# WHOIGit/ifcb_classifier

Measured on AMD Instinct MI355X. Metric: train images/sec, inception_v3 299^2 IFCB ROIs, higher is better.
Workload: dtype bf16; 1 GPU; inception_v3 100-class bf16 TRAIN, batch 256 per GPU, synthetic u8 ROIs h,w~U{32..299} resized on-GPU to 299x299 (BASELINE.json configs[1]); global_batch=256, parallelism=dp1, program_lanes=4, IFCBK_LANES=4, weight_gradient_lanes=1, optimizer=adam lr=1e-3, loss=CE + 0.4*CE_aux, input_pipeline=preprocess then step on one stream

## Files before the change

ifcb_classifier_amd/_lib.py:

```python
import ctypes as C
import os

_HERE = os.path.dirname(os.path.abspath(__file__))
LIB_PATH = os.path.join(_HERE, 'libifcbk.so')
if os.environ.get('IFCBK_LIB'):
    _alt = os.environ['IFCBK_LIB']
    if not (os.path.isabs(_alt) and os.path.isfile(_alt)):
        raise RuntimeError('IFCBK_LIB must be the absolute path of an existing libifcbk build, got %r' % _alt)
    import sys as _sys
    print('[ifcbk] IFCBK_LIB: loading %s instead of the in-tree library' % _alt, file=_sys.stderr)
    LIB_PATH = _alt

BF16, F32 = 0, 1
OK, EINVAL, EHIP, ENOMEM, EUNSUPPORTED = 0, -1, -2, -3, -4

(OP_CONV_FWD, OP_CONV_DGRAD, OP_CONV_WGRAD, OP_WEIGHT_PACK, OP_BN_FINALIZE, OP_BN_APPLY, OP_BN_BWD,
 OP_MAXPOOL_FWD, OP_MAXPOOL_BWD, OP_AVGPOOL_FWD, OP_AVGPOOL_BWD, OP_HEAD_FWD, OP_HEAD_BWD,
 OP_SOFTMAX_XENT, OP_SOFTMAX, OP_ADAM, OP_MEMSET, OP_COPY2D, OP_DROPOUT_MASK, OP_CONV_FWD_AFFINE,
 OP_WEIGHT_PACK_MULTI, OP_CONV_WGRAD_SEG, OP_BN_APPLY_MAXPOOL, OP_BN_BWD_MAXPOOL, OP_CONV_DGRAD_BNSTAT,
 OP_BN_BWD_PARTIALS, OP_BN_STATS, OP_AVGPOOL_AFFINE, OP_CONV_FWD_AFFINE_SEG, OP_SGD, OP_RETIRED_31,
 OP_BIAS_RELU_BWD, OP_DROPOUT, OP_FLATTEN_CHW, OP_STEM_U8_FWD, OP_STEM_U8_WGRAD, OP_CONV_FWD_AFFINE_MAXPOOL,
 OP_STEP_COUNTERS, OP_CONV_WGRAD_GROUP, OP_SOFTMAX_XENT_W) = range(1, 41)

OP_NAMES = {1: 'conv_fwd', 2: 'conv_dgrad', 3: 'conv_wgrad', 4: 'weight_pack', 5: 'bn_finalize', 6: 'bn_apply',
            7: 'bn_bwd', 8: 'maxpool_fwd', 9: 'maxpool_bwd', 10: 'avgpool_fwd', 11: 'avgpool_bwd', 12: 'head_fwd',
            13: 'head_bwd', 14: 'softmax_xent', 15: 'softmax', 16: 'adam', 17: 'memset', 18: 'copy2d',
            19: 'dropout_mask', 20: 'conv_fwd_affine', 21: 'weight_pack_multi', 22: 'conv_wgrad', 23: 'bn_apply_maxpool',
            24: 'bn_bwd_maxpool', 25: 'conv_dgrad', 26: 'bn_bwd', 27: 'bn_stats', 28: 'avgpool_fwd', 29: 'conv_fwd_affine', 30: 'sgd', 31: 'retired',
            32: 'bias_relu_bwd', 33: 'dropout', 34: 'flatten_chw', 35: 'conv_fwd', 36: 'conv_wgrad', 37: 'conv_fwd_affine', 38: 'step_counters', 39: 'conv_wgrad',
            40: 'softmax_xent_w'}


class ConvDesc(C.Structure):
    _fields_ = [(n, C.c_int32) for n in
                ('N', 'H', 'W', 'C', 'ldx', 'K', 'R', 'S', 'stride_h', 'stride_w', 'pad_h', 'pad_w', 'P', 'Q',
                 'ldy', 'Cw', 'dtype')]


class BnDesc(C.Structure):
    _fields_ = [(n, C.c_int32) for n in ('M', 'C', 'ldx', 'ldy', 'relu', 'dtype')] + \
               [('eps', C.c_float), ('momentum', C.c_float)]


class PoolDesc(C.Structure):
    _fields_ = [(n, C.c_int32) for n in
                ('N', 'H', 'W', 'C', 'ldx', 'R', 'S', 'stride_h', 'stride_w', 'pad_h', 'pad_w', 'P', 'Q', 'ldy',
                 'dtype')]


class HeadDesc(C.Structure):
    _fields_ = [(n, C.c_int32) for n in ('N', 'HW', 'C', 'ldx', 'NC', 'dtype')] + [('keep_scale', C.c_float)]


class RoiDesc(C.Structure):
    _fields_ = [(n, C.c_int32) for n in ('n_img', 'S', 'in_channels', 'out_channels', 'flip_bits_valid', 'dtype')] + \
               [('mean', C.c_float * 3), ('std', C.c_float * 3), ('tin_scale', C.c_float * 3),
                ('tin_shift', C.c_float * 3)]


class WgradItem(C.Structure):
    _fields_ = [('d', ConvDesc), ('x', C.c_void_p), ('dy', C.c_void_p), ('dw', C.c_void_p)]


class PackItem(C.Structure):
    _fields_ = [('w_master', C.c_void_p), ('w', C.c_void_p), ('wT', C.c_void_p), ('K', C.c_int32), ('RS', C.c_int32),
                ('C', C.c_int32), ('Cw', C.c_int32), ('first_block', C.c_int64), ('wT_ld', C.c_int32), ('pad_', C.c_int32)]


class _OpU(C.Union):
    _fields_ = [('conv', ConvDesc), ('bn', BnDesc), ('pool', PoolDesc), ('head', HeadDesc)]


class Op(C.Structure):
    _fields_ = [('kind', C.c_int32), ('flags', C.c_int32), ('p', C.c_void_p * 12), ('i', C.c_int64 * 4),
                ('f', C.c_float * 8), ('u', _OpU)]


_vp, _i, _f, _sz = C.c_void_p, C.c_int, C.c_float, C.c_size_t
_PROTOS = {
    'ifcbk_version': (C.c_char_p, []),
    'ifcbk_ctx_create': (_i, [_i, C.POINTER(_vp)]),
    'ifcbk_ctx_destroy': (_i, [_vp]),
    'ifcbk_ctx_reserve': (_i, [_vp, _sz]),
    'ifcbk_ctx_workspace_bytes': (_sz, [_vp]),
    'ifcbk_ctx_set_lanes': (_i, [_vp, _i]),
    'ifcbk_ctx_live_graphs': (_i, [_vp]),
    'ifcbk_last_error': (C.c_char_p, [_vp]),
    'ifcbk_conv2d_fwd': (_i, [_vp, C.POINTER(ConvDesc), _vp, _vp, _vp, _vp, _vp]),
    'ifcbk_conv2d_fwd_affine': (_i, [_vp, C.POINTER(ConvDesc), _vp, _vp, _vp, _vp, _vp, _vp, _i, _i, _vp]),
    'ifcbk_conv2d_fwd_affine_maxpool_ok': (_i, [C.POINTER(ConvDesc)]),
    'ifcbk_conv2d_fwd_affine_maxpool': (_i, [_vp, C.POINTER(ConvDesc), _vp, _vp, _vp, _i, _vp, _vp, _i, _vp]),
    'ifcbk_conv2d_dgrad': (_i, [_vp, C.POINTER(ConvDesc), _vp, _vp, _vp, _i, _vp]),
    'ifcbk_conv2d_wgrad': (_i, [_vp, C.POINTER(ConvDesc), _vp, _vp, _vp, _i, _vp]),
    'ifcbk_conv2d_wgrad_segments': (_i, [_vp, C.POINTER(ConvDesc), _vp, _vp, _i, C.POINTER(_vp), C.POINTER(C.c_int32), _i, _vp]),
    'ifcbk_bn_finalize_ld': (_i, [_vp, C.POINTER(BnDesc), _vp, _i, _i] + [_vp] * 9),
    'ifcbk_conv2d_wgrad_workspace': (_sz, [C.POINTER(ConvDesc)]),
    'ifcbk_conv2d_wgrad_group': (_i, [_vp, _i, C.POINTER(ConvDesc), C.POINTER(_vp), C.POINTER(_vp), C.POINTER(_vp), _i, _vp]),
    'ifcbk_conv2d_wgrad_group_workspace': (_sz, [_i, C.POINTER(ConvDesc)]),
    'ifcbk_conv2d_wgrad_group_member_kh': (_i, [C.POINTER(ConvDesc)]),
    'ifcbk_conv2d_wgrad_group_info': (_i, [_i, C.POINTER(ConvDesc), C.POINTER(_i), C.POINTER(_i), C.POINTER(_i)]),
    'ifcbk_conv2d_fwd_mblocks': (_i, [C.POINTER(ConvDesc)]),
    'ifcbk_weight_pack': (_i, [_vp, C.POINTER(ConvDesc), _vp, _vp, _vp, _vp]),
    'ifcbk_weight_pack_multi': (_i, [_vp, _vp, _i, C.c_int64, _i, _vp]),
    'ifcbk_bn_finalize': (_i, [_vp, C.POINTER(BnDesc), _vp, _i] + [_vp] * 9),
    'ifcbk_bn_apply': (_i, [_vp, C.POINTER(BnDesc), _vp, _vp, _vp, _vp, _i, _vp, _vp]),
    'ifcbk_bn_bwd': (_i, [_vp, C.POINTER(BnDesc), _vp, _vp, _vp, _i, _vp, _vp, _vp, _vp, _i, _vp, _i, _i, _vp, _vp,
                          _i, _vp, _vp, _vp]),
    'ifcbk_conv2d_fwd_affine_segments': (_i, [_vp, C.POINTER(ConvDesc), _vp, _vp, _i, C.POINTER(_vp), C.POINTER(C.c_int32),
                                          C.POINTER(C.c_int32), C.POINTER(C.c_int32), _vp, _vp, _vp]),
    'ifcbk_avgpool3x3_affine': (_i, [_vp, C.POINTER(PoolDesc), _vp, _vp, _vp, _i, _vp, _vp]),
    'ifcbk_bn_stats_rows': (_i, [C.c_int64]),
    'ifcbk_bn_stats': (_i, [_vp, C.POINTER(BnDesc), _vp, _vp, _vp]),
    'ifcbk_conv2d_dgrad_bnstat_mblocks': (_i, [C.POINTER(ConvDesc)]),
    'ifcbk_conv2d_dgrad_bnstat': (_i, [_vp, C.POINTER(ConvDesc), _vp, _vp, _vp, _vp, _i, _vp, _vp, _vp, _vp, _vp, _vp]),
    'ifcbk_bn_bwd_partials': (_i, [_vp, C.POINTER(BnDesc), _vp, _vp, _i, _vp, _vp, _vp, _vp, _vp, _vp, _i, _vp, _i, _vp, _vp, _i,
                                   _vp]),
    'ifcbk_bn_bwd_partials_ld': (_i, [_vp, C.POINTER(BnDesc), _vp, _vp, _i, _vp, _vp, _vp, _vp, _vp, _vp, _i, _i, _vp, _i, _vp, _vp,
                                      _i, _vp]),
    'ifcbk_bn_apply_maxpool': (_i, [_vp, C.POINTER(PoolDesc), _vp, _vp, _vp, _i, _vp, _vp, _vp]),
    'ifcbk_bn_bwd_maxpool': (_i, [_vp, C.POINTER(PoolDesc), _vp, _vp, _vp, _vp, _vp, _vp, _vp, _vp, _i, _vp, _i, _vp, _vp, _i,
                                  _vp]),
    'ifcbk_maxpool_fwd': (_i, [_vp, C.POINTER(PoolDesc), _vp, _vp, _vp, _vp]),
    'ifcbk_maxpool_bwd': (_i, [_vp, C.POINTER(PoolDesc), _vp, _vp, _vp, _i, _vp]),
    'ifcbk_avgpool_fwd': (_i, [_vp, C.POINTER(PoolDesc), _vp, _vp, _vp]),
    'ifcbk_avgpool_bwd': (_i, [_vp, C.POINTER(PoolDesc), _vp, _vp, _i, _vp]),
    'ifcbk_head_fwd': (_i, [_vp, C.POINTER(HeadDesc), _vp, _vp, _vp, _vp, _vp, _vp, _vp]),
    'ifcbk_head_bwd': (_i, [_vp, C.POINTER(HeadDesc), _vp, _vp, _vp, _vp, _vp, _vp, _vp, _i, _i, _vp]),
    'ifcbk_dropout_mask': (_i, [_vp, _vp, C.c_int64, _f, C.c_uint64, C.c_uint64, _vp]),
    'ifcbk_bias_relu_bwd': (_i, [_vp, C.c_int64, _i, _i, _vp, _i, _vp, _i, _vp, _i, _i, _vp, _i, _vp]),
    'ifcbk_bias_relu_bwd_workspace': (_sz, [C.c_int64, _i]),
    'ifcbk_bias_relu_bwd_rows': (_i, [C.c_int64]),
    'ifcbk_dropout_apply': (_i, [_vp, C.c_int64, _i, _vp, _vp, _f, _vp, _i, _vp]),
    'ifcbk_flatten_chw': (_i, [_vp, _i, _i, _i, _i, _vp, _i, _vp, _i, _i, _vp]),
    'ifcbk_softmax_xent': (_i, [_vp, _vp, _vp, _i, _i, _f, _vp, _i, _vp, _vp]),
    'ifcbk_softmax': (_i, [_vp, _vp, _i, _i, _vp, _vp]),
    'ifcbk_softmax_xent_w': (_i, [_vp, _vp, _vp, _vp, _i, _i, _f, _vp, _i, _vp, _vp]),
    'ifcbk_step_counters': (_i, [_vp, _vp, _i, _vp, _vp, _vp]),
    'ifcbk_adam_flat': (_i, [_vp, _vp, _vp, _vp, _vp, C.c_int64, _f, _f, _f, _f, _f, _i, _f, _vp]),
    'ifcbk_sgd_flat': (_i, [_vp, _vp, _vp, _vp, C.c_int64, _f, _f, _f, _f, _vp]),
    'ifcbk_roi_preprocess': (_i, [_vp, C.POINTER(RoiDesc), _vp, _vp, _vp, _vp, _vp, _i, _i, _vp, _vp, _vp]),
    'ifcbk_roi_preprocess_workspace': (_sz, [C.POINTER(RoiDesc), _i, _i]),
    'ifcbk_u8_channel_moments': (_i, [_vp, _vp, _i, C.c_int64, _i, _vp, _vp]),
    'ifcbk_stem_u8_rows': (_i, [C.POINTER(ConvDesc)]),
    'ifcbk_stem_u8_fwd': (_i, [_vp, C.POINTER(ConvDesc), _vp, _vp, _vp, _vp, _vp, _vp, _vp, _i, _vp]),
    'ifcbk_stem_u8_wgrad_workspace': (_sz, [C.POINTER(ConvDesc)]),
    'ifcbk_stem_u8_wgrad': (_i, [_vp, C.POINTER(ConvDesc), _vp, _vp, _vp, _vp, _i, _vp]),
    'ifcbk_nchw_to_nhwc': (_i, [_vp, _vp, _i, _i, _i, _i, _i, _i, C.POINTER(_f), C.POINTER(_f), _vp, _vp]),
    'ifcbk_nhwc_to_nchw_f32': (_i, [_vp, _vp, _i, _i, _i, _i, _i, _i, _vp, _vp]),
    'ifcbk_run_program': (_i, [_vp, C.POINTER(Op), _i, _vp, C.POINTER(_f)]),
    'ifcbk_run_program_ev': (_i, [_vp, C.POINTER(Op), _i, _vp, _i]),
    'ifcbk_program_times': (_i, [_vp, _i, _i, C.POINTER(_f)]),
    'ifcbk_program_capture': (_i, [_vp, C.POINTER(Op), _i, C.POINTER(_vp)]),
    'ifcbk_graph_launch': (_i, [_vp, _vp, _vp]),
    'ifcbk_graph_destroy': (_i, [_vp, _vp]),
    'ifcbk_op_kernel': (_i, [C.POINTER(Op), C.c_char_p, _sz]),
    'ifcbk_op_cost': (_i, [C.POINTER(Op), C.POINTER(C.c_double), C.POINTER(C.c_double)]),
}
EXPORTS = tuple(_PROTOS)

_lib = None


def load():
    global _lib
    if _lib is None:
        if not os.path.exists(LIB_PATH):
            raise RuntimeError('libifcbk.so not found at %s -- build it with `python -c "import __graft_entry__ as g; '
                               'g.build()"` (hipcc --offload-arch=gfx950); there is no CPU fallback' % LIB_PATH)
        import torch
        lib = C.CDLL(LIB_PATH)
        for name, (res, args) in _PROTOS.items():
            fn = getattr(lib, name)
            fn.restype = res
            fn.argtypes = args
        _lib = lib
    return _lib


class Context:

    def __init__(self, device=0):
        self.lib = load()
        h = _vp()
        rc = self.lib.ifcbk_ctx_create(int(device), C.byref(h))
        if rc != 0:
            raise RuntimeError('ifcbk_ctx_create(device=%d) failed with %d: %s' % (device, rc, self.lib.ifcbk_last_error(None).decode()))
        self.h = h
        self.device = device

    def call(self, name, *args):
        rc = getattr(self.lib, name)(self.h, *args)
        if rc != 0:
            raise RuntimeError('%s failed (%d): %s' % (name, rc, self.lib.ifcbk_last_error(self.h).decode()))

    def reserve(self, nbytes):
        self.call('ifcbk_ctx_reserve', int(nbytes))

    def run_program(self, ops, n, stream, op_ms=None):
        self.call('ifcbk_run_program', ops, int(n), stream, op_ms)

    def capture(self, ops, n):
        g = _vp()
        self.call('ifcbk_program_capture', ops, int(n), C.byref(g))
        return g

    def graph_launch(self, g, stream):
        self.call('ifcbk_graph_launch', g, stream)

    def live_graphs(self):
        return int(self.lib.ifcbk_ctx_live_graphs(self.h)) if self.h else 0

    def close(self):
        if getattr(self, 'h', None):
            self.lib.ifcbk_ctx_destroy(self.h)
            self.h = None

    def __del__(self):
        try:
            self.close()
        except Exception:
            pass


class PlanOnlyContext:

    def __init__(self):
        self.lib = load()
        self.h = None
        self.device = None

    def reserve(self, nbytes):
        pass

    def close(self):
        pass

    def call(self, name, *args):
        raise RuntimeError('%s: this engine was built with plan_only=True (no HIP context)' % name)

    run_program = capture = graph_launch = call


def ptr(t):
    return None if t is None else _vp(t.data_ptr())


def cur_stream():
    import torch
    return _vp(torch.cuda.current_stream().cuda_stream)
```

ifcb_classifier_amd/csrc/bn.hip:

```cpp
#include "common.h"
#include <stdlib.h>

namespace {

#ifdef IFCBK_EXPERIMENT_NOFINALIZE
__global__ void experiment_empty_kernel(float* p) { if (p && threadIdx.x == 1000) p[0] = 0.f; }
bool experiment_skip_finalize(hipStream_t st) {
    static const char* e = getenv("IFCBK_EXPERIMENT_NOFINALIZE");
    static const char* k = getenv("IFCBK_EXPERIMENT_EMPTYFINALIZE");
    static long seen = 0;
    if (!e) return false;
    const bool skip = ++seen > atol(e);
    if (skip && k) hipLaunchKernelGGL(experiment_empty_kernel, dim3(1), dim3(64), 0, st, (float*)nullptr);
    return skip;
}
#else
constexpr bool experiment_skip_finalize(hipStream_t) { return false; }
#endif

__global__ __launch_bounds__(1024) void bn_finalize_kernel(const float* part, int mblocks, int ldp, int C, double invM,
                                                            double unbias, const float* gamma, const float* beta,
                                                            float* rmean, float* rvar, float* mean_o, float* invstd_o,
                                                            float* scale, float* shift, float eps, float momentum) {
    __shared__ double s1[64][16], s2[64][16];
// ... 437 lines not shown
        }
    }
#pragma unroll
    for (int off = 8; off < 64; off <<= 1)
#pragma unroll
        for (int j = 0; j < E; ++j) {
            sb[j] += __shfl_xor(sb[j], off);
            sg[j] += __shfl_xor(sg[j], off);
        }
    if (lane < 8) {
#pragma unroll
        for (int j = 0; j < E; ++j) {
            red[wave][0][cc * E + j] = sb[j];
            red[wave][1][cc * E + j] = sg[j];
        }
    }
    __syncthreads();
    if (t < 2 * CG) {
        int which = t / CG, n = t - which * CG;
        int ch = blockIdx.y * CG + n;
        if (ch < C) {
            float s = red[0][which][n] + red[1][which][n] + red[2][which][n] + red[3][which][n];
            part[((size_t)blockIdx.x * 2 + which) * C + ch] = s;
        }
    }
}

__global__ __launch_bounds__(1024) void bn_bwd_finalize_kernel(const float* part, int ntiles, int C, float* dgamma,
                                                                float* dbeta, float* tmp, int accumulate, int ldp) {
    __shared__ double s[2][64][16];
    const int c = threadIdx.x & 15, rg = threadIdx.x >> 4;
    const int ch = blockIdx.x * 16 + c;
    double a = 0.0, b = 0.0;
    if (ch < C) {
        int i = rg;
        for (; i + 192 < ntiles; i += 256) {
            float v[8];
#pragma unroll
            for (int u = 0; u < 4; ++u) {
                v[2 * u] = part[((size_t)(i + 64 * u) * 2 + 0) * ldp + ch];
                v[2 * u + 1] = part[((size_t)(i + 64 * u) * 2 + 1) * ldp + ch];
            }
#pragma unroll
            for (int u = 0; u < 4; ++u) {
                a += (double)v[2 * u];
                b += (double)v[2 * u + 1];
            }
        }
        for (; i < ntiles; i += 64) {
            a += (double)part[((size_t)i * 2 + 0) * ldp + ch];
            b += (double)part[((size_t)i * 2 + 1) * ldp + ch];
        }
    }
    s[0][rg][c] = a;
    s[1][rg][c] = b;
    __syncthreads();
    if (threadIdx.x < 16 && ch < C) {
        double sa = 0.0, sg = 0.0;
        for (int i = 0; i < 64; ++i) {
            sa += s[0][i][c];
            sg += s[1][i][c];
        }
        tmp[ch] = (float)sa;
        tmp[C + ch] = (float)sg;
        dbeta[ch] = accumulate ? dbeta[ch] + (float)sa : (float)sa;
        dgamma[ch] = accumulate ? dgamma[ch] + (float)sg : (float)sg;
    }
}

template <class T, int MASK, bool POOLED>
__global__ __launch_bounds__(256) void bn_bwd_dx_kernel(const T* x, int ldx, const T* y, int ldy, const T* dy, int lddy,
                                                         const float* gamma, const float* mean, const float* invstd,
                                                         const float* scale, const float* shift, const float* tmp,
                                                         T* dx, int lddx, T* dres, int lddres, int dres_acc, int64_t M,
                                                         int C, float invM, fastdiv_t fcpr, PoolGather pg) {
    constexpr int E = Chunk<T>::N;
    extern __shared__ __attribute__((aligned(16))) float coef[];
    for (int c = threadIdx.x; c < C; c += 256) {
        float is = invstd[c], a_ = gamma[c] * is, dg = tmp[C + c] * invM, db = tmp[c] * invM;
        coef[c] = a_;
        coef[C + c] = -a_ * is * dg;
        coef[2 * C + c] = a_ * (mean[c] * is * dg - db);
        if (MASK == 2) {
            coef[3 * C + c] = scale[c];
            coef[4 * C + c] = shift[c];
        }
    }
    __syncthreads();
    const int cpr = C / E;
    const int64_t total = M * cpr;
    int64_t i = (int64_t)blockIdx.x * (256 * EW_ITER) + threadIdx.x;
#pragma unroll 2
    for (int it = 0; it < EW_ITER; ++it, i += 256) {
        if (i >= total) break;
        uint32_t m = fdiv((uint32_t)i, fcpr);
        int c = ((int)i - (int)m * cpr) * E;
        float fx[E], fy[E], fd[E], o[E];
        Chunk<T>::load(x + (int64_t)m * ldx + c, fx);
        if (POOLED) pooled_dy<T>(pg, dy, m, c, fd);
        else Chunk<T>::load(dy + (int64_t)m * lddy + c, fd);
        if (MASK == 1) Chunk<T>::load(y + (int64_t)m * ldy + c, fy);
#pragma unroll
        for (int j = 0; j < E; ++j) {
            float dz = fd[j];
            if (MASK == 1) dz = fy[j] > 0.f ? dz : 0.f;
            if (MASK == 2) dz = (fx[j] * coef[3 * C + c + j] + coef[4 * C + c + j]) > 0.f ? dz : 0.f;
            fd[j] = dz;
            o[j] = coef[c + j] * dz + (coef[C + c + j] * fx[j] + coef[2 * C + c + j]);
        }
        if (dres_acc & 2) {
            float fo[E];
            Chunk<T>::load(dx + (int64_t)m * lddx + c, fo);
#pragma unroll
            for (int j = 0; j < E; ++j) o[j] += fo[j];
        }
        if (dres) {
            T* rp = dres + (int64_t)m * lddres + c;
            if (dres_acc & 1) {
                float fr[E];
                Chunk<T>::load(rp, fr);
#pragma unroll
                for (int j = 0; j < E; ++j) fd[j] += fr[j];
            }
            Chunk<T>::store(rp, fd);
        }
        Chunk<T>::store(dx + (int64_t)m * lddx + c, o);
    }
}

template <class T>
int apply_t(ifcbk_ctx* ctx, const ifcbk_bn_desc* d, const void* x, const float* scale, const float* shift,
            const void* residual, int ldr, void* y, hipStream_t st) {
    constexpr int E = Chunk<T>::N;
    if (d->C % E || d->ldx % E || d->ldy % E) IFCBK_FAIL(ctx, IFCBK_EINVAL, "bn_apply: channels must be multiples of %d", E);
    const int cpr = d->C / E;
    const int64_t total = (int64_t)d->M * cpr;
    if (total >= (1ll << 31)) IFCBK_FAIL(ctx, IFCBK_EINVAL, "bn_apply: tensor too large");
    dim3 grid(cdiv(total, 256 * EW_ITER)), block(256);
    const size_t shm = (size_t)2 * d->C * sizeof(float);
    const fastdiv_t fc = make_fastdiv(cpr);
    const T* xx = (const T*)x; const T* rr = (const T*)residual; T* yy = (T*)y;
    if (d->relu && rr) hipLaunchKernelGGL((bn_apply_kernel<T, true, true>), grid, block, shm, st, xx, d->ldx, scale, shift, rr, ldr, yy, d->ldy, (int64_t)d->M, cpr, fc);
    else if (d->relu) hipLaunchKernelGGL((bn_apply_kernel<T, true, false>), grid, block, shm, st, xx, d->ldx, scale, shift, rr, ldr, yy, d->ldy, (int64_t)d->M, cpr, fc);
    else if (rr) hipLaunchKernelGGL((bn_apply_kernel<T, false, true>), grid, block, shm, st, xx, d->ldx, scale, shift, rr, ldr, yy, d->ldy, (int64_t)d->M, cpr, fc);
    else hipLaunchKernelGGL((bn_apply_kernel<T, false, false>), grid, block, shm, st, xx, d->ldx, scale, shift, rr, ldr, yy, d->ldy, (int64_t)d->M, cpr, fc);
    IFCBK_LAUNCH_CHECK(ctx, "bn_apply");
    return 0;
}

template <class T>
int bwd_t(ifcbk_ctx* ctx, const ifcbk_bn_desc* d, const void* x, const void* y, const void* dy, int lddy,
          const float* gamma, const float* mean, const float* invstd, void* dx, int lddx, void* dres, int lddres,
          int dres_accumulate, float* dgamma, float* dbeta, int param_accumulate, const float* scale, const float* shift,
          hipStream_t st, const PoolGather* pool = nullptr, const float* part_in = nullptr, int ntiles_in = 0, int part_ld_in = 0) {
    constexpr int E = Chunk<T>::N;
    constexpr int CG = 8 * E;
    PoolGather pg = {};
    if (pool) pg = *pool;
    const int C = d->C;
    if (C % E || d->ldx % E || lddy % E || lddx % E) IFCBK_FAIL(ctx, IFCBK_EINVAL, "bn_bwd: channels must be multiples of %d", E);
    const int64_t M = d->M;
    const int rows = bwd_rows(M, cdiv(C, CG));
    int ntiles = cdiv(M, rows);
    size_t need = ((size_t)ntiles * 2 * C + 2 * C) * sizeof(float);
    if (need > ctx->ws_bytes) IFCBK_FAIL(ctx, IFCBK_ENOMEM, "bn_bwd: workspace %zu > reserved %zu", need, ctx->ws_bytes);
    float* part = (float*)ctx->ws;
    float* tmp = part + (size_t)ntiles * 2 * C;
    const T* xx = (const T*)x; const T* yy = (const T*)y; const T* dd = (const T*)dy;
    dim3 g1(ntiles, cdiv(C, CG));
    const int mask = !d->relu ? 0 : ((scale && shift && !dres) ? 2 : 1);
    if (mask == 1 && !yy) IFCBK_FAIL(ctx, IFCBK_EINVAL, "bn_bwd: y is required for the ReLU mask");
    if (pool && pg.ph == 0 && pg.pw == 0) {
        if (mask == 1) IFCBK_FAIL(ctx, IFCBK_EINVAL, "bn_bwd_maxpool: needs scale/shift (the activation is not stored)");
        const int HB = (pg.H + 1) / 2, WB = (pg.W + 1) / 2;
        const int64_t nblk = (int64_t)(M / ((int64_t)pg.H * pg.W)) * HB * WB;
        const int64_t tot = nblk * (C / E);
        if (tot >= (1ll << 31) - 256) IFCBK_FAIL(ctx, IFCBK_EINVAL, "bn_bwd_maxpool: tensor too large");
        const int nt2 = cdiv(nblk, 256);
        if (((size_t)nt2 * 2 * C + 2 * C) * sizeof(float) > ctx->ws_bytes) IFCBK_FAIL(ctx, IFCBK_ENOMEM, "bn_bwd_maxpool: workspace");
        float* tmp2 = part + (size_t)nt2 * 2 * C;
        const fastdiv_t fHBWB = make_fastdiv(HB * WB), fWB = make_fastdiv(WB), fc2 = make_fastdiv(C / E);
        dim3 g2(nt2, cdiv(C, CG));
        if (mask == 2) hipLaunchKernelGGL((bn_bwd_reduce_pool2x2_kernel<T, 2>), g2, dim3(256), 0, st, xx, d->ldx, dd, mean, invstd, scale, shift, part, C, pg, HB, WB, (uint32_t)nblk, fHBWB, fWB);
        else hipLaunchKernelGGL((bn_bwd_reduce_pool2x2_kernel<T, 0>), g2, dim3(256), 0, st, xx, d->ldx, dd, mean, invstd, scale, shift, part, C, pg, HB, WB, (uint32_t)nblk, fHBWB, fWB);
        IFCBK_LAUNCH_CHECK(ctx, "bn_bwd_reduce_pool2x2");
        if (!experiment_skip_finalize(st)) hipLaunchKernelGGL(bn_bwd_finalize_kernel, dim3(cdiv(C, 16)), dim3(1024), 0, st, (const float*)part, nt2, C, dgamma, dbeta, tmp2, param_accumulate, C);
        IFCBK_LAUNCH_CHECK(ctx, "bn_bwd_finalize");
        const float invM2 = (float)(1.0 / (double)M);
        const size_t shm2 = (size_t)5 * C * sizeof(float);
        if (mask == 2) hipLaunchKernelGGL((bn_bwd_dx_pool2x2_kernel<T, 2>), dim3(cdiv(tot, 256)), dim3(256), shm2, st, xx, d->ldx, dd, gamma, mean, invstd, scale, shift, (const float*)tmp2, (T*)dx, lddx, C, invM2, pg, HB, WB, (uint32_t)tot, fc2, fHBWB, fWB);
        else hipLaunchKernelGGL((bn_bwd_dx_pool2x2_kernel<T, 0>), dim3(cdiv(tot, 256)), dim3(256), shm2, st, xx, d->ldx, dd, gamma, mean, invstd, scale, shift, (const float*)tmp2, (T*)dx, lddx, C, invM2, pg, HB, WB, (uint32_t)tot, fc2, fHBWB, fWB);
        IFCBK_LAUNCH_CHECK(ctx, "bn_bwd_dx_pool2x2");
        return 0;
    }
    if (part_in) {
        if (mask != 2 || dres) IFCBK_FAIL(ctx, IFCBK_EINVAL, "bn_bwd_partials: ReLU layer without residual, scale/shift required");
        part = const_cast<float*>(part_in);
        ntiles = ntiles_in;
        tmp = (float*)ctx->ws;
        if ((size_t)2 * C * sizeof(float) > ctx->ws_bytes) IFCBK_FAIL(ctx, IFCBK_ENOMEM, "bn_bwd_partials: workspace");
    } else if (pool) {
        if (mask == 1) IFCBK_FAIL(ctx, IFCBK_EINVAL, "bn_bwd_maxpool: needs scale/shift (the activation is not stored)");
        if (mask == 2) hipLaunchKernelGGL((bn_bwd_reduce_kernel<T, 2, true>), g1, dim3(256), 0, st, xx, d->ldx, yy, d->ldy, dd, lddy, mean, invstd, scale, shift, part, M, C, pg, rows);
        else hipLaunchKernelGGL((bn_bwd_reduce_kernel<T, 0, true>), g1, dim3(256), 0, st, xx, d->ldx, yy, d->ldy, dd, lddy, mean, invstd, scale, shift, part, M, C, pg, rows);
    } else if (mask == 2) hipLaunchKernelGGL((bn_bwd_reduce_kernel<T, 2, false>), g1, dim3(256), 0, st, xx, d->ldx, yy, d->ldy, dd, lddy, mean, invstd, scale, shift, part, M, C, pg, rows);
    else if (mask == 1) hipLaunchKernelGGL((bn_bwd_reduce_kernel<T, 1, false>), g1, dim3(256), 0, st, xx, d->ldx, yy, d->ldy, dd, lddy, mean, invstd, scale, shift, part, M, C, pg, rows);
    else hipLaunchKernelGGL((bn_bwd_reduce_kernel<T, 0, false>), g1, dim3(256), 0, st, xx, d->ldx, yy, d->ldy, dd, lddy, mean, invstd, scale, shift, part, M, C, pg, rows);
    IFCBK_LAUNCH_CHECK(ctx, "bn_bwd_reduce");
    if (!experiment_skip_finalize(st)) hipLaunchKernelGGL(bn_bwd_finalize_kernel, dim3(cdiv(C, 16)), dim3(1024), 0, st, (const float*)part, ntiles, C, dgamma, dbeta, tmp, param_accumulate, (part_in && part_ld_in > 0) ? part_ld_in : C);
    IFCBK_LAUNCH_CHECK(ctx, "bn_bwd_finalize");
    const int64_t total = M * (C / E);
    if (total >= (1ll << 31)) IFCBK_FAIL(ctx, IFCBK_EINVAL, "bn_bwd: tensor too large");
    const float invM = (float)(1.0 / (double)M);
    dim3 g3(cdiv(total, 256 * EW_ITER));
    const size_t shm = (size_t)5 * C * sizeof(float);
    const fastdiv_t fc = make_fastdiv(C / E);
    if (pool) {
        if (mask == 2) hipLaunchKernelGGL((bn_bwd_dx_kernel<T, 2, true>), g3, dim3(256), shm, st, xx, d->ldx, yy, d->ldy, dd, lddy, gamma, mean, invstd, scale, shift, (const float*)tmp, (T*)dx, lddx, (T*)dres, lddres, dres_accumulate, M, C, invM, fc, pg);
        else hipLaunchKernelGGL((bn_bwd_dx_kernel<T, 0, true>), g3, dim3(256), shm, st, xx, d->ldx, yy, d->ldy, dd, lddy, gamma, mean, invstd, scale, shift, (const float*)tmp, (T*)dx, lddx, (T*)dres, lddres, dres_accumulate, M, C, invM, fc, pg);
    } else if (mask == 2) hipLaunchKernelGGL((bn_bwd_dx_kernel<T, 2, false>), g3, dim3(256), shm, st, xx, d->ldx, yy, d->ldy, dd, lddy, gamma, mean, invstd, scale, shift, (const float*)tmp, (T*)dx, lddx, (T*)dres, lddres, dres_accumulate, M, C, invM, fc, pg);
    else if (mask == 1) hipLaunchKernelGGL((bn_bwd_dx_kernel<T, 1, false>), g3, dim3(256), shm, st, xx, d->ldx, yy, d->ldy, dd, lddy, gamma, mean, invstd, scale, shift, (const float*)tmp, (T*)dx, lddx, (T*)dres, lddres, dres_accumulate, M, C, invM, fc, pg);
    else hipLaunchKernelGGL((bn_bwd_dx_kernel<T, 0, false>), g3, dim3(256), shm, st, xx, d->ldx, yy, d->ldy, dd, lddy, gamma, mean, invstd, scale, shift, (const float*)tmp, (T*)dx, lddx, (T*)dres, lddres, dres_accumulate, M, C, invM, fc, pg);
    IFCBK_LAUNCH_CHECK(ctx, "bn_bwd_dx");
    return 0;
}

}

extern "C" int ifcbk_bn_finalize(ifcbk_ctx* ctx, const ifcbk_bn_desc* d, const float* part, int mblocks,
                                 const float* gamma, const float* beta, float* running_mean, float* running_var,
                                 float* mean, float* invstd, float* scale, float* shift, void* stream) {
    return ifcbk_bn_finalize_ld(ctx, d, part, mblocks, 0, gamma, beta, running_mean, running_var, mean, invstd, scale, shift, stream);
}

extern "C" int ifcbk_bn_finalize_ld(ifcbk_ctx* ctx, const ifcbk_bn_desc* d, const float* part, int mblocks, int part_ld,
                                    const float* gamma, const float* beta, float* running_mean, float* running_var,
                                    float* mean, float* invstd, float* scale, float* shift, void* stream) {
    if (!d || d->C <= 0) IFCBK_FAIL(ctx, IFCBK_EINVAL, "bn_finalize: bad desc");
    hipStream_t st = (hipStream_t)stream;
    int ldp = part_ld > 0 ? part_ld : d->C;
    if (part) {
        double M = (double)d->M;
        double unbias = d->M > 1 ? M / (M - 1.0) : 1.0;
        if (mblocks > 1536) {
            const int rpc = 64;
            int nchunk = cdiv(mblocks, rpc);
            size_t need = (size_t)nchunk * 2 * d->C * sizeof(float);
            if (need > ctx->ws_bytes) IFCBK_FAIL(ctx, IFCBK_ENOMEM, "bn_finalize: workspace %zu > reserved %zu", need, ctx->ws_bytes);
            hipLaunchKernelGGL(bn_prereduce_kernel, dim3(cdiv(d->C, 64), nchunk), dim3(256), 0, st, part, mblocks, ldp, d->C, rpc,
                               (float*)ctx->ws);
            IFCBK_LAUNCH_CHECK(ctx, "bn_prereduce");
            part = (const float*)ctx->ws;
            mblocks = nchunk;
            ldp = d->C;
        }
        if (!experiment_skip_finalize(st)) hipLaunchKernelGGL(bn_finalize_kernel, dim3(cdiv(d->C, 16)), dim3(1024), 0, st, part, mblocks, ldp, d->C, 1.0 / M,
                           unbias, gamma, beta, running_mean, running_var, mean, invstd, scale, shift, d->eps,
                           d->momentum);
    } else {
        hipLaunchKernelGGL(bn_eval_scale_kernel, dim3(cdiv(d->C, 256)), dim3(256), 0, st, d->C, gamma, beta,
                           (const float*)running_mean, (const float*)running_var, scale, shift, d->eps);
    }
    IFCBK_LAUNCH_CHECK(ctx, "bn_finalize");
    return 0;
}

extern "C" int ifcbk_bn_stats_rows(int64_t M) { return (int)((M + STAT_ROWS - 1) / STAT_ROWS); }

extern "C" int ifcbk_bn_stats(ifcbk_ctx* ctx, const ifcbk_bn_desc* d, const void* x, float* part, void* stream) {
    if (!d || !x || !part) IFCBK_FAIL(ctx, IFCBK_EINVAL, "bn_stats: null operand");
    if (d->dtype != IFCBK_BF16 && d->dtype != IFCBK_F32) IFCBK_FAIL(ctx, IFCBK_EUNSUPPORTED, "bn_stats: dtype must be bf16 or f32");
    const int e = dtype_chunk(d->dtype);
    if (d->C % e || d->ldx % e || d->M <= 0) IFCBK_FAIL(ctx, IFCBK_EINVAL, "bn_stats: C=%d ldx=%d must be multiples of %d, M > 0", d->C, d->ldx, e);
    const dim3 grid((unsigned)ifcbk_bn_stats_rows(d->M), (unsigned)cdiv(d->C, 8 * e));
    if (d->dtype == IFCBK_F32) hipLaunchKernelGGL(bn_stats_kernel<float>, grid, dim3(256), 0, (hipStream_t)stream, (const float*)x, d->ldx, part, d->M, d->C);
    else hipLaunchKernelGGL(bn_stats_kernel<bf16_t>, grid, dim3(256), 0, (hipStream_t)stream, (const bf16_t*)x, d->ldx, part, d->M, d->C);
    IFCBK_LAUNCH_CHECK(ctx, "bn_stats");
    return 0;
}

extern "C" int ifcbk_bn_apply(ifcbk_ctx* ctx, const ifcbk_bn_desc* d, const void* x, const float* scale,
                              const float* shift, const void* residual, int ldr, void* y, void* stream) {
    if (!d) IFCBK_FAIL(ctx, IFCBK_EINVAL, "bn_apply: null desc");
    if (d->dtype == IFCBK_F32) return apply_t<float>(ctx, d, x, scale, shift, residual, ldr, y, (hipStream_t)stream);
    if (d->dtype == IFCBK_BF16) return apply_t<bf16_t>(ctx, d, x, scale, shift, residual, ldr, y, (hipStream_t)stream);
    IFCBK_FAIL(ctx, IFCBK_EINVAL, "bn_apply: bad dtype");
}

extern "C" int ifcbk_bn_bwd(ifcbk_ctx* ctx, const ifcbk_bn_desc* d, const void* x, const void* y, const void* dy,
                            int lddy, const float* gamma, const float* mean, const float* invstd, void* dx, int lddx,
                            void* dres, int lddres, int dres_accumulate, float* dgamma, float* dbeta,
                            int param_accumulate, const float* scale, const float* shift, void* stream) {
    if (!d) IFCBK_FAIL(ctx, IFCBK_EINVAL, "bn_bwd: null desc");
    if (d->dtype == IFCBK_F32)
        return bwd_t<float>(ctx, d, x, y, dy, lddy, gamma, mean, invstd, dx, lddx, dres, lddres, dres_accumulate, dgamma,
                            dbeta, param_accumulate, scale, shift, (hipStream_t)stream);
    if (d->dtype == IFCBK_BF16)
        return bwd_t<bf16_t>(ctx, d, x, y, dy, lddy, gamma, mean, invstd, dx, lddx, dres, lddres, dres_accumulate, dgamma,
                             dbeta, param_accumulate, scale, shift, (hipStream_t)stream);
    IFCBK_FAIL(ctx, IFCBK_EINVAL, "bn_bwd: bad dtype");
}

namespace {
struct ApplyPoolArgs {
    int H, W, P, Q, cpr, ldx, ldy, sh, sw, ph, pw, relu;
    uint32_t total;
    fastdiv_t f_cpr, f_q, f_p;
};
template <class T>
__global__ __launch_bounds__(256) void bn_apply_maxpool_kernel(const T* x, const float* scale, const float* shift, T* y,
                                                               uint8_t* arg, ApplyPoolArgs a) {
    constexpr int E = Chunk<T>::N;
    extern __shared__ __attribute__((aligned(16))) float coef[];
    const int C = a.cpr * E;
    for (int c = threadIdx.x; c < C; c += 256) {
        coef[c] = scale[c];
        coef[C + c] = shift[c];
    }
    __syncthreads();
    const uint32_t i = xcd_remap(blockIdx.x, gridDim.x) * 256u + threadIdx.x;
    if (i >= a.total) return;
    const uint32_t pix = fdiv(i, a.f_cpr);
    const int c = (int)(i - pix * a.cpr) * E;
    const uint32_t t2 = fdiv(pix, a.f_q);
    const int q = (int)(pix - t2 * a.Q);
    const uint32_t n = fdiv(t2, a.f_p);
    const int p = (int)(t2 - n * a.P);
    const int h0 = p * a.sh - a.ph, w0 = q * a.sw - a.pw;
    float sc[E], sf[E], best[E];
    int bi[E];
#pragma unroll
    for (int j = 0; j < E; ++j) { sc[j] = coef[c + j]; sf[j] = coef[C + c + j]; best[j] = -INFINITY; bi[j] = 0; }
    typename Chunk<T>::raw_t rv[9];
#pragma unroll
    for (int r = 0; r < 3; ++r)
#pragma unroll
        for (int s = 0; s < 3; ++s) {
            const int h = min(max(h0 + r, 0), a.H - 1), w = min(max(w0 + s, 0), a.W - 1);
            rv[r * 3 + s] = Chunk<T>::load_raw(x + ((int64_t)(n * a.H + h) * a.W + w) * a.ldx + c);
        }
    bool first = true;
#pragma unroll
    for (int r = 0; r < 3; ++r)
#pragma unroll
        for (int s = 0; s < 3; ++s) {
            const int h = h0 + r, w = w0 + s;
            const bool in = h >= 0 && h < a.H && w >= 0 && w < a.W;
            float f[E];
            Chunk<T>::widen(rv[r * 3 + s], f);
#pragma unroll
            for (int j = 0; j < E; ++j) {
                float v = f[j] * sc[j] + sf[j];
                if (a.relu) v = fmaxf(v, 0.f);
                v = Chunk<T>::round(v);
                if (in && (first || v > best[j] || v != v)) { best[j] = v; bi[j] = r * 3 + s; }
            }
            first = first && !in;
        }
    Chunk<T>::store(y + (int64_t)pix * a.ldy + c, best);
    if (arg) ArgPack<E>::store(arg + (int64_t)pix * C + c, bi);
}

int pooled_check(ifcbk_ctx* ctx, const ifcbk_pool_desc* d, const char* who) {
    if (!d || (d->dtype != IFCBK_BF16 && d->dtype != IFCBK_F32)) IFCBK_FAIL(ctx, IFCBK_EINVAL, "%s: bad desc", who);
    const int e = dtype_chunk(d->dtype);
    if (d->C % e || d->ldx % e || d->ldy % e) IFCBK_FAIL(ctx, IFCBK_EINVAL, "%s: channels must be multiples of %d", who, e);
    if (d->R != 3 || d->S != 3 || d->stride_h != 2 || d->stride_w != 2 || d->pad_h > 1 || d->pad_w > 1 || d->pad_h < 0 || d->pad_w < 0)
        IFCBK_FAIL(ctx, IFCBK_EUNSUPPORTED, "%s: only 3x3 / stride 2 / pad <= 1 max pools are fused", who);
    if ((int64_t)d->N * d->H * d->W * (d->C / e) >= (1ll << 31) - 256) IFCBK_FAIL(ctx, IFCBK_EINVAL, "%s: tensor too large", who);
    return 0;
}
}

extern "C" int ifcbk_bn_apply_maxpool(ifcbk_ctx* ctx, const ifcbk_pool_desc* d, const void* x, const float* scale,
                                      const float* shift, int relu, void* y, uint8_t* argmax, void* stream) {
    if (int e = pooled_check(ctx, d, "bn_apply_maxpool")) return e;
    ApplyPoolArgs a;
    a.H = d->H; a.W = d->W; a.P = d->P; a.Q = d->Q; a.ldx = d->ldx; a.ldy = d->ldy;
    a.sh = 2; a.sw = 2; a.ph = d->pad_h; a.pw = d->pad_w; a.relu = relu;
    a.cpr = d->C / dtype_chunk(d->dtype);
    a.total = (uint32_t)((int64_t)d->N * d->P * d->Q * a.cpr);
    a.f_cpr = make_fastdiv(a.cpr); a.f_q = make_fastdiv(d->Q); a.f_p = make_fastdiv(d->P);
    if (a.total == 0) return IFCBK_OK;
    const size_t shm = (size_t)2 * d->C * sizeof(float);
    hipStream_t st = (hipStream_t)stream;
    if (d->dtype == IFCBK_F32) hipLaunchKernelGGL(bn_apply_maxpool_kernel<float>, dim3(cdiv(a.total, 256)), dim3(256), shm, st, (const float*)x, scale, shift, (float*)y, argmax, a);
    else hipLaunchKernelGGL(bn_apply_maxpool_kernel<bf16_t>, dim3(cdiv(a.total, 256)), dim3(256), shm, st, (const bf16_t*)x, scale, shift, (bf16_t*)y, argmax, a);
    IFCBK_LAUNCH_CHECK(ctx, "bn_apply_maxpool");
    return 0;
}

extern "C" int ifcbk_bn_bwd_partials_ld(ifcbk_ctx* ctx, const ifcbk_bn_desc* d, const void* x, const void* dy, int lddy,
                                        const float* gamma, const float* mean, const float* invstd, const float* scale,
                                        const float* shift, const float* part, int ntiles, int part_ld, void* dx, int lddx,
                                        float* dgamma, float* dbeta, int param_accumulate, void* stream) {
    if (!d || !part || ntiles <= 0 || part_ld < 0) IFCBK_FAIL(ctx, IFCBK_EINVAL, "bn_bwd_partials: bad args");
    if (d->dtype == IFCBK_F32)
        return bwd_t<float>(ctx, d, x, nullptr, dy, lddy, gamma, mean, invstd, dx, lddx, nullptr, 0, 0, dgamma, dbeta,
                            param_accumulate, scale, shift, (hipStream_t)stream, nullptr, part, ntiles, part_ld);
    if (d->dtype == IFCBK_BF16)
        return bwd_t<bf16_t>(ctx, d, x, nullptr, dy, lddy, gamma, mean, invstd, dx, lddx, nullptr, 0, 0, dgamma, dbeta,
                             param_accumulate, scale, shift, (hipStream_t)stream, nullptr, part, ntiles, part_ld);
    IFCBK_FAIL(ctx, IFCBK_EINVAL, "bn_bwd_partials: bad dtype");
}

extern "C" int ifcbk_bn_bwd_partials(ifcbk_ctx* ctx, const ifcbk_bn_desc* d, const void* x, const void* dy, int lddy,
                                     const float* gamma, const float* mean, const float* invstd, const float* scale,
                                     const float* shift, const float* part, int ntiles, void* dx, int lddx, float* dgamma,
                                     float* dbeta, int param_accumulate, void* stream) {
    return ifcbk_bn_bwd_partials_ld(ctx, d, x, dy, lddy, gamma, mean, invstd, scale, shift, part, ntiles, 0, dx, lddx, dgamma, dbeta,
                                    param_accumulate, stream);
}

extern "C" int ifcbk_bn_bwd_maxpool(ifcbk_ctx* ctx, const ifcbk_pool_desc* d, const void* x, const void* dpool,
                                    const uint8_t* argmax, const float* gamma, const float* mean, const float* invstd,
                                    const float* scale, const float* shift, int relu, void* dx, int lddx, float* dgamma,
                                    float* dbeta, int param_accumulate, void* stream) {
    if (int e = pooled_check(ctx, d, "bn_bwd_maxpool")) return e;
    if (!argmax || !dpool) IFCBK_FAIL(ctx, IFCBK_EINVAL, "bn_bwd_maxpool: pooled gradient and arg-max required");
    ifcbk_bn_desc b;
    b.M = (int64_t)d->N * d->H * d->W; b.C = d->C; b.ldx = d->ldx; b.ldy = d->ldx; b.relu = relu; b.dtype = d->dtype;
    b.eps = 0.f; b.momentum = 0.f;
    PoolGather pg;
    pg.arg = argmax; pg.H = d->H; pg.W = d->W; pg.P = d->P; pg.Q = d->Q; pg.ph = d->pad_h; pg.pw = d->pad_w;
    pg.ldp = d->ldy; pg.C = d->C;
    pg.fHW = make_fastdiv(d->H * d->W); pg.fW = make_fastdiv(d->W);
    if (d->dtype == IFCBK_F32)
        return bwd_t<float>(ctx, &b, x, nullptr, dpool, 0, gamma, mean, invstd, dx, lddx, nullptr, 0, 0, dgamma, dbeta,
                            param_accumulate, scale, shift, (hipStream_t)stream, &pg);
    return bwd_t<bf16_t>(ctx, &b, x, nullptr, dpool, 0, gamma, mean, invstd, dx, lddx, nullptr, 0, 0, dgamma, dbeta,
                         param_accumulate, scale, shift, (hipStream_t)stream, &pg);
}
```

ifcb_classifier_amd/csrc/conv_stem_u8.hip:

```cpp
#include "common.h"
#include <stdlib.h>

namespace {

constexpr int K1 = 32;
constexpr int PIXB = 2048;

struct StemArgs {
    const uint8_t* g;
    const float* w;
    const float* ab;
    void* y;
    const void* dy;
    float* part;
    const float* scale;
    const float* shift;
    int relu, H, W, P, Q, ld;
    unsigned M, PQ;
    fastdiv_t dPQ, dQ;
    unsigned rows, gpr;
    fastdiv_t dP, dG;
#ifdef IFCBK_EXPERIMENT_STEM
    int dbg;
#endif
};
#ifdef IFCBK_EXPERIMENT_STEM
#define STEM_DBG(a, bit) ((a).dbg & (bit))
#else
#define STEM_DBG(a, bit) 0
#endif

template <class T> __device__ __forceinline__ void store8(T* p, const float* f);
template <> __device__ __forceinline__ void store8<bf16_t>(bf16_t* p, const float* f) { *reinterpret_cast<uint4*>(p) = pack8(f); }
template <> __device__ __forceinline__ void store8<float>(float* p, const float* f) {
    *reinterpret_cast<float4*>(p) = make_float4(f[0], f[1], f[2], f[3]);
    *reinterpret_cast<float4*>(p + 4) = make_float4(f[4], f[5], f[6], f[7]);
}
template <class T> __device__ __forceinline__ void load8(const T* p, float* f);
template <> __device__ __forceinline__ void load8<bf16_t>(const bf16_t* p, float* f) { unpack8(*reinterpret_cast<const uint4*>(p), f); }
template <> __device__ __forceinline__ void load8<float>(const float* p, float* f) {
    *reinterpret_cast<float4*>(f) = *reinterpret_cast<const float4*>(p);
    *reinterpret_cast<float4*>(f + 4) = *reinterpret_cast<const float4*>(p + 4);
}

__device__ __forceinline__ void taps_raw(const StemArgs& a, unsigned m, uint8_t* gb) {
    const unsigned n = fdiv(m, a.dPQ), rem = m - n * a.PQ;
    const unsigned p = fdiv(rem, a.dQ), q = rem - p * (unsigned)a.Q;
    const uint8_t* s = a.g + ((size_t)n * a.H + 2 * p) * a.W + 2 * q;
#pragma unroll
    for (int r = 0; r < 3; ++r)
#pragma unroll
        for (int c = 0; c < 3; ++c) gb[r * 3 + c] = s[(size_t)r * a.W + c];
}

constexpr int UNR = 4;

template <class T, bool AFFINE>
__global__ __launch_bounds__(256) void stem_u8_fwd_kernel(StemArgs a) {
    const int c8 = threadIdx.x & 3, pl = threadIdx.x >> 2;
    float we[8][9], bias[8];
    {
        float av[3], bv[3];
#pragma unroll
        for (int c = 0; c < 3; ++c) { av[c] = a.ab[c]; bv[c] = a.ab[3 + c]; }
#pragma unroll
        for (int j = 0; j < 8; ++j) {
            const float* wk = a.w + (size_t)(c8 * 8 + j) * 27;
            float b = 0.f;
#pragma unroll
            for (int t = 0; t < 9; ++t) {
                const float w0 = wk[t * 3], w1 = wk[t * 3 + 1], w2 = wk[t * 3 + 2];
                we[j][t] = w0 * av[0] + w1 * av[1] + w2 * av[2];
                b += w0 * bv[0] + w1 * bv[1] + w2 * bv[2];
            }
            bias[j] = b;
        }
    }
    float sc[8], sh[8];
    if (AFFINE) {
#pragma unroll
        for (int j = 0; j < 8; ++j) { sc[j] = a.scale[c8 * 8 + j]; sh[j] = a.shift[c8 * 8 + j]; }
    }
    float s1[8], s2[8];
#pragma unroll
    for (int j = 0; j < 8; ++j) s1[j] = s2[j] = 0.f;
    const unsigned m0 = blockIdx.x * (unsigned)PIXB + pl;
    T* y = (T*)a.y;
    for (int it = 0; it < PIXB / 64; it += UNR) {
        if (m0 + it * 64 >= a.M) break;
        uint8_t gb[UNR][9];
#pragma unroll
        for (int u = 0; u < UNR; ++u) {
            const unsigned m = m0 + (it + u) * 64;
            taps_raw(a, m < a.M ? m : a.M - 1, gb[u]);
        }
#pragma unroll
        for (int u = 0; u < UNR; ++u) {
            const unsigned m = m0 + (it + u) * 64;
            if (m >= a.M) break;
            float gt[9], o[8];
#pragma unroll
            for (int t = 0; t < 9; ++t) gt[t] = (float)gb[u][t];
#pragma unroll
            for (int j = 0; j < 8; ++j) {
                float v = bias[j];
#pragma unroll
                for (int t = 0; t < 9; ++t) v = fmaf(gt[t], we[j][t], v);
                if (AFFINE) {
                    v = fmaf(v, sc[j], sh[j]);
                    if (a.relu) v = v > 0.f ? v : 0.f;
                } else {
                    v = Chunk<T>::round(v);
                    s1[j] += v;
                    s2[j] = fmaf(v, v, s2[j]);
                }
                o[j] = v;
            }
            store8<T>(y + (size_t)m * a.ld + c8 * 8, o);
        }
    }
    if (AFFINE || !a.part) return;
    __shared__ float red[4][2][K1];
#pragma unroll
    for (int j = 0; j < 8; ++j) {
#pragma unroll
        for (int d = 4; d < 64; d <<= 1) {
            s1[j] += __shfl_xor(s1[j], d);
            s2[j] += __shfl_xor(s2[j], d);
        }
    }
    const int lane = threadIdx.x & 63, wv = threadIdx.x >> 6;
    if (lane < 4) {
#pragma unroll
        for (int j = 0; j < 8; ++j) { red[wv][0][lane * 8 + j] = s1[j]; red[wv][1][lane * 8 + j] = s2[j]; }
    }
    __syncthreads();
    if (threadIdx.x < 2 * K1) {
        const int st = threadIdx.x >> 5, ch = threadIdx.x & 31;
        a.part[((size_t)blockIdx.x * 2 + st) * K1 + ch] = (red[0][st][ch] + red[1][st][ch]) + (red[2][st][ch] + red[3][st][ch]);
    }
}

template <class T>
__global__ __launch_bounds__(256) void stem_u8_wgrad_kernel(StemArgs a) {
    const int c8 = threadIdx.x & 3, pl = threadIdx.x >> 2;
    float acc[8][10];
#pragma unroll
    for (int j = 0; j < 8; ++j)
#pragma unroll
        for (int t = 0; t < 10; ++t) acc[j][t] = 0.f;
    const unsigned m0 = blockIdx.x * (unsigned)PIXB + pl;
    const T* dy = (const T*)a.dy;
    for (int it = 0; it < PIXB / 64; it += UNR) {
        if (m0 + it * 64 >= a.M) break;
        uint8_t gb[UNR][9];
        float d[UNR][8];
#pragma unroll
        for (int u = 0; u < UNR; ++u) {
            const unsigned m = m0 + (it + u) * 64, mc = m < a.M ? m : a.M - 1;
            load8<T>(dy + (size_t)mc * a.ld + c8 * 8, d[u]);
            taps_raw(a, mc, gb[u]);
        }
#pragma unroll
        for (int u = 0; u < UNR; ++u) {
            if (m0 + (it + u) * 64 >= a.M) break;
            float gt[9];
#pragma unroll
            for (int t = 0; t < 9; ++t) gt[t] = (float)gb[u][t];
#pragma unroll
            for (int j = 0; j < 8; ++j) {
#pragma unroll
                for (int t = 0; t < 9; ++t) acc[j][t] = fmaf(d[u][j], gt[t], acc[j][t]);
                acc[j][9] += d[u][j];
            }
        }
    }
    __shared__ float red[4][K1 * 10];
    const int lane = threadIdx.x & 63, wv = threadIdx.x >> 6;
#pragma unroll
    for (int j = 0; j < 8; ++j)
#pragma unroll
        for (int t = 0; t < 10; ++t) {
            float v = acc[j][t];
#pragma unroll
            for (int d = 4; d < 64; d <<= 1) v += __shfl_xor(v, d);
            if (lane < 4) red[wv][(lane * 8 + j) * 10 + t] = v;
        }
    __syncthreads();
    for (int i = threadIdx.x; i < K1 * 10; i += 256)
        a.part[(size_t)blockIdx.x * (K1 * 10) + i] = (red[0][i] + red[1][i]) + (red[2][i] + red[3][i]);
}

typedef __attribute__((ext_vector_type(16))) float f32x16_t;
constexpr int RB = 8;

__device__ __forceinline__ unsigned bfbits(float f) { return __float_as_uint(f) >> 16; }
__device__ __forceinline__ unsigned bfpair(unsigned lo, unsigned hi) { return lo | (hi << 16); }
__device__ __forceinline__ void split3(float w, unsigned& hi, unsigned& mid, unsigned& lo) {
    hi = f2bf(w);
    const float r1 = w - bf2f((bf16_t)hi);
    mid = f2bf(r1);
    lo = f2bf(r1 - bf2f((bf16_t)mid));
}
__device__ __forceinline__ bf16x8_t frag(unsigned a, unsigned b, unsigned c, unsigned d) {
    u32x4_t v = {a, b, c, d};
    return __builtin_bit_cast(bf16x8_t, v);
}

template <bool AFFINE>
__global__ __launch_bounds__(256) void stem_u8_fwd_mfma_kernel(StemArgs a) {
    const int lane = threadIdx.x & 63, wv = __builtin_amdgcn_readfirstlane(threadIdx.x >> 6);
    const int j = lane & 31, h = lane >> 5;
    bf16x8_t W1, W2;
    {
        const float* wk = a.w + (size_t)j * 27;
        unsigned hi[9], mid[9], lo[9], bh, bm, bl;
        float b = 0.f;
#pragma unroll
        for (int t = 0; t < 9; ++t) {
            const float w0 = wk[t * 3], w1 = wk[t * 3 + 1], w2 = wk[t * 3 + 2];
            split3(w0 * a.ab[0] + w1 * a.ab[1] + w2 * a.ab[2], hi[t], mid[t], lo[t]);
            b += w0 * a.ab[3] + w1 * a.ab[4] + w2 * a.ab[5];
        }
        split3(b, bh, bm, bl);
        if (h == 0) {
            W1 = frag(bfpair(hi[0], hi[1]), bfpair(hi[2], hi[3]), bfpair(hi[4], hi[5]), bfpair(hi[6], hi[7]));
            W2 = frag(bfpair(mid[0], mid[1]), bfpair(mid[2], mid[3]), bfpair(mid[4], mid[5]), bfpair(mid[6], mid[7]));
        } else {
            W1 = frag(bfpair(hi[8], mid[8]), bfpair(lo[8], bh), bfpair(bm, bl), 0u);
            W2 = frag(bfpair(lo[0], lo[1]), bfpair(lo[2], lo[3]), bfpair(lo[4], lo[5]), bfpair(lo[6], lo[7]));
        }
    }
    float sc = 1.f, sh = 0.f;
    if (AFFINE) { sc = a.scale[j]; sh = a.shift[j]; }
    float s1 = 0.f, s2 = 0.f;
    unsigned voff[16];
#pragma unroll
    for (int v = 0; v < 16; ++v) voff[v] = ((unsigned)(8 * (v >> 2) + 4 * h + (v & 3)) * (unsigned)a.ld + (unsigned)j) * 2u;
    const unsigned row0 = blockIdx.x * (unsigned)RB, nitem = (unsigned)RB * a.gpr;
    const unsigned ONE = 0x3f80u;
    const unsigned ovl = a.gpr * 32 - (unsigned)a.Q;
    auto fetch = [&](unsigned item, unsigned& row, unsigned& grp, unsigned short* r01, uint8_t* r2) {
        const unsigned rr = fdiv(item, a.dG);
        grp = item - rr * a.gpr;
        row = row0 + rr;
        const unsigned rowc = row < a.rows ? row : a.rows - 1;
        const unsigned n = fdiv(rowc, a.dP), p = rowc - n * (unsigned)a.P;
        const unsigned q = grp * 32 - (grp == a.gpr - 1 ? ovl : 0u) + j;
        const uint8_t* s = a.g + ((size_t)n * a.H + 2 * p) * a.W + 2 * q;
#pragma unroll
        for (int r = 0; r < 3; ++r) {
            __builtin_memcpy(&r01[r], s + (size_t)r * a.W, 2);
            r2[r] = s[(size_t)r * a.W + 2];
        }
    };
    unsigned row, grp, row_n, grp_n;
    unsigned short r01[3], r01_n[3];
    uint8_t r2[3], r2_n[3];
    fetch(wv, row_n, grp_n, r01_n, r2_n);
    __builtin_amdgcn_s_waitcnt(0x0F70);
    for (unsigned item = wv; item < nitem; item += 4) {
        row = row_n; grp = grp_n;
#pragma unroll
        for (int r = 0; r < 3; ++r) { r01[r] = r01_n[r]; r2[r] = r2_n[r]; }
        if (row >= a.rows) break;
        __builtin_amdgcn_sched_barrier(0);
        unsigned t[9];
#pragma unroll
        for (int r = 0; r < 3; ++r) {
            t[3 * r] = bfbits((float)(r01[r] & 0xffu));
            t[3 * r + 1] = bfbits((float)(r01[r] >> 8));
            t[3 * r + 2] = bfbits((float)r2[r]);
        }
        if (STEM_DBG(a, 1)) {
#pragma unroll
            for (int i = 0; i < 9; ++i) t[i] = bfbits((float)((lane + i) & 255));
        }
        fetch(item + 4 < nitem ? item + 4 : item, row_n, grp_n, r01_n, r2_n);
        const bf16x8_t G2 = frag(bfpair(t[0], t[1]), bfpair(t[2], t[3]), bfpair(t[4], t[5]), bfpair(t[6], t[7]));
        const bf16x8_t G1 = h ? frag(bfpair(t[8], t[8]), bfpair(t[8], ONE), bfpair(ONE, ONE), 0u) : G2;
        f32x16_t acc;
#pragma unroll
        for (int v = 0; v < 16; ++v) acc[v] = 0.f;
        acc = __builtin_amdgcn_mfma_f32_32x32x16_bf16(G1, W1, acc, 0, 0, 0);
        acc = __builtin_amdgcn_mfma_f32_32x32x16_bf16(G2, W2, acc, 0, 0, 0);
        const unsigned skip = grp == a.gpr - 1 ? ovl : 0u;
        const size_t gbase = ((size_t)row * a.Q + grp * 32 - skip) * a.ld * 2;
        uint8_t* yb = (uint8_t*)a.y + (((size_t)(unsigned)__builtin_amdgcn_readfirstlane((unsigned)(gbase >> 32)) << 32) |
                                       (size_t)(unsigned)__builtin_amdgcn_readfirstlane((unsigned)gbase));
        unsigned short ob[16];
#pragma unroll
        for (int v = 0; v < 16; ++v) {
            float x = acc[v];
            if (AFFINE) {
                x = fmaf(x, sc, sh);
                if (a.relu) x = x > 0.f ? x : 0.f;
            }
            ob[v] = f2bf(x);
        }
        if (!AFFINE && !STEM_DBG(a, 4)) {
            if (skip == 0) {
#pragma unroll
                for (int v = 0; v < 16; ++v) {
                    const float x = bf2f(ob[v]);
                    s1 += x;
                    s2 = fmaf(x, x, s2);
                }
            } else {
#pragma unroll
                for (int v = 0; v < 16; ++v) {
                    const float x = (unsigned)(8 * (v >> 2) + 4 * h + (v & 3)) >= skip ? bf2f(ob[v]) : 0.f;
                    s1 += x;
                    s2 = fmaf(x, x, s2);
                }
            }
        }
#pragma unroll
        for (int v = 0; v < 16; ++v)
            if (!STEM_DBG(a, 2) || ob[v] == 0x1234) *reinterpret_cast<bf16_t*>(yb + voff[v]) = ob[v];
        __builtin_amdgcn_sched_barrier(0);
    }
    if (AFFINE || !a.part) return;
    __shared__ float red[4][2][K1];
    s1 += __shfl_xor(s1, 32);
    s2 += __shfl_xor(s2, 32);
    if (h == 0) { red[wv][0][j] = s1; red[wv][1][j] = s2; }
    __syncthreads();
    if (threadIdx.x < 2 * K1) {
        const int st = threadIdx.x >> 5, ch = threadIdx.x & 31;
        a.part[((size_t)blockIdx.x * 2 + st) * K1 + ch] = (red[0][st][ch] + red[1][st][ch]) + (red[2][st][ch] + red[3][st][ch]);
    }
}

__global__ __launch_bounds__(256) void stem_u8_wgrad_mfma_kernel(StemArgs a) {
    const int lane = threadIdx.x & 63, wv = __builtin_amdgcn_readfirstlane(threadIdx.x >> 6);
    const int c = lane & 15, kg = lane >> 4;
    const int tr = c < 9 ? c / 3 : 0, tc = c < 9 ? c % 3 : 0;
    f32x4_t acc0 = {0.f, 0.f, 0.f, 0.f}, acc1 = {0.f, 0.f, 0.f, 0.f};
    const unsigned row0 = blockIdx.x * (unsigned)RB, nitem = (unsigned)RB * a.gpr;
    const bf16_t* dy = (const bf16_t*)a.dy;
    for (unsigned item = wv; item < nitem; item += 4) {
        const unsigned rr = fdiv(item, a.dG), grp = item - rr * a.gpr, row = row0 + rr;
        if (row >= a.rows) break;
        const unsigned n = fdiv(row, a.dP), p = row - n * (unsigned)a.P;
        const unsigned q0 = grp * 32 + 8 * kg;
        const bf16_t* dp = dy + (size_t)row * a.Q * a.ld + c;
        const uint8_t* s = a.g + ((size_t)n * a.H + 2 * p + tr) * a.W + tc;
        unsigned d0[8], d1[8], gb[8];
#pragma unroll
        for (int e = 0; e < 8; ++e) {
            const unsigned q = q0 + e;
            const bool ok = q < (unsigned)a.Q;
            const unsigned qc = ok ? q : (unsigned)a.Q - 1;
            const unsigned v0 = dp[(size_t)qc * a.ld], v1 = dp[(size_t)qc * a.ld + 16];
            d0[e] = ok ? v0 : 0u;
            d1[e] = ok ? v1 : 0u;
            gb[e] = s[2 * qc];
        }
        unsigned g16[8];
#pragma unroll
        for (int e = 0; e < 8; ++e) g16[e] = c < 9 ? bfbits((float)gb[e]) : (c == 9 ? 0x3f80u : 0u);
        const bf16x8_t A0 = frag(bfpair(d0[0], d0[1]), bfpair(d0[2], d0[3]), bfpair(d0[4], d0[5]), bfpair(d0[6], d0[7]));
        const bf16x8_t A1 = frag(bfpair(d1[0], d1[1]), bfpair(d1[2], d1[3]), bfpair(d1[4], d1[5]), bfpair(d1[6], d1[7]));
        const bf16x8_t B = frag(bfpair(g16[0], g16[1]), bfpair(g16[2], g16[3]), bfpair(g16[4], g16[5]), bfpair(g16[6], g16[7]));
        acc0 = __builtin_amdgcn_mfma_f32_16x16x32_bf16(A0, B, acc0, 0, 0, 0);
        acc1 = __builtin_amdgcn_mfma_f32_16x16x32_bf16(A1, B, acc1, 0, 0, 0);
    }
    __shared__ float red[4][K1][16];
#pragma unroll
    for (int v = 0; v < 4; ++v) {
        red[wv][4 * kg + v][c] = acc0[v];
        red[wv][16 + 4 * kg + v][c] = acc1[v];
    }
    __syncthreads();
    for (int i = threadIdx.x; i < K1 * 10; i += 256) {
        const int k = i / 10, t = i - k * 10;
        a.part[(size_t)blockIdx.x * (K1 * 10) + i] = (red[0][k][t] + red[1][k][t]) + (red[2][k][t] + red[3][k][t]);
    }
}

__global__ __launch_bounds__(640) void stem_u8_wgrad_reduce_kernel(const float* part, int nblk, const float* ab, float* dw, int accumulate) {
    __shared__ double s[64][10];
    __shared__ double tot[10];
    const int k = blockIdx.x, t = threadIdx.x % 10, rg = threadIdx.x / 10;
    double v = 0.0;
    int i = rg;
    for (; i + 192 < nblk; i += 256) {
        float f[4];
#pragma unroll
        for (int u = 0; u < 4; ++u) f[u] = part[((size_t)(i + 64 * u) * K1 + k) * 10 + t];
#pragma unroll
        for (int u = 0; u < 4; ++u) v += (double)f[u];
    }
    for (; i < nblk; i += 64) v += (double)part[((size_t)i * K1 + k) * 10 + t];
    s[rg][t] = v;
    __syncthreads();
    if (threadIdx.x < 10) {
        double z = 0.0;
        for (int r = 0; r < 64; ++r) z += s[r][threadIdx.x];
        tot[threadIdx.x] = z;
    }
    __syncthreads();
    if (threadIdx.x < 27) {
        const int tap = threadIdx.x / 3, c = threadIdx.x % 3;
        const float val = (float)((double)ab[c] * tot[tap] + (double)ab[3 + c] * tot[9]);
        float* o = dw + (size_t)k * 27 + threadIdx.x;
        *o = accumulate ? *o + val : val;
    }
}

bool stem_ok(const ifcbk_conv_desc* d) {
    return d && (d->dtype == IFCBK_BF16 || d->dtype == IFCBK_F32) && d->K == K1 && d->R == 3 && d->S == 3 && d->stride_h == 2 &&
           d->stride_w == 2 && d->pad_h == 0 && d->pad_w == 0 && d->Cw == 3 && d->N > 0 && d->H >= 3 && d->W >= 3 &&
           d->P == (d->H - 3) / 2 + 1 && d->Q == (d->W - 3) / 2 + 1 && d->ldy >= K1 && d->ldy % 8 == 0 &&
           (int64_t)d->N * d->P * d->Q < (1ll << 31) - PIXB;
}

StemArgs stem_args(const ifcbk_conv_desc* d, const uint8_t* g, const float* w, const float* ab) {
    StemArgs a = {};
    a.g = g; a.w = w; a.ab = ab;
    a.H = d->H; a.W = d->W; a.P = d->P; a.Q = d->Q; a.ld = d->ldy;
    a.PQ = (unsigned)(d->P * d->Q);
    a.M = (unsigned)((int64_t)d->N * d->P * d->Q);
    a.dPQ = make_fastdiv(a.PQ);
    a.dQ = make_fastdiv((unsigned)d->Q);
    a.rows = (unsigned)(d->N * d->P);
    a.gpr = (unsigned)cdiv(d->Q, 32);
    a.dP = make_fastdiv((unsigned)d->P);
    a.dG = make_fastdiv(a.gpr);
#ifdef IFCBK_EXPERIMENT_STEM
    a.dbg = getenv("IFCBK_STEM_DBG") ? atoi(getenv("IFCBK_STEM_DBG")) : 0;
#endif
    return a;
}

}

static bool stem_mfma(const ifcbk_conv_desc* d) { return d->dtype == IFCBK_BF16 && d->Q >= 32; }
extern "C" int ifcbk_stem_u8_rows(const ifcbk_conv_desc* d) {
    if (!stem_ok(d)) return 0;
    return stem_mfma(d) ? cdiv((int64_t)d->N * d->P, RB) : cdiv((int64_t)d->N * d->P * d->Q, PIXB);
}

extern "C" size_t ifcbk_stem_u8_wgrad_workspace(const ifcbk_conv_desc* d) {
    return stem_ok(d) ? (size_t)ifcbk_stem_u8_rows(d) * K1 * 10 * sizeof(float) : 0;
}

extern "C" int ifcbk_stem_u8_fwd(ifcbk_ctx* ctx, const ifcbk_conv_desc* d, const uint8_t* g, const float* w_master, const float* ab,
                                 void* y, float* bn_part, const float* scale, const float* shift, int relu, void* stream) {
    if (!stem_ok(d)) IFCBK_FAIL(ctx, IFCBK_EUNSUPPORTED, "stem_u8_fwd: 3x3 / stride 2 / unpadded / 32 output channels / Cw = 3 only");
    if (!g || !w_master || !ab || !y || ((scale == nullptr) != (shift == nullptr))) IFCBK_FAIL(ctx, IFCBK_EINVAL, "stem_u8_fwd: null operand");
    StemArgs a = stem_args(d, g, w_master, ab);
    a.y = y; a.part = bn_part; a.scale = scale; a.shift = shift; a.relu = relu;
    const dim3 grid((unsigned)ifcbk_stem_u8_rows(d)), blk(256);
    hipStream_t st = (hipStream_t)stream;
    const bool f32 = d->dtype == IFCBK_F32;
    if (scale) {
        if (f32) hipLaunchKernelGGL((stem_u8_fwd_kernel<float, true>), grid, blk, 0, st, a);
        else if (stem_mfma(d)) hipLaunchKernelGGL((stem_u8_fwd_mfma_kernel<true>), grid, blk, 0, st, a);
        else hipLaunchKernelGGL((stem_u8_fwd_kernel<bf16_t, true>), grid, blk, 0, st, a);
    } else {
        if (f32) hipLaunchKernelGGL((stem_u8_fwd_kernel<float, false>), grid, blk, 0, st, a);
        else if (stem_mfma(d)) hipLaunchKernelGGL((stem_u8_fwd_mfma_kernel<false>), grid, blk, 0, st, a);
        else hipLaunchKernelGGL((stem_u8_fwd_kernel<bf16_t, false>), grid, blk, 0, st, a);
    }
    IFCBK_LAUNCH_CHECK(ctx, "stem_u8_fwd");
    return IFCBK_OK;
}

extern "C" int ifcbk_stem_u8_wgrad(ifcbk_ctx* ctx, const ifcbk_conv_desc* d, const uint8_t* g, const void* dy, const float* ab,
                                   float* dw, int accumulate, void* stream) {
    if (!stem_ok(d)) IFCBK_FAIL(ctx, IFCBK_EUNSUPPORTED, "stem_u8_wgrad: 3x3 / stride 2 / unpadded / 32 output channels / Cw = 3 only");
    if (!g || !dy || !ab || !dw) IFCBK_FAIL(ctx, IFCBK_EINVAL, "stem_u8_wgrad: null operand");
    const size_t need = ifcbk_stem_u8_wgrad_workspace(d);
    if (need > ctx->ws_bytes) IFCBK_FAIL(ctx, IFCBK_ENOMEM, "stem_u8_wgrad: workspace %zu > reserved %zu", need, ctx->ws_bytes);
    StemArgs a = stem_args(d, g, nullptr, ab);
    a.dy = dy; a.part = (float*)ctx->ws;
    const int nblk = ifcbk_stem_u8_rows(d);
    hipStream_t st = (hipStream_t)stream;
    if (d->dtype == IFCBK_F32) hipLaunchKernelGGL(stem_u8_wgrad_kernel<float>, dim3(nblk), dim3(256), 0, st, a);
    else if (stem_mfma(d)) hipLaunchKernelGGL(stem_u8_wgrad_mfma_kernel, dim3(nblk), dim3(256), 0, st, a);
    else hipLaunchKernelGGL(stem_u8_wgrad_kernel<bf16_t>, dim3(nblk), dim3(256), 0, st, a);
    IFCBK_LAUNCH_CHECK(ctx, "stem_u8_wgrad");
    hipLaunchKernelGGL(stem_u8_wgrad_reduce_kernel, dim3(K1), dim3(640), 0, st, (const float*)ctx->ws, nblk, ab, dw, accumulate);
    IFCBK_LAUNCH_CHECK(ctx, "stem_u8_wgrad_reduce");
    return IFCBK_OK;
}
```

ifcb_classifier_amd/csrc/ctx.hip:

```cpp
#include "common.h"
#include <execinfo.h>
#include <signal.h>
#include <stdlib.h>
#include <string.h>
#include <unistd.h>

static void segv_backtrace(int sig) {
    static const char head[] = "\n[ifcbk] fatal signal -- host backtrace:\n";
    (void)!write(2, head, sizeof(head) - 1);
    void* frames[48];
    const int n = backtrace(frames, 48);
    backtrace_symbols_fd(frames, n, 2);
    signal(sig, SIG_DFL);
    raise(sig);
}
static void maybe_install_backtrace() {
    static int done = 0;
    if (done) return;
    done = 1;
    const char* e = getenv("IFCBK_SEGV_BACKTRACE");
    if (!e || !atoi(e)) return;
    void* warm[4];
    (void)backtrace(warm, 4);
    static char altstack[1 << 16];
    stack_t ss;
    ss.ss_sp = altstack; ss.ss_size = sizeof(altstack); ss.ss_flags = 0;
    sigaltstack(&ss, nullptr);
    struct sigaction sa;
    memset(&sa, 0, sizeof(sa));
    sa.sa_handler = segv_backtrace;
    sa.sa_flags = SA_ONSTACK | SA_NODEFER;
    sigaction(SIGSEGV, &sa, nullptr);
    sigaction(SIGABRT, &sa, nullptr);
    sigaction(SIGBUS, &sa, nullptr);
}

extern "C" const char* ifcbk_version(void) { return "ifcbk 0.1 (gfx950, bf16 MFMA)"; }

static char g_create_err[256] = "no ifcbk_ctx_create call has failed";

extern "C" int ifcbk_ctx_create(int device, ifcbk_ctx** out) {
    if (!out) return IFCBK_EINVAL;
    *out = nullptr;
    maybe_install_backtrace();
    int n = 0;
    hipError_t e = hipGetDeviceCount(&n);
    if (e != hipSuccess || device < 0 || device >= n) {
        snprintf(g_create_err, sizeof(g_create_err), "ifcbk_ctx_create(device=%d): hipGetDeviceCount -> %d device(s), %s", device, n,
                 hipGetErrorString(e));
        return IFCBK_EHIP;
    }
    ifcbk_ctx* c = (ifcbk_ctx*)calloc(1, sizeof(ifcbk_ctx));
    if (!c) return IFCBK_ENOMEM;
    c->device = device;
    c->ws_lanes = 4;
    const char* what = "hipSetDevice";
    e = hipSetDevice(device);
    if (e == hipSuccess) { what = "hipMalloc"; e = hipMalloc(&c->zeros, 4096); }
    if (e == hipSuccess) { what = "hipMemset"; e = hipMemset(c->zeros, 0, 4096); }
    if (e != hipSuccess) {
        snprintf(g_create_err, sizeof(g_create_err), "ifcbk_ctx_create(device=%d): %s: %s", device, what, hipGetErrorString(e));
        free(c);
        return IFCBK_EHIP;
    }
    *out = c;
    return IFCBK_OK;
}

static void graph_free(ifcbk_ctx* c, ifcbk_graph* g);

extern "C" int ifcbk_ctx_destroy(ifcbk_ctx* c) {
    if (!c) return IFCBK_OK;
    while (c->graphs) graph_free(c, c->graphs);
    if (c->ws_base) (void)hipFree(c->ws_base);
    if (c->zeros) (void)hipFree(c->zeros);
    for (int l = 1; l < IFCBK_MAX_LANES; ++l) {
        if (c->lane_st[l]) (void)hipStreamDestroy(c->lane_st[l]);
        if (c->cap_st[l]) (void)hipStreamDestroy(c->cap_st[l]);
    }
    for (int i = 0; i < c->n_xev; ++i) (void)hipEventDestroy(c->xev[i]);
    for (int i = 0; i < c->n_cev; ++i) (void)hipEventDestroy(c->cev[i]);
    free(c->cev);
    for (int i = 0; i < c->n_ev; ++i) (void)hipEventDestroy(c->ev[i]);
    free(c->ev);
    for (int s = 0; s < 256; ++s) {
        for (int i = 0; i < c->slot_n[s]; ++i) (void)hipEventDestroy(c->slot_ev[s][i]);
        free(c->slot_ev[s]);
        free(c->slot_rec[s]);
    }
    free(c);
    return IFCBK_OK;
}

extern "C" int ifcbk_ctx_reserve(ifcbk_ctx* c, size_t bytes) {
    if (!c) return IFCBK_EINVAL;
    if (bytes <= c->ws_bytes) return IFCBK_OK;
    IFCBK_HIP(c, hipSetDevice(c->device));
    IFCBK_HIP(c, hipDeviceSynchronize());
    if (c->ws_base) IFCBK_HIP(c, hipFree(c->ws_base));
    c->ws = c->ws_base = nullptr;
    c->ws_bytes = 0;
    bytes = (bytes + 255) & ~(size_t)255;
    IFCBK_HIP(c, hipMalloc(&c->ws_base, bytes * (size_t)c->ws_lanes));
    c->ws = c->ws_base;
    c->ws_bytes = bytes;
    ++c->ws_epoch;
    return IFCBK_OK;
}

extern "C" size_t ifcbk_ctx_workspace_bytes(ifcbk_ctx* c) { return c ? c->ws_bytes : 0; }

extern "C" int ifcbk_ctx_set_lanes(ifcbk_ctx* c, int lanes) {
    if (!c || lanes < 1 || lanes > IFCBK_MAX_LANES) return IFCBK_EINVAL;
    if (lanes == c->ws_lanes) return IFCBK_OK;
    if (c->ws_base && lanes > c->ws_lanes)
        IFCBK_FAIL(c, IFCBK_EINVAL, "ctx_set_lanes: %d arenas are reserved; set the lane count before ifcbk_ctx_reserve", c->ws_lanes);
    if (!c->ws_base) c->ws_lanes = lanes;
    return IFCBK_OK;
}

extern "C" int ifcbk_ctx_live_graphs(ifcbk_ctx* c) { return c ? c->n_graphs : 0; }

extern "C" const char* ifcbk_last_error(ifcbk_ctx* c) { return c ? c->err : g_create_err; }

static int run_one(ifcbk_ctx* c, const ifcbk_op* o, void* st) {
    void* const* p = o->p;
    const int acc = o->flags & 1, pacc = (o->flags >> 1) & 1;
    switch (o->kind) {
        case IFCBK_OP_CONV_FWD: return ifcbk_conv2d_fwd(c, &o->u.conv, p[0], p[1], p[2], (float*)p[3], st);
        case IFCBK_OP_CONV_FWD_AFFINE:
            return ifcbk_conv2d_fwd_affine(c, &o->u.conv, p[0], p[1], p[2], (const float*)p[3], (const float*)p[4], p[5],
                                           (int)o->i[0], (o->flags >> 2) & 1, st);
        case IFCBK_OP_CONV_DGRAD: return ifcbk_conv2d_dgrad(c, &o->u.conv, p[0], p[1], p[2], acc, st);
        case IFCBK_OP_CONV_WGRAD: return ifcbk_conv2d_wgrad(c, &o->u.conv, p[0], p[1], (float*)p[2], acc, st);
        case IFCBK_OP_CONV_FWD_AFFINE_MAXPOOL:
            return ifcbk_conv2d_fwd_affine_maxpool(c, &o->u.conv, p[0], p[1], p[2], (int)o->i[0], (const float*)p[3], (const float*)p[4],
                                                   (o->flags >> 2) & 1, st);
        case IFCBK_OP_STEM_U8_FWD:
            return ifcbk_stem_u8_fwd(c, &o->u.conv, (const uint8_t*)p[0], (const float*)p[1], (const float*)p[2], p[3], (float*)p[4],
                                     (const float*)p[5], (const float*)p[6], (o->flags >> 2) & 1, st);
        case IFCBK_OP_STEM_U8_WGRAD:
            return ifcbk_stem_u8_wgrad(c, &o->u.conv, (const uint8_t*)p[0], p[1], (const float*)p[2], (float*)p[3], acc, st);
        case IFCBK_OP_CONV_WGRAD_SEG: {
            float* dws[4];
            int32_t ks[4];
            int ns = 0;
            for (int k = 0; k < 4 && o->i[k] > 0; ++k) { dws[ns] = (float*)p[2 + k]; ks[ns] = (int32_t)o->i[k]; ++ns; }
            return ifcbk_conv2d_wgrad_segments(c, &o->u.conv, p[0], p[1], ns, dws, ks, acc, st);
        }
        case IFCBK_OP_WEIGHT_PACK_MULTI:
            return ifcbk_weight_pack_multi(c, (const ifcbk_pack_item*)p[0], (int)o->i[0], o->i[1], (int)o->i[2], st);
        case IFCBK_OP_WEIGHT_PACK: return ifcbk_weight_pack(c, &o->u.conv, (const float*)p[0], p[1], p[2], st);
        case IFCBK_OP_BN_FINALIZE:
            return ifcbk_bn_finalize_ld(c, &o->u.bn, (const float*)p[0], (int)o->i[0], (int)o->i[1], (const float*)p[1], (const float*)p[2],
                                     (float*)p[3], (float*)p[4], (float*)p[5], (float*)p[6], (float*)p[7], (float*)p[8], st);
        case IFCBK_OP_BN_APPLY:
            return ifcbk_bn_apply(c, &o->u.bn, p[0], (const float*)p[1], (const float*)p[2], p[3], (int)o->i[0], p[4], st);
        case IFCBK_OP_BN_BWD:
            return ifcbk_bn_bwd(c, &o->u.bn, p[0], p[1], p[2], (int)o->i[0], (const float*)p[3], (const float*)p[4],
                                (const float*)p[5], p[6], (int)o->i[1], p[7], (int)o->i[2], acc | (((o->flags >> 3) & 1) << 1), (float*)p[8], (float*)p[9],
                                pacc, (const float*)p[10], (const float*)p[11], st);
        case IFCBK_OP_CONV_DGRAD_BNSTAT:
            return ifcbk_conv2d_dgrad_bnstat(c, &o->u.conv, p[0], p[1], p[2], p[3], (int)o->i[0], (const float*)p[4], (const float*)p[5],
                                             (const float*)p[6], (const float*)p[7], (float*)p[8], st);
        case IFCBK_OP_BN_BWD_PARTIALS:
            return ifcbk_bn_bwd_partials_ld(c, &o->u.bn, p[0], p[1], (int)o->i[0], (const float*)p[2], (const float*)p[3], (const float*)p[4],
                                            (const float*)p[5], (const float*)p[6], (const float*)p[7], (int)o->i[1], (int)o->i[3], p[8],
                                            (int)o->i[2], (float*)p[9], (float*)p[10], pacc, st);
        case IFCBK_OP_CONV_FWD_AFFINE_SEG: {
            void* ys[4];
            int32_t ld[4], ks[4], af[4];
            int ns = 0;
            for (int k = 0; k < 4 && (o->i[k] & 0xfffff) > 0; ++k) {
                ys[ns] = p[2 + k]; ks[ns] = (int32_t)(o->i[k] & 0xfffff); ld[ns] = (int32_t)((o->i[k] >> 20) & 0xfffff);
                af[ns] = (int32_t)((o->i[k] >> 40) & 1); ++ns;
            }
            return ifcbk_conv2d_fwd_affine_segments(c, &o->u.conv, p[0], p[1], ns, ys, ld, ks, af, (const float*)p[6], (const float*)p[7], st);
        }
        case IFCBK_OP_BN_STATS: return ifcbk_bn_stats(c, &o->u.bn, p[0], (float*)p[1], st);
        case IFCBK_OP_AVGPOOL_AFFINE:
            return ifcbk_avgpool3x3_affine(c, &o->u.pool, p[0], (const float*)p[1], (const float*)p[2], (o->flags >> 2) & 1, p[3], st);
        case IFCBK_OP_BN_APPLY_MAXPOOL:
            return ifcbk_bn_apply_maxpool(c, &o->u.pool, p[0], (const float*)p[1], (const float*)p[2], (int)o->i[0], p[3], (uint8_t*)p[4], st);
        case IFCBK_OP_BN_BWD_MAXPOOL:
            return ifcbk_bn_bwd_maxpool(c, &o->u.pool, p[0], p[1], (const uint8_t*)p[2], (const float*)p[3], (const float*)p[4],
                                        (const float*)p[5], (const float*)p[6], (const float*)p[7], (int)o->i[0], p[8], (int)o->i[1],
                                        (float*)p[9], (float*)p[10], pacc, st);
        case IFCBK_OP_MAXPOOL_FWD: return ifcbk_maxpool_fwd(c, &o->u.pool, p[0], p[1], (uint8_t*)p[2], st);
        case IFCBK_OP_MAXPOOL_BWD: return ifcbk_maxpool_bwd(c, &o->u.pool, p[0], (const uint8_t*)p[1], p[2], acc, st);
        case IFCBK_OP_AVGPOOL_FWD: return ifcbk_avgpool_fwd(c, &o->u.pool, p[0], p[1], st);
        case IFCBK_OP_AVGPOOL_BWD: return ifcbk_avgpool_bwd(c, &o->u.pool, p[0], p[1], acc, st);
        case IFCBK_OP_HEAD_FWD:
            return ifcbk_head_fwd(c, &o->u.head, p[0], (const uint8_t*)p[1], (const float*)p[2], (const float*)p[3],
                                  (float*)p[4], (float*)p[5], st);
        case IFCBK_OP_HEAD_BWD:
            return ifcbk_head_bwd(c, &o->u.head, (const float*)p[0], (const float*)p[1], (const uint8_t*)p[2],
                                  (const float*)p[3], (float*)p[4], (float*)p[5], p[6], (int)o->i[0], pacc, st);
        case IFCBK_OP_SOFTMAX_XENT:
            return ifcbk_softmax_xent(c, (const float*)p[0], (const int64_t*)p[1], (int)o->i[0], (int)o->i[1], o->f[0],
                                      (float*)p[2], acc, (float*)p[3], st);
        case IFCBK_OP_SOFTMAX_XENT_W:
            return ifcbk_softmax_xent_w(c, (const float*)p[0], (const int64_t*)p[1], (const float*)p[4], (int)o->i[0], (int)o->i[1], o->f[0],
                                        (float*)p[2], acc, (float*)p[3], st);
        case IFCBK_OP_SOFTMAX: return ifcbk_softmax(c, (const float*)p[0], (int)o->i[0], (int)o->i[1], (float*)p[1], st);
        case IFCBK_OP_ADAM:
            return ifcbk_adam_flat(c, (float*)p[0], (const float*)p[1], (float*)p[2], (float*)p[3], o->i[0], o->f[0], o->f[1],
                                   o->f[2], o->f[3], o->f[4], (int)o->i[1], o->f[5], st);
        case IFCBK_OP_SGD:
            return ifcbk_sgd_flat(c, (float*)p[0], (const float*)p[1], (float*)p[2], o->i[0], o->f[0], o->f[1], o->f[2], o->f[3], st);
        case IFCBK_OP_MEMSET:
            IFCBK_HIP(c, hipMemsetAsync(p[0], (int)o->i[1], (size_t)o->i[0], (hipStream_t)st));
            return 0;
        case IFCBK_OP_COPY2D:
            IFCBK_HIP(c, hipMemcpy2DAsync(p[0], (size_t)o->i[0], p[1], (size_t)o->i[1], (size_t)o->i[2], (size_t)o->i[3],
                                          hipMemcpyDeviceToDevice, (hipStream_t)st));
            return 0;
        case IFCBK_OP_BIAS_RELU_BWD:
            return ifcbk_bias_relu_bwd(c, o->u.bn.M, o->u.bn.C, o->u.bn.dtype, p[0], o->u.bn.ldx, p[1], o->u.bn.ldy, p[2], (int)o->i[0],
                                       o->u.bn.relu, (float*)p[3], pacc, st);
        case IFCBK_OP_DROPOUT:
            return ifcbk_dropout_apply(c, o->i[0], (int)o->i[1], p[0], (const uint8_t*)p[1], o->f[0], p[2], acc, st);
        case IFCBK_OP_FLATTEN_CHW:
            return ifcbk_flatten_chw(c, (int)o->i[0], (int)o->i[1], (int)o->i[2], (int)(o->i[3] >> 32), p[0], (int)(o->i[3] & 0xffffffff),
                                     p[1], (o->flags >> 2) & 1, acc, st);
        case IFCBK_OP_CONV_WGRAD_GROUP: {
            const ifcbk_wgrad_item* it = (const ifcbk_wgrad_item*)p[0];
            const int n = (int)o->i[0];
            if (!it || n < 1 || n > 8) IFCBK_FAIL(c, IFCBK_EINVAL, "run_program: wgrad group of %d", n);
            ifcbk_conv_desc ds[8];
            const void *xs[8], *dys[8];
            float* dws[8];
            for (int k = 0; k < n; ++k) { ds[k] = it[k].d; xs[k] = it[k].x; dys[k] = it[k].dy; dws[k] = it[k].dw; }
            return ifcbk_conv2d_wgrad_group(c, n, ds, xs, dys, dws, acc, st);
        }
        case IFCBK_OP_STEP_COUNTERS:
            return ifcbk_step_counters(c, (int64_t*)p[0], (int)o->i[0], (float*)p[1], (const float*)p[2], st);
        case IFCBK_OP_DROPOUT_MASK:
            return ifcbk_dropout_mask(c, (uint8_t*)p[0], o->i[0], o->f[0], (uint64_t)o->i[1], (uint64_t)o->i[2], st);
        default: IFCBK_FAIL(c, IFCBK_EINVAL, "run_program: unknown op kind %d", o->kind);
    }
}

static inline int op_lane(const ifcbk_op* o) { return (o->flags >> 8) & 7; }
static inline int op_wait(const ifcbk_op* o) { return (o->flags >> 12) & 255; }

static int lane_resources(ifcbk_ctx* c, int used) {
    if (c->n_xev < 64) {
        for (int i = c->n_xev; i < 64; ++i) IFCBK_HIP(c, hipEventCreateWithFlags(&c->xev[i], hipEventDisableTiming));
        c->n_xev = 64;
    }
    for (int l = 1; l < IFCBK_MAX_LANES; ++l)
        if ((used >> l & 1) && !c->lane_st[l]) IFCBK_HIP(c, hipStreamCreateWithFlags(&c->lane_st[l], hipStreamNonBlocking));
    return IFCBK_OK;
}

static int lane_order(ifcbk_ctx* c, hipStream_t waiter, hipStream_t waited) {
    hipEvent_t ev;
    if (c->capturing) {
        if (c->cev_next >= c->n_cev) IFCBK_FAIL(c, IFCBK_EINVAL, "lane_order: capture event pool exhausted");
        ev = c->cev[c->cev_next++];
    } else {
        ev = c->xev[c->xev_next];
        c->xev_next = (c->xev_next + 1) & 63;
    }
    IFCBK_HIP(c, hipEventRecord(ev, waited));
    IFCBK_HIP(c, hipStreamWaitEvent(waiter, ev, 0));
    return IFCBK_OK;
}

static int run_lanes(ifcbk_ctx* c, const ifcbk_op* ops, int n, hipStream_t s0, hipEvent_t* ev, unsigned char* rec = nullptr) {
    hipStream_t st[IFCBK_MAX_LANES] = {s0};
    int used = 1;
    for (int i = 0; i < n; ++i) used |= 1 << op_lane(&ops[i]);
    if (used >> c->ws_lanes) IFCBK_FAIL(c, IFCBK_EINVAL, "run_program: an op names a lane beyond the %d this ctx has arenas for (ifcbk_ctx_set_lanes)", c->ws_lanes);
    if (int e = lane_resources(c, used)) return e;
    for (int l = 1; l < IFCBK_MAX_LANES; ++l)
        if (used >> l & 1) {
            st[l] = c->capturing ? c->cap_st[l] : c->lane_st[l];
            if (int e = lane_order(c, st[l], s0)) return e;
        }
    int rc = IFCBK_OK;
    for (int i = 0; i < n && !rc; ++i) {
        const int L = op_lane(&ops[i]);
        const int wm = op_wait(&ops[i]) & used & ~(1 << L);
        for (int j = 0; j < IFCBK_MAX_LANES && !rc; ++j)
            if (wm >> j & 1) {
                if (c->capturing && L != 0 && j != 0) {
                    rc = lane_order(c, st[0], st[j]);
                    if (!rc) rc = lane_order(c, st[L], st[0]);
                } else {
                    rc = lane_order(c, st[L], st[j]);
                }
            }
        if (rc) break;
        c->ws = (char*)c->ws_base + (size_t)L * c->ws_bytes;
        const bool timed = ev && (!rec || (ops[i].flags & 0x80));
        if (rec) rec[i] = timed;
        if (timed) IFCBK_HIP(c, hipEventRecord(ev[2 * i], st[L]));
        rc = run_one(c, &ops[i], st[L]);
        if (rc) {
            size_t len = strlen(c->err);
            snprintf(c->err + len, sizeof(c->err) - len, " [op %d kind %d]", i, ops[i].kind);
            break;
        }
        if (timed) IFCBK_HIP(c, hipEventRecord(ev[2 * i + 1], st[L]));
    }
    c->ws = c->ws_base;
    for (int l = 1; l < IFCBK_MAX_LANES; ++l)
        if (used >> l & 1) (void)lane_order(c, s0, st[l]);
    return rc;
}

extern "C" int ifcbk_run_program(ifcbk_ctx* c, const ifcbk_op* ops, int n, void* stream, float* op_ms) {
    if (!c || (!ops && n > 0)) return IFCBK_EINVAL;
    hipStream_t st = (hipStream_t)stream;
    if (op_ms) {
        if (c->n_ev < 2 * n) {
            hipEvent_t* ev = (hipEvent_t*)realloc(c->ev, sizeof(hipEvent_t) * (2 * n));
// ... 104 lines not shown
        (void)hipGraphExecDestroy(x);
        (void)hipGraphDestroy(g);
        IFCBK_FAIL(c, IFCBK_ENOMEM, "program_capture: out of host memory");
    }
    r->magic = GRAPH_MAGIC; r->owner = c;
    r->graph = g; r->exec = x; r->ws_epoch = c->ws_epoch; r->n_ops = n;
    r->next = c->graphs;
    if (c->graphs) c->graphs->prev = r;
    c->graphs = r;
    ++c->n_graphs;
    *out = r;
    return IFCBK_OK;
}

extern "C" int ifcbk_graph_launch(ifcbk_ctx* c, ifcbk_graph* g, void* stream) {
    if (!c || !g) return IFCBK_EINVAL;
    if (g->magic != GRAPH_MAGIC || g->owner != c) IFCBK_FAIL(c, IFCBK_EINVAL, "graph_launch: not a live graph of this ctx");
    if (g->ws_epoch != c->ws_epoch) IFCBK_FAIL(c, IFCBK_EINVAL, "graph_launch: the workspace moved since this graph was captured; capture it again");
    IFCBK_HIP(c, hipGraphLaunch(g->exec, (hipStream_t)stream));
    return IFCBK_OK;
}

extern "C" int ifcbk_graph_destroy(ifcbk_ctx* c, ifcbk_graph* g) {
    if (!g) return IFCBK_OK;
    if (!c) return IFCBK_EINVAL;
    if (g->magic != GRAPH_MAGIC || g->owner != c) IFCBK_FAIL(c, IFCBK_EINVAL, "graph_destroy: not a live graph of this ctx");
    graph_free(c, g);
    return IFCBK_OK;
}

extern "C" int ifcbk_op_kernel(const ifcbk_op* o, char* name, size_t cap) {
    if (!o || !name || cap < 1) return IFCBK_EINVAL;
    name[0] = 0;
    switch (o->kind) {
        case IFCBK_OP_CONV_FWD_AFFINE_SEG: {
            const ifcbk_conv_desc& d = o->u.conv;
            int bmt = 0, btn = 0;
            if (d.dtype == IFCBK_F32) { snprintf(name, cap, "conv_igemm<float, %d, 2, 2, 4>", ifcbk_conv_f32_nt(d.K)); break; }
            if (ifcbk_conv_big_plan(d.dtype, d.N * d.P * d.Q, d.K, d.R * d.S * d.C, &bmt, &btn))
                snprintf(name, cap, "conv_pp2<%d, %d, %d, 4>", btn, bmt, bmt == 10 ? 4 : bmt / 2);
            else
                snprintf(name, cap, "conv_igemm<unsigned short, %d, 2, 2, 4>", ifcbk_conv_fwd_nt(d.K, d.N * d.P * d.Q));
            break;
        }
        case IFCBK_OP_CONV_FWD: case IFCBK_OP_CONV_FWD_AFFINE: {
            const ifcbk_conv_desc& d = o->u.conv;
            int wm = ifcbk_conv_fwd_wm(d.N * d.P * d.Q, d.K);
            int bmt = 0, btn = 0;
            if (d.dtype == IFCBK_F32) { snprintf(name, cap, "conv_igemm<float, %d, 2, 2, 0>", ifcbk_conv_f32_nt(d.K)); break; }
            const bool rows = ifcbk_conv_rows_ok(d.dtype, d.C, d.K, d.R, d.S, d.stride_h, d.stride_w, d.pad_h, d.pad_w, d.Q) && !(o->kind == IFCBK_OP_CONV_FWD_AFFINE && o->p[5]);
            if (!rows && d.stride_h == 1 && d.stride_w == 1 && !(o->kind == IFCBK_OP_CONV_FWD_AFFINE && o->p[5]) &&
                ifcbk_conv_flat_rows(d.dtype, d.N, d.H, d.W, d.C, d.K, d.R, d.S, d.pad_h, d.pad_w, d.P, d.Q)) {
                snprintf(name, cap, "conv_flat<%d, %d, %d, %d, 0>", d.C, d.K, d.R, d.S);
                break;
            }
            if (!rows && d.stride_h == 1 && d.stride_w == 1) {
                if (const int smt = ifcbk_conv_slab_plan(d.dtype, d.N, d.H, d.W, d.C, d.K, d.R, d.S, d.pad_h, d.pad_w, d.P, d.Q)) {
                    snprintf(name, cap, "conv_slab<%d, %d, %d, %d, 50, 0>", d.K <= 128 ? 2 : 3, smt, smt == 10 ? 4 : smt / 2, d.R * d.S);
                    break;
                }
            }
            if (!rows && !(o->kind == IFCBK_OP_CONV_FWD_AFFINE && o->p[5]) &&
                ifcbk_conv_pp3_plan(d.dtype, d.N * d.P * d.Q, d.K, d.R * d.S * d.C, o->kind == IFCBK_OP_CONV_FWD_AFFINE ? 1 : 0)) {
                ifcbk_conv_pp3_name(d.R * d.S * d.C, o->kind == IFCBK_OP_CONV_FWD_AFFINE,
                                    d.R == 1 && d.S == 1 && d.pad_h == 0 && d.pad_w == 0 && d.stride_h == 1 && d.stride_w == 1, name, cap);
                break;
            }
            if (!rows && ifcbk_conv_big_plan(d.dtype, d.N * d.P * d.Q, d.K, d.R * d.S * d.C, &bmt, &btn)) {
                snprintf(name, cap, "conv_pp2<%d, %d, %d, 0>", btn, bmt, bmt == 10 ? 4 : bmt / 2);
                break;
            }
            if (ifcbk_conv_rows_ok(d.dtype, d.C, d.K, d.R, d.S, d.stride_h, d.stride_w, d.pad_h, d.pad_w, d.Q) && !(o->kind == IFCBK_OP_CONV_FWD_AFFINE && o->p[5]))
                snprintf(name, cap, "conv_rows3x3<%d, %d>", d.C, d.K);
            else if (!(o->kind == IFCBK_OP_CONV_FWD_AFFINE && o->p[5]) && ifcbk_conv_ws_shape(d.dtype, d.N * d.P * d.Q, d.K, d.R * d.S * d.C))
                snprintf(name, cap, "conv_ws<%d>", ifcbk_conv_fwd_nt(d.K, d.N * d.P * d.Q));
            else
            snprintf(name, cap, "conv_igemm<unsigned short, %d, %d, %d, 0>", ifcbk_conv_fwd_nt(d.K, d.N * d.P * d.Q), wm, wm == 4 ? 3 : 2);
            break;
        }
        case IFCBK_OP_CONV_DGRAD: case IFCBK_OP_CONV_DGRAD_BNSTAT: {
            const ifcbk_conv_desc& d = o->u.conv;
            int wm = ifcbk_conv_fwd_wm(d.N * d.H * d.W, d.C);
            {
                if (o->kind == IFCBK_OP_CONV_DGRAD && !(o->flags & 1) && ifcbk_conv_rows_ok(d.dtype, d.K, d.C, d.R, d.S, d.stride_h, d.stride_w, 2 - d.pad_h, 2 - d.pad_w, d.W)) {
                    snprintf(name, cap, "conv_rows3x3<%d, %d>", d.K, d.C);
                    break;
                }
                const bool s2 = d.stride_h == 2 || d.stride_w == 2;
                if (!s2 && !(o->kind == IFCBK_OP_CONV_DGRAD && (o->flags & 1)) &&
                    ifcbk_conv_flat_rows(d.dtype, d.N, d.P, d.Q, d.K, d.C, d.R, d.S, d.R - 1 - d.pad_h, d.S - 1 - d.pad_w, d.H, d.W)) {
                    snprintf(name, cap, "conv_flat<%d, %d, %d, %d, %d>", d.K, d.C, d.R, d.S, o->kind == IFCBK_OP_CONV_DGRAD_BNSTAT ? 3 : 0);
                    break;
                }
                if (!s2) {
                    if (const int smt = ifcbk_conv_slab_plan(d.dtype, d.N, d.P, d.Q, d.K, d.C, d.R, d.S, d.R - 1 - d.pad_h, d.S - 1 - d.pad_w, d.H, d.W)) {
                        snprintf(name, cap, "conv_slab<%d, %d, %d, %d, 50, %d>", d.C <= 128 ? 2 : 3, smt, smt == 10 ? 4 : smt / 2, d.R * d.S,
                                 o->kind == IFCBK_OP_CONV_DGRAD_BNSTAT ? 3 : 0);
                        break;
                    }
                }
                int bmt = 0, btn = 0;
                if (!s2 && o->kind == IFCBK_OP_CONV_DGRAD && !(o->flags & 1) && ifcbk_conv_pp3_plan(d.dtype, d.N * d.H * d.W, d.C, d.R * d.S * d.K, 0)) {
                    ifcbk_conv_pp3_name(d.R * d.S * d.K, false, d.R == 1 && d.S == 1 && d.pad_h == 0 && d.pad_w == 0, name, cap);
                    break;
                }
                if (!s2 && ifcbk_conv_big_plan(d.dtype, d.N * d.H * d.W, d.C, d.R * d.S * d.K, &bmt, &btn)) {
                    snprintf(name, cap, "conv_pp2<%d, %d, %d, %d>", btn, bmt, bmt == 10 ? 4 : bmt / 2, o->kind == IFCBK_OP_CONV_DGRAD_BNSTAT ? 3 : 0);
                    break;
                }
                if (o->kind == IFCBK_OP_CONV_DGRAD && !(o->flags & 1) && !s2 && ifcbk_conv_ws_shape(d.dtype, d.N * d.H * d.W, d.C, d.R * d.S * d.K)) {
                    snprintf(name, cap, "conv_ws<%d>", ifcbk_conv_fwd_nt(d.C, d.N * d.H * d.W));
                    break;
                }
                const bool classes = d.stride_h == 2 && d.stride_w == 2 && d.R >= 2 && d.S >= 2 && d.H >= 2 && d.W >= 2;
                if (d.dtype == IFCBK_F32) {
                    snprintf(name, cap, "conv_igemm<float, %d, 2, 2, %d>", ifcbk_conv_f32_nt(d.C),
                             o->kind == IFCBK_OP_CONV_DGRAD_BNSTAT ? 3 : classes ? 2 : (s2 ? 1 : 0));
                    break;
                }
                snprintf(name, cap, "conv_igemm<unsigned short, %d, %d, %d, %d>", ifcbk_conv_fwd_nt(d.C, classes ? d.N * ((d.H + 1) / 2) * ((d.W + 1) / 2) : d.N * d.H * d.W), wm, wm == 4 ? 3 : 2,
                         o->kind == IFCBK_OP_CONV_DGRAD_BNSTAT ? 3 : classes ? 2 : (s2 ? 1 : 0));
            }
            break;
        }
        case IFCBK_OP_CONV_WGRAD: case IFCBK_OP_CONV_WGRAD_SEG: {
            int mt = 0, cols = 0;
            ifcbk_conv_wgrad_shape(&o->u.conv, &mt, &cols);
            if (mt < 0) {
                snprintf(name, cap, "conv_wgrad_pp<%d, 0>", -mt);
            }
            else if (o->u.conv.dtype == IFCBK_F32) snprintf(name, cap, "conv_wgrad_f32<%d>", mt);
            else if (cols == 2) snprintf(name, cap, "conv_wgrad_flat");
            else if (mt == 0) snprintf(name, cap, "conv_wgrad_stem");
            else if (cols) snprintf(name, cap, "conv_wgrad_cols<%d, 4>", mt);
            else snprintf(name, cap, "conv_wgrad_rows<%d>", mt);
            break;
        }
        case IFCBK_OP_CONV_WGRAD_GROUP: {
            const ifcbk_wgrad_item* it = (const ifcbk_wgrad_item*)o->p[0];
            const int n = (int)o->i[0];
            ifcbk_conv_desc ds[8];
            int kh = 0;
            if (it && n >= 1 && n <= 8) {
                for (int k = 0; k < n; ++k) ds[k] = it[k].d;
                if (ifcbk_conv2d_wgrad_group_info(n, ds, &kh, nullptr, nullptr) == IFCBK_OK) {
                    if (kh == 16) snprintf(name, cap, "conv_wgrad_flatg");
                    else snprintf(name, cap, "conv_wgrad_ppg<%d>", kh);
                }
            }
            break;
        }
        case IFCBK_OP_CONV_FWD_AFFINE_MAXPOOL: snprintf(name, cap, "conv_rows3x3<%d, %d, true>", o->u.conv.C, o->u.conv.K); break;
        case IFCBK_OP_STEM_U8_FWD: snprintf(name, cap, "stem_u8_fwd_kernel"); break;
        case IFCBK_OP_STEM_U8_WGRAD: snprintf(name, cap, "stem_u8_wgrad_kernel"); break;
        case IFCBK_OP_BN_APPLY: snprintf(name, cap, "bn_apply_kernel"); break;
        case IFCBK_OP_BN_BWD: snprintf(name, cap, "bn_bwd"); break;
        case IFCBK_OP_BN_BWD_PARTIALS: snprintf(name, cap, "bn_bwd(partials)"); break;
        case IFCBK_OP_BN_APPLY_MAXPOOL: snprintf(name, cap, "bn_apply_maxpool_kernel"); break;
        case IFCBK_OP_BN_BWD_MAXPOOL: snprintf(name, cap, "bn_bwd(maxpool)"); break;
        case IFCBK_OP_BN_FINALIZE: snprintf(name, cap, "bn_finalize_kernel"); break;
        case IFCBK_OP_BN_STATS: snprintf(name, cap, "bn_stats_kernel"); break;
        case IFCBK_OP_MAXPOOL_FWD: snprintf(name, cap, "maxpool_fwd_kernel"); break;
        case IFCBK_OP_MAXPOOL_BWD: snprintf(name, cap, "maxpool_bwd_kernel"); break;
        case IFCBK_OP_AVGPOOL_FWD: case IFCBK_OP_AVGPOOL_AFFINE: snprintf(name, cap, "avgpool_fwd_kernel"); break;
        case IFCBK_OP_AVGPOOL_BWD: snprintf(name, cap, "avgpool_bwd_kernel"); break;
        case IFCBK_OP_ADAM: snprintf(name, cap, "adam_kernel"); break;
        case IFCBK_OP_SGD: snprintf(name, cap, "sgd_kernel"); break;
        case IFCBK_OP_BIAS_RELU_BWD: snprintf(name, cap, "bias_relu_bwd_kernel"); break;
        case IFCBK_OP_DROPOUT: snprintf(name, cap, "dropout_apply_kernel"); break;
        case IFCBK_OP_FLATTEN_CHW: snprintf(name, cap, "flatten_chw_kernel"); break;
        case IFCBK_OP_WEIGHT_PACK: snprintf(name, cap, "weight_pack_kernel"); break;
        case IFCBK_OP_WEIGHT_PACK_MULTI: snprintf(name, cap, "weight_pack_multi_kernel"); break;
        default: break;
    }
    return IFCBK_OK;
}

extern "C" int ifcbk_op_cost(const ifcbk_op* o, double* flops, double* bytes) {
    double fl = 0, by = 0;
    switch (o->kind) {
        case IFCBK_OP_CONV_FWD: case IFCBK_OP_CONV_FWD_AFFINE: case IFCBK_OP_CONV_FWD_AFFINE_SEG: case IFCBK_OP_CONV_DGRAD: case IFCBK_OP_CONV_WGRAD:
        case IFCBK_OP_CONV_WGRAD_SEG: case IFCBK_OP_CONV_DGRAD_BNSTAT: {
            const ifcbk_conv_desc& d = o->u.conv;
            double mac = (double)d.N * d.P * d.Q * d.K * d.R * d.S * d.Cw;
            fl = 2.0 * mac;
            double xin = (double)d.N * d.H * d.W * d.C * 2, yout = (double)d.N * d.P * d.Q * d.K * 2,
                   wb = (double)d.K * d.R * d.S * d.C * 2;
            by = xin + yout + wb + (o->kind == IFCBK_OP_CONV_DGRAD_BNSTAT ? xin : 0);
            break;
        }
        case IFCBK_OP_CONV_WGRAD_GROUP: {
            const ifcbk_wgrad_item* it = (const ifcbk_wgrad_item*)o->p[0];
            for (int k = 0; it && k < (int)o->i[0] && k < 8; ++k) {
                const ifcbk_conv_desc& d = it[k].d;
                fl += 2.0 * d.N * d.P * d.Q * d.K * d.R * d.S * d.Cw;
                by += (double)d.N * d.H * d.W * d.C * 2 + (double)d.N * d.P * d.Q * d.K * 2 + (double)d.K * d.R * d.S * d.C * 2;
            }
            break;
        }
        case IFCBK_OP_CONV_FWD_AFFINE_MAXPOOL: {
            const ifcbk_conv_desc& d = o->u.conv;
            fl = 2.0 * d.N * d.P * d.Q * d.K * d.R * d.S * d.Cw;
            by = (double)d.N * d.H * d.W * d.C * 2 + (double)d.N * ((d.P - 3) / 2 + 1) * ((d.Q - 3) / 2 + 1) * d.K * 2;
            break;
        }
        case IFCBK_OP_STEM_U8_FWD: case IFCBK_OP_STEM_U8_WGRAD: {
            const ifcbk_conv_desc& d = o->u.conv;
            fl = 2.0 * d.N * d.P * d.Q * d.K * d.R * d.S * d.Cw;
            by = (double)d.N * d.H * d.W + (double)d.N * d.P * d.Q * d.K * 2;
            break;
        }
        case IFCBK_OP_BN_APPLY: by = (double)o->u.bn.M * o->u.bn.C * (2 + 2 + (o->p[3] ? 2 : 0)); break;
        case IFCBK_OP_BN_STATS: by = (double)o->u.bn.M * o->u.bn.C * 2; break;
        case IFCBK_OP_BN_BWD: by = (double)o->u.bn.M * o->u.bn.C * (2.0 * (o->u.bn.relu ? 6 : 4) + 2 + (o->p[7] ? 2 : 0)); break;
        case IFCBK_OP_BN_BWD_PARTIALS: by = (double)o->u.bn.M * o->u.bn.C * (2 + 2 + 2); break;
        case IFCBK_OP_BN_APPLY_MAXPOOL: {
            const ifcbk_pool_desc& d = o->u.pool;
            by = ((double)d.N * d.H * d.W * 2 + (double)d.N * d.P * d.Q * 3) * d.C;
            break;
        }
        case IFCBK_OP_BN_BWD_MAXPOOL: {
            const ifcbk_pool_desc& d = o->u.pool;
            by = ((double)d.N * d.H * d.W * (2 * 2 + 2) + (double)d.N * d.P * d.Q * 3 * 2) * d.C;
            break;
        }
        case IFCBK_OP_MAXPOOL_FWD: case IFCBK_OP_AVGPOOL_FWD: case IFCBK_OP_MAXPOOL_BWD: case IFCBK_OP_AVGPOOL_BWD: case IFCBK_OP_AVGPOOL_AFFINE: {
            const ifcbk_pool_desc& d = o->u.pool;
            by = ((double)d.N * d.H * d.W + (double)d.N * d.P * d.Q) * d.C * 2;
            break;
        }
        case IFCBK_OP_HEAD_FWD: case IFCBK_OP_HEAD_BWD: {
            const ifcbk_head_desc& d = o->u.head;
            fl = 2.0 * d.N * d.C * d.NC * (o->kind == IFCBK_OP_HEAD_BWD ? 2 : 1);
            by = (double)d.N * d.HW * d.C * 2;
            break;
        }
        case IFCBK_OP_ADAM: by = (double)o->i[0] * 28; break;
        case IFCBK_OP_SGD: by = (double)o->i[0] * (o->p[2] ? 20 : 12); break;
        default: break;
    }
    if (flops) *flops = fl;
    if (bytes) *bytes = by;
    return 0;
}
```

ifcb_classifier_amd/engine.py:

```python
import ctypes as C
import math
import os

import torch

from . import _lib
from ._lib import Op, ConvDesc, BnDesc, PoolDesc, HeadDesc, RoiDesc


_DISPATCH_SWITCHES = ('IFCBK_CONV_PP3', 'IFCBK_CONV_PP3_GRID', 'IFCBK_WGRAD_LANE', 'IFCBK_WGRAD_GROUP', 'IFCBK_WGRAD_GROUP_MINKH', 'IFCBK_CONV_BIG', 'IFCBK_CONV_SLAB', 'IFCBK_CONV_BIG_MT', 'IFCBK_CONV_BIG_TN', 'IFCBK_CONV_FLAT', 'IFCBK_CONV_NT',
                      'IFCBK_CONV_WM', 'IFCBK_CONV_WS', 'IFCBK_CONV_WS_TILES', 'IFCBK_CONV_ROWS', 'IFCBK_WGRAD_PP',
                      'IFCBK_WGRAD_PP_KH', 'IFCBK_WGRAD_COLS', 'IFCBK_WGRAD_STEM', 'IFCBK_WGRAD_ROUNDS', 'IFCBK_WGRAD_FLAT',
                      'IFCBK_BN_BWD_ROWS')


def _dispatch_env():
    return tuple(os.environ.get(k) for k in _DISPATCH_SWITCHES)


def dtype_is_bf16(eng):
    return eng.dtype == 'bf16'


def _vp(t, byte_off=0):
# ... 323 lines not shown
        self.Wsh = torch.zeros(soff, dtype=self.tdtype, device=dev)
        self.stats = torch.zeros(stoff, dtype=torch.float32, device=dev)

    def init_weights(self, seed=None):
        g = torch.Generator(device='cpu')
        if seed is None:
            seed = int(torch.randint(0, 2 ** 31 - 1, (1,)).item())
        g.manual_seed(int(seed))
        incep = self.net.name == 'inception_v3'
        for key, (o, n, shape, kind, node) in self.poff.items():
            v = self.pviews[key]
            how = getattr(node, 'init', None)
            if kind in ('conv', 'lin_w') and how is not None:
                rf = shape[2] * shape[3] if len(shape) == 4 else 1
                fan_in, fan_out = shape[1] * rf, shape[0] * rf
                w = torch.empty(shape)
                if how == 'default':
                    w.uniform_(-1.0 / math.sqrt(fan_in), 1.0 / math.sqrt(fan_in), generator=g)
                elif how == 'kaiming_uniform':
                    w.uniform_(-math.sqrt(6.0 / fan_in), math.sqrt(6.0 / fan_in), generator=g)
                elif how == 'kaiming_out':
                    w.normal_(0, math.sqrt(2.0 / fan_out), generator=g)
                elif how == 'kaiming_in':
                    w.normal_(0, math.sqrt(2.0 / fan_in), generator=g)
                elif how == 'normal01':
                    w.normal_(0, 0.01, generator=g)
                else:
                    raise ValueError(how)
                v.copy_(w.to(self.dev))
            elif kind == 'cbias':
                wshape = self.poff[key[:-4] + 'weight'][2]
                fan_in = int(math.prod(wshape[1:]))
                if node.init == 'default':
                    v.copy_(((torch.rand(shape, generator=g) * 2 - 1) / math.sqrt(fan_in)).to(self.dev))
                else:
                    v.zero_()
            elif kind == 'bn_cbias':
                v.zero_()
            elif kind == 'conv':
                w = torch.empty(shape)
                if incep:
                    std = 0.01 if key.startswith('AuxLogits.conv1') else 0.1
                    torch.nn.init.trunc_normal_(w, 0.0, std, -2 * std, 2 * std, generator=g)
                else:
                    fan_out = shape[0] * shape[2] * shape[3]
                    w.normal_(0, math.sqrt(2.0 / fan_out), generator=g)
                v.copy_(w.to(self.dev))
            elif kind == 'bn_w':
                v.fill_(1.0)
            elif kind == 'bn_b':
                v.zero_()
            elif kind == 'fc_w':
                bound = 1.0 / math.sqrt(shape[1])
                v.copy_(((torch.rand(shape, generator=g) * 2 - 1) * bound).to(self.dev))
            elif kind == 'fc_b':
                fan_in = self.poff[key[:-4] + 'weight'][2][1]
                bound = 1.0 / math.sqrt(fan_in)
                v.copy_(((torch.rand(shape, generator=g) * 2 - 1) * bound).to(self.dev))
        self.params_changed()

    def params_changed(self):
        self.packed = False
        self.eval_stats_ready = False

    def _alloc_acts(self):
        net, dev, N = self.net, self.dev, self.max_batch
        Nt = self.train_batch
        bf = self.tdtype
        self.act = {}
        self.grad = {}
        grouped_raw = {m.raw.id: m for g in self.groups for m in g.members if m.cpool is None}
        for b in net.bufs:
            if b.id in grouped_raw:
                continue
            self.act[b.id] = torch.zeros(N, b.H, b.W, b.C, dtype=bf, device=dev)
        for g in self.groups:
            g.raw = torch.zeros(N, g.x.H, g.x.W, g.Ktot, dtype=bf, device=dev)
            for m in g.members:
                if m.cpool is None:
                    self.act[m.raw.id] = g.raw[..., m.koff:m.koff + m.K]
        need_grad = set()
        for n in net.nodes:
            if getattr(n, 'kind', '') == 'conv':
                need_grad.add(n.y.buf.id)
                if n.residual is not None:
                    need_grad.add(n.residual.buf.id)
            elif n.kind in ('max', 'avg', 'cb', 'drop', 'flat', 'bnr'):
                need_grad.add(n.y.buf.id)
        need_grad.discard(net.input.id)
        for bid in need_grad:
            b = net.bufs[bid]
            if b.name.endswith(':raw'):
                continue
            self.grad[bid] = torch.zeros(Nt, b.H, b.W, b.C, dtype=bf, device=dev)
        dp_world = self._dp_world_arg
        if dp_world is None:
            try:
                dp_world = int(os.environ.get('WORLD_SIZE', '0')) or None
            except ValueError:
                dp_world = None
        if dp_world is None:
            dp_world = 1
            try:
                import torch.distributed as _d
                if _d.is_available() and _d.is_initialized():
                    dp_world = _d.get_world_size()
            except Exception:
                dp_world = 1
        self.dp_world = max(1, int(dp_world))
        dp_world = self.dp_world
        self.NL = max(1, min(8, int(os.environ.get('IFCBK_LANES', '2' if dp_world > 1 else '4'))))
        self.NL_eval = max(1, min(self.NL, int(os.environ.get('IFCBK_LANES_EVAL', '2'))))
        gm = os.environ.get('IFCBK_GRAPH', 'eval')
        self.graph_eval = gm not in ('0', 'off', 'none')
        self.graph_train = gm in ('1', 'all', 'train')
        self.wgrad_lane = int(os.environ.get('IFCBK_WGRAD_LANE', '1' if self.NL >= 2 else '0'))
        if self.NL - self.wgrad_lane < 1:
            self.wgrad_lane = 0
        if not self.plan_only:
            self.ctx.call('ifcbk_ctx_set_lanes', self.NL)
        max_raw = max([n.P * n.Q * n.K for n in self.convs] + [8])
        self.draw = [torch.zeros(Nt * max_raw, dtype=bf, device=dev) for _ in range(self.NL)]
        gmax = max([g.x.H * g.x.W * g.Ktot for g in self.groups] + [0])
        self.draw_group = torch.zeros(max(1, Nt * gmax), dtype=bf, device=dev)
        mb = max([self.ctx.lib.ifcbk_conv2d_fwd_mblocks(C.byref(self._conv_desc(n, N))) * 2 * n.K for n in self.convs] +
                 [self.ctx.lib.ifcbk_conv2d_fwd_mblocks(C.byref(self._group_desc(g, N))) * 2 * g.Ktot for g in self.groups] +
                 [self.ctx.lib.ifcbk_bn_stats_rows(N * n.x.H * n.x.W) * 2 * n.K for n in self.bnrs] + [16])
        self.bn_part = [torch.zeros(mb, dtype=torch.float32, device=dev) for _ in range(self.NL)]
        self.argmax = {}
        for k, n in enumerate(net.nodes):
            if n.kind == 'max':
                self.argmax[k] = torch.zeros(Nt, n.P, n.Q, n.x.C, dtype=torch.uint8, device=dev)
        self.heads = [n for n in net.nodes if n.kind == 'head']
        for h in self.heads:
            h.feat = torch.zeros(N, h.C, dtype=torch.float32, device=dev)
            h.logits = torch.zeros(N, h.NC, dtype=torch.float32, device=dev)
            h.dlogits = torch.zeros(N, h.NC, dtype=torch.float32, device=dev)
            h.mask = torch.ones(N, h.C, dtype=torch.uint8, device=dev) if h.dropout else None
        self.drops = [n for n in net.nodes if n.kind == 'drop']
        for n in self.drops:
            n.mask = torch.ones(N, n.x.H * n.x.W * n.x.C, dtype=torch.uint8, device=dev)
        self.probs = torch.zeros(N, net.NC, dtype=torch.float32, device=dev)
        self.tgt_bufs = [torch.zeros(N, dtype=torch.int64, device=dev) for _ in range(2)]
        self.in_bufs = [self.act[net.input.id], torch.zeros_like(self.act[net.input.id])]
        self.in_slot = 0
        self.stem_u8 = None
        first = [n for n in self.convs if n.x.buf.is_input]
        if (os.environ.get('IFCBK_STEM_U8', '1') != '0' and len(first) == 1 and first[0].group is None
                and self.ctx.lib.ifcbk_stem_u8_rows(C.byref(self._conv_desc(first[0], N))) > 0):
            self.stem_u8 = first[0]
            self.in_u8 = [torch.zeros(N, net.S, net.S, dtype=torch.uint8, device=dev) for _ in range(2)]
            self.in_ab = [torch.zeros(6, dtype=torch.float32, device=dev) for _ in range(2)]
            self._in_ab_host = [None, None]
        self.in_kind = ['nhwc', 'nhwc']
        self.pre_stream = self.pre_ctx = None
        self.ev_ready, self.ev_free, self.prefetched = [None, None], [None, None], None
        self.loss = torch.zeros(1, dtype=torch.float32, device=dev)
        self.loss_sum = torch.zeros(1, dtype=torch.float32, device=dev)
        self.class_weight = None if self._class_weights_arg is None else torch.tensor(self._class_weights_arg, dtype=torch.float32, device=dev)
        ws = 1 << 20
        for n in self.convs:
            d = self._conv_desc(n, Nt)
            ws = max(ws, self.ctx.lib.ifcbk_conv2d_wgrad_workspace(C.byref(d)))
            M = Nt * n.P * n.Q
            ws = max(ws, (((M + 255) // 256) * 2 * n.K + 2 * n.K) * 4)
        for g in self.groups:
            ws = max(ws, self.ctx.lib.ifcbk_conv2d_wgrad_workspace(C.byref(self._group_desc(g, Nt))))
        for n in self.plains:
            ws = max(ws, self.ctx.lib.ifcbk_conv2d_wgrad_workspace(C.byref(self._conv_desc(n, Nt))),
                     self.ctx.lib.ifcbk_bias_relu_bwd_workspace(Nt * n.P * n.Q, n.K))
        for n in self.bnrs:
            M = Nt * n.x.H * n.x.W
            ws = max(ws, (((M + 255) // 256) * 2 * n.K + 2 * n.K) * 4)
        if self.stem_u8 is not None:
            ws = max(ws, self.ctx.lib.ifcbk_stem_u8_wgrad_workspace(C.byref(self._conv_desc(self.stem_u8, Nt))))
        self.ctx.reserve(ws)

    @property
    def target(self):
        return self.tgt_bufs[self.in_slot]

    def _select_slot(self, slot):
        self.in_slot = slot
        self.act[self.net.input.id] = self.in_bufs[slot]

    def prefetch_stream(self):
        if self.plan_only:
            raise RuntimeError('prefetch: this engine was built with plan_only=True')
        if self.pre_stream is None:
            self.pre_stream = torch.cuda.Stream(self.dev)
            self.pre_ctx = _lib.Context(self.dev.index)
        return self.pre_stream

    def prefetch_begin(self):
        self.prefetch_stream()
        slot = 1 - self.in_slot
        if self.ev_free[slot] is not None:
            self.pre_stream.wait_event(self.ev_free[slot])
        return slot, self.pre_stream

    def prefetch_end(self, slot):
        ev = torch.cuda.Event()
        ev.record(self.pre_stream)
        self.ev_ready[slot] = ev
        self.prefetched = slot

    def use_prefetched(self):
        slot = self.prefetched
        if slot is None:
            raise RuntimeError('use_prefetched: nothing was prefetched')
        cur = torch.cuda.current_stream(self.dev)
        ev = torch.cuda.Event()
        ev.record(cur)
        self.ev_free[self.in_slot] = ev
        cur.wait_event(self.ev_ready[slot])
        self._select_slot(slot)
        self.prefetched = None
        return slot

    def activation_bytes(self):
        tot = sum(t.numel() * t.element_size() for t in self.act.values())
        tot += sum(t.numel() * t.element_size() for t in self.grad.values())
        return tot + sum(t.numel() for t in self.draw) * self.esize

    def _conv_desc(self, n, N):
        if (n.R * n.S > 1 and n.R == n.x.H and n.S == n.x.W and n.ph == 0 and n.pw == 0 and n.P == 1 and n.Q == 1
                and n.x.is_full and n.Cw == n.x.C):
            CC = n.R * n.S * n.x.C
            return ConvDesc(N, 1, 1, CC, CC, n.K, 1, 1, 1, 1, 0, 0, 1, 1, n.y.buf.C, CC, self.cdtype)
        return ConvDesc(N, n.x.H, n.x.W, n.x.C, n.x.buf.C, n.K, n.R, n.S, n.sh, n.sw, n.ph, n.pw, n.P, n.Q,
                        n.y.buf.C, n.Cw, self.cdtype)

    def zeros_k(self, K):
        z = getattr(self, '_zeros_k', None)
        if z is None or z.numel() < K:
            z = self._zeros_k = torch.zeros(max(K, 4096), dtype=torch.float32, device=self.dev)
        return z

    def _pack_desc(self, n, d):
        if n.K_real == n.K:
            return d
        dp = ConvDesc.from_buffer_copy(d)
        dp.K = n.K_real
        return dp

    def _group_desc(self, g, N):
        x = g.x
        return ConvDesc(N, x.H, x.W, x.C, x.buf.C, g.Ktot, 1, 1, 1, 1, 0, 0, x.H, x.W, g.Ktot, x.C, self.cdtype)

    def _aptr(self, view, grad=False):
        t = (self.grad if grad else self.act)[view.buf.id]
        return _vp(t, self.esize * view.coff)

    def _pptr(self, key, which='P'):
        o = self.poff[key][0]
        return _vp(getattr(self, which), 4 * o)

    def _stat(self, n, k):
        return _vp(self.stats, 4 * (n.st_off + k * n.st_ld))

    def _raw_ptr(self, n):
        if n.group is not None and n.cpool is None:
            return _vp(n.group.raw, self.esize * n.koff), n.group.Ktot
        return _vp(self.act[n.raw.id]), n.K

    def _pre_ptr(self, n):
        return _vp(n.group.raw, self.esize * n.koff), n.group.Ktot

    def plan(self, N):
        if N > self.max_batch:
            raise RuntimeError('batch %d exceeds the engine capacity %d' % (N, self.max_batch))
        key = (N, self.in_slot, self.in_kind[self.in_slot])
        if key not in self._plans:
            self._plans[key] = self._build(N)
            self._plans[key].dispatch_env = _dispatch_env()
        pl = self._plans[key]
        if pl.dispatch_env != _dispatch_env():
            raise RuntimeError('a kernel-dispatch switch (%s) changed after the plan for batch %d was built: build a new model/engine '
                               'instead' % (', '.join(k for k, v in zip(_DISPATCH_SWITCHES, pl.dispatch_env) if os.environ.get(k) != v), N))
        return pl

    def _build(self, N):
        net = self.net
        fwd_t, fwd_e, bwd = OpList(), OpList(), OpList()
        pack, evalprep = OpList(), OpList()
        written = set()

        def acc_flag(buf):
            a = 1 if buf.id in written else 0
            written.add(buf.id)
            return a

        readers = {}
        for m in net.nodes:
            for v in ((m.x, getattr(m, 'residual', None)) if m.kind == 'conv' else (m.x,)):
                if v is not None:
                    readers.setdefault(v.buf.id, []).append(m)
        pool_cand = {}
        for kk, m in enumerate(net.nodes):
            if (m.kind == 'max' and m.R == 3 and m.S == 3 and m.sh == 2 and m.sw == 2 and m.ph <= 1 and m.pw <= 1
                    and m.x.is_full and len(readers.get(m.x.buf.id, ())) == 1):
                prod = [c for c in net.nodes if c.kind == 'conv' and c.y.buf.id == m.x.buf.id]
                if (len(prod) == 1 and prod[0].y.is_full and prod[0].relu and prod[0].residual is None
                        and prod[0].group is None and bool(prod[0].aux) == bool(m.aux)):
                    pool_cand[prod[0]] = (m, kk)
        fused_pool = dict(pool_cand) if os.environ.get('IFCBK_FUSE_POOL', '1') != '0' else {}
        fused_pool_nodes = {v[0] for v in fused_pool.values()}
        self.fused_pool = fused_pool
        fused_pool_eval = {}
        if os.environ.get('IFCBK_FUSE_POOL_EVAL', '1') != '0' and not self.plan_only:
            for cn, (pn, pk) in pool_cand.items():
                if (pn.ph == 0 and pn.pw == 0 and cn.y.buf.C == cn.K
                        and self.ctx.lib.ifcbk_conv2d_fwd_affine_maxpool_ok(C.byref(self._conv_desc(cn, N)))):
                    fused_pool_eval[cn] = pn
        fused_pool_eval_nodes = set(fused_pool_eval.values())
        bnstat_of = {}
        fuse_bnstat = os.environ.get('IFCBK_FUSE_BNSTAT', '1')
        if fuse_bnstat not in ('0', '1'):
            raise ValueError('IFCBK_FUSE_BNSTAT must be 0 or 1, got %r' % fuse_bnstat)
        keep = []
        if fuse_bnstat == '1':
            for cnode in net.nodes:
                if cnode.kind != 'conv' or cnode.group is not None or cnode.x.buf.is_input or not cnode.x.is_full:
                    continue
                if len(readers.get(cnode.x.buf.id, ())) != 1:
                    continue
                prod = [c for c in net.nodes if c.kind == 'conv' and c.y.buf.id == cnode.x.buf.id]
                if (len(prod) == 1 and prod[0].y.is_full and prod[0].relu and prod[0].residual is None
                        and prod[0] not in fused_pool and bool(prod[0].aux) == bool(cnode.aux)
                        and self._conv_desc(cnode, N).C == cnode.x.C
                        and self.ctx.lib.ifcbk_conv2d_dgrad_bnstat_mblocks(C.byref(self._conv_desc(cnode, N))) > 0):
                    bnstat_of[cnode] = prod[0]
        bnstat_done = {}

        NL = self.NL
        producers = {}
        for m in net.nodes:
            if m.kind != 'head':
                producers.setdefault(m.y.buf.id, []).append(m)


        def follows_of():
            f = {}
            for m in net.nodes:
                if m.aux or m.kind == 'head':
                    continue
                prods = producers.get(m.x.buf.id, [])
                if (len(prods) == 1 and prods[0].y.is_full and m.x.is_full and len(readers.get(m.x.buf.id, ())) == 1
                        and not prods[0].aux):
                    f[m] = prods[0]
            return f

        def assign_lanes(nl):
            follows = follows_of()
            head_of = {}
            for m in net.nodes:
                if m.aux or m.kind == 'head':
                    continue
                head_of[m] = head_of[follows[m]] if m in follows and follows[m] in head_of else m
            by_tensor = {}
            for m in net.nodes:
                if not m.aux and m.kind != 'head' and head_of.get(m) is m:
                    by_tensor.setdefault(m.x.buf.id, []).append(m)
            rank = {}
            for heads in by_tensor.values():
                for k, h in enumerate(heads):
                    rank[h] = k
            lanes = {}
            for m in net.nodes:
                if m.aux:
                    lanes[m] = 1 % nl
                elif m.kind == 'head':
                    lanes[m] = 0
                else:
                    lanes[m] = rank[head_of[m]] % nl
            return lanes

        WLs = list(range(NL - self.wgrad_lane, NL))
        wl_next = [0]
        lane_of = assign_lanes(NL - self.wgrad_lane)
        lane_eval = assign_lanes(self.NL_eval)
        if not hasattr(self, 'draw_own'):
            self.draw_own = {}

        def _carve(nelem):
            if not self.wgrad_lane:
                return torch.empty(nelem, dtype=self.tdtype, device=self.dev)
            if getattr(self, '_draw_pool', None) is None:
                tot = 0
                for m in self.convs:
                    if m.group is None or m.cpool is not None:
                        tot += (self.train_batch * m.P * m.Q * m.K + 127) // 128 * 128
                for gq in self.groups:
                    tot += (self.train_batch * gq.x.H * gq.x.W * gq.Ktot + 127) // 128 * 128
                self._draw_pool = torch.empty(max(tot, 128), dtype=self.tdtype, device=self.dev)
                self._draw_used = 0
            n = (nelem + 127) // 128 * 128
            if self._draw_used + n > self._draw_pool.numel():
                return torch.empty(nelem, dtype=self.tdtype, device=self.dev)
            v = self._draw_pool[self._draw_used:self._draw_used + nelem]
            self._draw_used += n
            return v

        def own_draw(m):
            if m not in self.draw_own:
                self.draw_own[m] = _carve(self.train_batch * m.P * m.Q * m.K)
            return self.draw_own[m]

        def group_draw(gq):
            if not self.wgrad_lane:
                return self.draw_group
            if getattr(gq, 'draw_own', None) is None:
                gq.draw_own = _carve(self.train_batch * gq.x.H * gq.x.W * gq.Ktot)
            return gq.draw_own

        def ra(v):
            return ('a', v.buf.id, v.coff, v.coff + v.C)

        def rg(v):
            return ('g', v.buf.id, v.coff, v.coff + v.C)

        def rraw(m):
            if m.group is not None and m.cpool is None:
                return ('gr', id(m.group), m.koff, m.koff + m.K)
            return ('r', m.raw.id, 0, m.K)

        absorbed = self.absorbed_pools

        def rdg(m):
            return ('dg', id(m.group), m.koff, m.koff + m.K)

        rst = lambda m: ('s', id(m), 0, 1)
        rbp = lambda L: ('bp', L, 0, 1)
        ram = lambda kk: ('am', kk, 0, 1)

        bwd_groups = []
        for k, n in enumerate(net.nodes):
            grp = OpList()
            L = lane_of[n]
            if n.kind == 'conv':
                M = N * n.P * n.Q
                d = self._conv_desc(n, N)
                raw, ldraw = self._raw_ptr(n)
                dfw = ConvDesc.from_buffer_copy(d)
                dfw.ldy = ldraw
                wk = _vp(self.Wsh, self.esize * n.w_off)
                wT = _vp(self.Wsh, self.esize * n.wT_off)
                ckey, bkey = n.conv_key + '.weight', n.bn_key
                mb = self.ctx.lib.ifcbk_conv2d_fwd_mblocks(C.byref(d))
                u8 = self.stem_u8 is n and self.in_kind[self.in_slot] == 'u8'
                if u8:
                    mb = self.ctx.lib.ifcbk_stem_u8_rows(C.byref(d))
                    gu8, gab = _vp(self.in_u8[self.in_slot]), _vp(self.in_ab[self.in_slot])
                bnd = BnDesc(M, n.K, ldraw, n.y.buf.C, 1 if n.relu else 0, self.cdtype, n.eps, 0.1)
                g = n.group
                first_of_group = g is not None and g.members[0] is n
                res = self._aptr(n.residual) if n.residual is not None else None
                ldr = n.residual.buf.C if n.residual is not None else 0
                for lst, train in ((fwd_t, True), (fwd_e, False)):
                    if n.aux and not train:
                        continue
                    Le = lane_eval[n]
                    if not train and g is not None and self.eval_groups:
                        if first_of_group:
                            gd = self._group_desc(g, N)
                            ys, iv, wr = [], [], []
                            for m in g.members:
                                if m.cpool is not None:
                                    pre, ldpre = self._pre_ptr(m)
                                    ys.append(pre); iv.append(m.K | (ldpre << 20)); wr.append(('gr', id(g), m.koff, m.koff + m.K))
                                else:
                                    ys.append(self._aptr(m.y)); iv.append(m.K | (m.y.buf.C << 20) | (1 << 40)); wr.append(ra(m.y))
                            ys += [None] * (4 - len(ys))
                            iv += [0] * (4 - len(iv))
                            lst.add(_lib.OP_CONV_FWD_AFFINE_SEG, '+'.join(m.name for m in g.members),
                                    p=(self._aptr(g.x), _vp(self.Wsh, self.esize * g.w_off), ys[0], ys[1], ys[2], ys[3],
                                       self._stat(g.members[0], 4), self._stat(g.members[0], 5)),
                                    i=iv, conv=gd, lane=Le, reads=[ra(g.x)], writes=wr)
                        if n.cpool is not None:
                            cp = n.cpool
                            pre, ldpre = self._pre_ptr(n)
                            ppd = PoolDesc(N, cp.x.H, cp.x.W, n.K, ldpre, 3, 3, 1, 1, 1, 1, cp.P, cp.Q, n.y.buf.C, self.cdtype)
                            lst.add(_lib.OP_AVGPOOL_AFFINE, cp.name + '(' + n.name + ')',
                                    p=(pre, self._stat(n, 4), self._stat(n, 5), self._aptr(n.y)), flags=4 if n.relu else 0, pool=ppd,
                                    lane=Le, reads=[('gr', id(g), n.koff, n.koff + n.K)], writes=[ra(n.y)])
                        continue
                    if not train and n.cpool is not None:
                        cp = n.cpool
                        pre, ldpre = self._pre_ptr(n)
                        dpre = ConvDesc(N, cp.x.H, cp.x.W, cp.x.C, cp.x.buf.C, n.K, 1, 1, 1, 1, 0, 0, n.P, n.Q, ldpre, n.Cw, self.cdtype)
                        rpre = ('gr', id(g), n.koff, n.koff + n.K)
                        lst.add(_lib.OP_CONV_FWD, n.name, p=(self._aptr(cp.x), wk, pre, None), conv=dpre, lane=Le,
                                reads=[ra(cp.x)], writes=[rpre])
                        ppd = PoolDesc(N, cp.x.H, cp.x.W, n.K, ldpre, 3, 3, 1, 1, 1, 1, cp.P, cp.Q, n.y.buf.C, self.cdtype)
                        lst.add(_lib.OP_AVGPOOL_AFFINE, cp.name + '(' + n.name + ')',
                                p=(pre, self._stat(n, 4), self._stat(n, 5), self._aptr(n.y)), flags=4 if n.relu else 0, pool=ppd,
                                lane=Le, reads=[rpre], writes=[ra(n.y)])
                        continue
                    if not train and u8:
                        lst.add(_lib.OP_STEM_U8_FWD, n.name,
                                p=(gu8, self._pptr(ckey), gab, self._aptr(n.y), None, self._stat(n, 4), self._stat(n, 5)),
                                flags=4 if n.relu else 0, conv=d, lane=Le, reads=[ra(n.x)], writes=[ra(n.y)])
                        continue
                    if not train and n in fused_pool_eval:
                        pn = fused_pool_eval[n]
                        lst.add(_lib.OP_CONV_FWD_AFFINE_MAXPOOL, n.name + '+' + pn.name,
                                p=(self._aptr(n.x), wk, self._aptr(pn.y), self._stat(n, 4), self._stat(n, 5)),
                                i=(pn.y.buf.C,), flags=4 if n.relu else 0, conv=d, lane=Le, reads=[ra(n.x)], writes=[ra(pn.y)])
                        continue
                    if not train:
                        lst.add(_lib.OP_CONV_FWD_AFFINE, n.name,
                                p=(self._aptr(n.x), wk, self._aptr(n.y), self._stat(n, 4), self._stat(n, 5), res),
                                i=(ldr,), flags=4 if n.relu else 0, conv=d, lane=Le,
                                reads=[ra(n.x)] + ([ra(n.residual)] if n.residual is not None else []), writes=[ra(n.y)])
                        continue
                    if g is not None:
                        if not first_of_group:
                            continue
                        gd = self._group_desc(g, N)
                        gmb = self.ctx.lib.ifcbk_conv2d_fwd_mblocks(C.byref(gd))
                        lst.add(_lib.OP_CONV_FWD, '+'.join(m.name for m in g.members),
                                p=(self._aptr(g.x), _vp(self.Wsh, self.esize * g.w_off), _vp(g.raw), _vp(self.bn_part[0])),
                                conv=gd, lane=0, reads=[ra(g.x)], writes=[('gr', id(g), 0, g.Ktot), rbp(0)])
                        for m in g.members:
                            mbk = m.bn_key
                            mraw, mld = self._raw_ptr(m)
                            mbnd = BnDesc(M, m.K, mld, m.y.buf.C, 1, self.cdtype, m.eps, 0.1)
                            if m.cpool is not None:
                                Lm, pn = lane_of[m], m.cpool
                                pre, ldpre = self._pre_ptr(m)
                                ppd = PoolDesc(N, pn.x.H, pn.x.W, m.K, ldpre, 3, 3, 1, 1, 1, 1, pn.P, pn.Q, mld, self.cdtype)
                                rpre, rr2 = ('gr', id(g), m.koff, m.koff + m.K), ('r', m.raw.id, 0, m.K)
                                lst.add(_lib.OP_AVGPOOL_FWD, pn.name + '(' + m.name + ')', p=(pre, mraw), pool=ppd, lane=Lm,
                                        reads=[rpre], writes=[rr2])
                                lst.add(_lib.OP_BN_STATS, m.name, p=(mraw, _vp(self.bn_part[Lm])), bn=mbnd, lane=Lm,
                                        reads=[rr2], writes=[rbp(Lm)])
                                lst.add(_lib.OP_BN_FINALIZE, m.name,
                                        p=(_vp(self.bn_part[Lm]), self._pptr(mbk + '.weight'), self._pptr(mbk + '.bias'),
                                           _vp(self.bviews[mbk + '.running_mean']), _vp(self.bviews[mbk + '.running_var']),
                                           self._stat(m, 0), self._stat(m, 1), self._stat(m, 2), self._stat(m, 3)),
                                        i=(self.ctx.lib.ifcbk_bn_stats_rows(M), m.K), bn=mbnd, lane=Lm, reads=[rbp(Lm)], writes=[rst(m)])
                                lst.add(_lib.OP_BN_APPLY, m.name,
                                        p=(mraw, self._stat(m, 2), self._stat(m, 3), None, self._aptr(m.y)), i=(0,), bn=mbnd,
# ... 82 lines not shown
                        lst.add(_lib.OP_CONV_FWD_AFFINE, n.name,
                                p=(self._aptr(n.x), wk, self._aptr(n.y), _vp(self.ones),
                                   self._pptr(n.key + '.bias') if n.bias else _vp(self.zeros_k(n.K)), None),
                                i=(0,), flags=4 if n.relu else 0, conv=d, lane=Lx, reads=[ra(n.x)], writes=[ra(n.y)])
                    else:
                        lst.add(_lib.OP_CONV_FWD, n.name, p=(self._aptr(n.x), wk, self._aptr(n.y), None), conv=d, lane=Lx,
                                reads=[ra(n.x)], writes=[ra(n.y)])
                needs_dgrad = not n.x.buf.is_input
                pack.add(_lib.OP_WEIGHT_PACK, n.name, p=(self._pptr(n.key + '.weight'), wk, wT if needs_dgrad else None),
                         i=(n.K if n.K != n.K_real else 0,), conv=self._pack_desc(n, d))
                bwd_groups.append(('cb', n, d, wT, needs_dgrad))
            elif n.kind == 'drop':
                cnt = N * n.x.H * n.x.W * n.x.C
                for lst, train in ((fwd_t, True), (fwd_e, False)):
                    lst.add(_lib.OP_DROPOUT, n.name, p=(self._aptr(n.x), _vp(n.mask) if train else None, self._aptr(n.y)),
                            i=(cnt, self.cdtype), f=(1.0 / (1.0 - n.p),), lane=L if train else lane_eval[n],
                            reads=[ra(n.x), ('dm', id(n), 0, 1)], writes=[ra(n.y)])
                bwd_groups.append(('drop', n, cnt))
            elif n.kind == 'flat':
                fi = (N, n.x.H * n.x.W, n.x.C, n.x.buf.C | (self.cdtype << 32))
                for lst, train in ((fwd_t, True), (fwd_e, False)):
                    lst.add(_lib.OP_FLATTEN_CHW, n.name, p=(self._aptr(n.x), self._aptr(n.y)), i=fi, flags=4,
                            lane=L if train else lane_eval[n], reads=[ra(n.x)], writes=[ra(n.y)])
                bwd_groups.append(('flat', n, fi))
            elif n.kind == 'bnr':
                M = N * n.x.H * n.x.W
                bkey = n.bn_key
                bnd = BnDesc(M, n.K, n.x.buf.C, n.K, 1 if n.relu else 0, self.cdtype, n.eps, 0.1)
                xp = self._aptr(n.x)
                fwd_t.add(_lib.OP_BN_STATS, n.name, p=(xp, _vp(self.bn_part[L])), bn=bnd, lane=L, reads=[ra(n.x)], writes=[rbp(L)])
                fwd_t.add(_lib.OP_BN_FINALIZE, n.name,
                          p=(_vp(self.bn_part[L]), self._pptr(bkey + '.weight'), self._pptr(bkey + '.bias'),
                             _vp(self.bviews[bkey + '.running_mean']), _vp(self.bviews[bkey + '.running_var']),
                             self._stat(n, 0), self._stat(n, 1), self._stat(n, 2), self._stat(n, 3)),
                          i=(self.ctx.lib.ifcbk_bn_stats_rows(M), n.K), bn=bnd, lane=L, reads=[rbp(L)], writes=[rst(n)])
                for lst, train in ((fwd_t, True), (fwd_e, False)):
                    lst.add(_lib.OP_BN_APPLY, n.name,
                            p=(xp, self._stat(n, 2 if train else 4), self._stat(n, 3 if train else 5), None, self._aptr(n.y)),
                            i=(0,), bn=bnd, lane=L if train else lane_eval[n], reads=[ra(n.x), rst(n)], writes=[ra(n.y)])
                evalprep.add(_lib.OP_BN_FINALIZE, n.name,
                             p=(None, self._pptr(bkey + '.weight'), self._pptr(bkey + '.bias'),
                                _vp(self.bviews[bkey + '.running_mean']), _vp(self.bviews[bkey + '.running_var']),
                                None, None, self._stat(n, 4), self._stat(n, 5)), i=(0,), bn=bnd)
                bwd_groups.append(('bnr', n, bnd))

        wg_of, wg_groups = {}, []
        if os.environ.get('IFCBK_WGRAD_GROUP', '1') != '0' and self.dtype == 'bf16':
            buckets = {}
            for gsp in reversed(bwd_groups):
                if gsp[0] != 'conv':
                    continue
                n = gsp[1]
                if n.group is not None or n.aux or (self.stem_u8 is n and self.in_kind[self.in_slot] == 'u8'):
                    continue
                dbw = ConvDesc.from_buffer_copy(gsp[2])
                dbw.ldy = n.K
                khv = self.ctx.lib.ifcbk_conv2d_wgrad_group_member_kh(C.byref(dbw))
                if khv <= 0:
                    continue
                key = n.name.split('.')[0] if net.name == 'inception_v3' else n.name.rsplit('.', 1)[0]
                buckets.setdefault((key, khv), []).append((n, dbw))
            for (key, khv), mem in buckets.items():
                for c0 in range(0, len(mem), 6):
                    part = mem[c0:c0 + 6]
                    if len(part) < 2:
                        continue
                    descs = (ConvDesc * len(part))(*[m[1] for m in part])
                    need = self.ctx.lib.ifcbk_conv2d_wgrad_group_workspace(len(part), descs)
                    if need == 0:
                        continue
                    grp_obj = dict(members=[m[0] for m in part], descs=[m[1] for m in part], ws=need, kh=khv, key=key)
                    wg_groups.append(grp_obj)
                    for m in part:
                        wg_of[m[0]] = grp_obj
            if wg_groups:
                need = max(gq['ws'] for gq in wg_groups)
                if not self.plan_only and need > self.ctx.lib.ifcbk_ctx_workspace_bytes(self.ctx.h):
                    self.ctx.reserve(need)
                for gq in wg_groups:
                    for m in gq['members']:
                        own_draw(m)
        self.wgrad_groups = wg_groups

        for g in reversed(bwd_groups):
            if g[0] == 'head':
                _, n, hd = g
                wkey, bkey = n.key + '.weight', n.key + '.bias'
                assert n.x.is_full
                acc = acc_flag(n.x.buf)
                assert acc == 0, 'head must be the first writer of its input gradient'
                bwd.add(_lib.OP_HEAD_BWD, n.name,
                        p=(_vp(n.dlogits), _vp(n.feat), _vp(n.mask) if n.dropout else None, self._pptr(wkey) if n.fc else None,
                           self._pptr(wkey, 'G') if n.fc else None, self._pptr(bkey, 'G') if n.fc else None, self._aptr(n.x, True)),
                        i=(n.x.buf.C,), head=hd, lane=lane_of[n], reads=[('hd', id(n), 0, 1)], writes=[rg(n.x)])
            elif g[0] == 'cb':
                _, n, d, wT, needs_dgrad = g
                L = lane_of[n]
                M = N * n.P * n.Q
                dy, ldy = self._aptr(n.y, True), n.y.buf.C
                if n.relu or n.bias:
                    bnd = BnDesc(M, n.K, ldy, ldy, 1 if n.relu else 0, self.cdtype, 0.0, 0.0)
                    bwd.add(_lib.OP_BIAS_RELU_BWD, n.name,
                            p=(self._aptr(n.y), dy, dy if n.relu else None, self._pptr(n.key + '.bias', 'G') if n.bias else None),
                            i=(ldy,), bn=bnd, lane=L, reads=[ra(n.y), rg(n.y)], writes=[rg(n.y)])
                bwd.add(_lib.OP_CONV_WGRAD, n.name, p=(self._aptr(n.x), dy, self._pptr(n.key + '.weight', 'G')), conv=d, lane=L,
                        reads=[ra(n.x), rg(n.y)], writes=[])
                if needs_dgrad:
                    assert n.x.is_full
                    acc = acc_flag(n.x.buf)
                    bwd.add(_lib.OP_CONV_DGRAD, n.name, p=(dy, wT, self._aptr(n.x, True)), flags=acc, conv=d, lane=L,
                            reads=[rg(n.y)], writes=[rg(n.x)])
            elif g[0] == 'drop':
                _, n, cnt = g
                acc = acc_flag(n.x.buf)
                bwd.add(_lib.OP_DROPOUT, n.name, p=(self._aptr(n.y, True), _vp(n.mask), self._aptr(n.x, True)), i=(cnt, self.cdtype),
                        f=(1.0 / (1.0 - n.p),), flags=acc, lane=lane_of[n], reads=[rg(n.y), ('dm', id(n), 0, 1)], writes=[rg(n.x)])
            elif g[0] == 'flat':
                _, n, fi = g
                assert n.x.is_full
                acc = acc_flag(n.x.buf)
                bwd.add(_lib.OP_FLATTEN_CHW, n.name, p=(self._aptr(n.x, True), self._aptr(n.y, True)), i=fi, flags=acc,
                        lane=lane_of[n], reads=[rg(n.y)], writes=[rg(n.x)])
            elif g[0] == 'bnr':
                _, n, bnd = g
                bkey = n.bn_key
                first = n.x.buf.id not in written
                if first:
                    assert n.x.is_full, 'the first gradient written into a concatenation must cover all of it: ' + n.name
                acc = acc_flag(n.x.buf)
                bwd.add(_lib.OP_BN_BWD, n.name,
                        p=(self._aptr(n.x), self._aptr(n.y), self._aptr(n.y, True), self._pptr(bkey + '.weight'),
                           self._stat(n, 0), self._stat(n, 1), self._aptr(n.x, True), None, self._pptr(bkey + '.weight', 'G'),
                           self._pptr(bkey + '.bias', 'G'), self._stat(n, 2), self._stat(n, 3)),
                        i=(n.K, n.x.buf.C, 0), flags=8 if acc else 0, bn=bnd, lane=lane_of[n],
                        reads=[ra(n.x), ra(n.y), rg(n.y), rst(n)], writes=[rg(n.x)])
            elif g[0] == 'pool':
                _, n, pd, k = g
                assert n.x.is_full
                if n in fused_pool_nodes:
                    continue
                if n in absorbed:
                    continue
                acc = acc_flag(n.x.buf)
                if n.kind == 'max':
                    bwd.add(_lib.OP_MAXPOOL_BWD, n.name, p=(self._aptr(n.y, True), _vp(self.argmax[k]), self._aptr(n.x, True)), flags=acc, pool=pd,
                            lane=lane_of[n], reads=[rg(n.y), ram(k)], writes=[rg(n.x)])
                else:
                    bwd.add(_lib.OP_AVGPOOL_BWD, n.name, p=(self._aptr(n.y, True), self._aptr(n.x, True)), flags=acc, pool=pd,
                            lane=lane_of[n], reads=[rg(n.y)], writes=[rg(n.x)])
            else:
                _, n, d, bnd, draw, wT, needs_dgrad = g
                wgq = wg_of.get(n)
                own = wgq is not None or (self.wgrad_lane and (n.group is None or n.cpool is not None))
                if own:
                    draw = _vp(own_draw(n))
                elif self.wgrad_lane:
                    draw = _vp(group_draw(n.group), self.esize * n.koff)
                LW = None
                if self.wgrad_lane:
                    LW = WLs[wl_next[0] % len(WLs)]
                    wl_next[0] += 1
                ckey, bkey = n.conv_key + '.weight', n.bn_key
                dres, lddres, dres_acc = None, 0, 0
                if n.residual is not None:
                    assert n.residual.is_full
                    dres_acc = acc_flag(n.residual.buf)
                    dres, lddres = self._aptr(n.residual, True), n.residual.buf.C
                grp = n.group
                L = lane_of[n]
                cp = n.cpool is not None
                rdraw = [rdg(n)] if (grp is not None and not cp) else [('draw', L, 0, 1)]
                if own:
                    rdraw = [('drawn', id(n), 0, 1)]
                rawp, _ld = self._raw_ptr(n)
                if n in fused_pool:
                    pn, pk = fused_pool[n]
                    ppd = PoolDesc(N, pn.x.H, pn.x.W, pn.x.C, _ld, 3, 3, 2, 2, pn.ph, pn.pw, pn.P, pn.Q, pn.y.buf.C, self.cdtype)
                    bwd.add(_lib.OP_BN_BWD_MAXPOOL, n.name + '+' + pn.name,
                            p=(rawp, self._aptr(pn.y, True), _vp(self.argmax[pk]), self._pptr(bkey + '.weight'),
                               self._stat(n, 0), self._stat(n, 1), self._stat(n, 2), self._stat(n, 3), draw,
                               self._pptr(bkey + '.weight', 'G'), self._pptr(bkey + '.bias', 'G')),
                            i=(1, n.K), pool=ppd, lane=L, reads=[rraw(n), rg(pn.y), ram(pk), rst(n)], writes=rdraw)
                elif n in bnstat_done:
                    ppart, nrow, pres = bnstat_done[n]
                    bwd.add(_lib.OP_BN_BWD_PARTIALS, n.name,
                            p=(rawp, self._aptr(n.y, True), self._pptr(bkey + '.weight'), self._stat(n, 0), self._stat(n, 1),
                               self._stat(n, 2), self._stat(n, 3), ppart, draw, self._pptr(bkey + '.weight', 'G'),
                               self._pptr(bkey + '.bias', 'G')),
                            i=(n.y.buf.C, nrow, n.K if (grp is None or cp) else grp.Ktot, 0), bn=bnd, lane=L,
                            reads=[rraw(n), rg(n.y), rst(n), pres], writes=rdraw)
                else:
                    bwd.add(_lib.OP_BN_BWD, n.name,
                            p=(rawp, self._aptr(n.y), self._aptr(n.y, True), self._pptr(bkey + '.weight'),
                               self._stat(n, 0), self._stat(n, 1), draw, dres, self._pptr(bkey + '.weight', 'G'),
                               self._pptr(bkey + '.bias', 'G'), self._stat(n, 2), self._stat(n, 3)),
                            i=(n.y.buf.C, n.K if (grp is None or cp) else grp.Ktot, lddres), flags=dres_acc, bn=bnd, lane=L,
                            reads=[rraw(n), ra(n.y), rg(n.y), rst(n)],
                            writes=rdraw + ([rg(n.residual)] if n.residual is not None else []))
                if cp:
                    pn = n.cpool
                    ppd = PoolDesc(N, pn.x.H, pn.x.W, n.K, grp.Ktot, 3, 3, 1, 1, 1, 1, pn.P, pn.Q, n.K, self.cdtype)
                    bwd.add(_lib.OP_AVGPOOL_BWD, pn.name + '(' + n.name + ')',
                            p=(draw, _vp(group_draw(grp), self.esize * n.koff)), flags=0, pool=ppd, lane=L,
                            reads=rdraw, writes=[rdg(n)])
                if grp is not None:
                    if grp.members[0] is n:
                        gd = self._group_desc(grp, N)
                        gdraw = group_draw(grp)
                        gp = [_vp(gdraw)] + [self._pptr(m.conv_key + '.weight', 'G') for m in grp.members]
                        gres = ('dg', id(grp), 0, grp.Ktot)
                        bwd.add(_lib.OP_CONV_WGRAD_SEG, '+'.join(m.name for m in grp.members),
                                p=[self._aptr(grp.x), gp[0]] + gp[1:], i=[m.K for m in grp.members], conv=gd,
                                lane=0 if LW is None else LW, reads=[ra(grp.x), gres], writes=[])
                        acc = acc_flag(grp.x.buf)
                        bwd.add(_lib.OP_CONV_DGRAD, '+'.join(m.name for m in grp.members),
                                p=(_vp(gdraw), _vp(self.Wsh, self.esize * grp.wT_off), self._aptr(grp.x, True)),
                                flags=acc, conv=gd, lane=0, reads=[gres], writes=[rg(grp.x)])
                    continue
                dbw = ConvDesc.from_buffer_copy(d)
                dbw.ldy = n.K
                if wgq is not None:
                    wgq.setdefault('seen', []).append(n)
                    if len(wgq['seen']) == len(wgq['members']):
                        mem = wgq['members']
                        items = (_lib.WgradItem * len(mem))()
                        for kq, (m, dq) in enumerate(zip(mem, wgq['descs'])):
                            items[kq].d = dq
                            items[kq].x = self._aptr(m.x).value
                            items[kq].dy = self.draw_own[m].data_ptr()
                            items[kq].dw = self._pptr(m.conv_key + '.weight', 'G').value
                        keep.append(items)
                        bwd.add(_lib.OP_CONV_WGRAD_GROUP, '+'.join(m.name for m in mem),
                                p=[C.addressof(items)] + [items[kq].dw for kq in range(len(mem))], i=(len(mem),), lane=L if LW is None else LW,
                                reads=[ra(m.x) for m in mem] + [('drawn', id(m), 0, 1) for m in mem], writes=[])
                elif self.stem_u8 is n and self.in_kind[self.in_slot] == 'u8':
                    bwd.add(_lib.OP_STEM_U8_WGRAD, n.name,
                            p=(_vp(self.in_u8[self.in_slot]), draw, _vp(self.in_ab[self.in_slot]), self._pptr(ckey, 'G')), conv=dbw,
                            lane=L if LW is None else LW, reads=[ra(n.x)] + rdraw, writes=[])
                else:
                    bwd.add(_lib.OP_CONV_WGRAD, n.name, p=(self._aptr(n.x), draw, self._pptr(ckey, 'G')), conv=dbw,
                            lane=L if LW is None else LW,
                            reads=[ra(n.x)] + rdraw, writes=[])
                if needs_dgrad:
                    assert n.x.is_full
                    acc = acc_flag(n.x.buf)
                    if n in bnstat_of and acc == 0:
                        pn = bnstat_of[n]
                        prow, pld = self._raw_ptr(pn)
                        nrow = self.ctx.lib.ifcbk_conv2d_dgrad_bnstat_mblocks(C.byref(dbw))
                        bwd.add(_lib.OP_CONV_DGRAD_BNSTAT, n.name,
                                p=(draw, wT, self._aptr(n.x, True), prow, self._stat(pn, 0), self._stat(pn, 1),
                                   self._stat(pn, 2), self._stat(pn, 3), _vp(self.bn_part[L])), i=(pld,), conv=dbw,
                                lane=L, reads=rdraw + [rraw(pn), rst(pn)], writes=[rg(n.x), rbp(L)])
                        bnstat_done[pn] = (_vp(self.bn_part[L]), nrow, rbp(L))
                    else:
                        bwd.add(_lib.OP_CONV_DGRAD, n.name, p=(draw, wT, self._aptr(n.x, True)), flags=acc, conv=dbw,
                                lane=L, reads=rdraw, writes=[rg(n.x)])

        class PlanObj:
            pass
        pl = PlanObj()
        pl.N = N
        pl.fwd_train, pl.fwd_eval, pl.bwd = Program(fwd_t), Program(fwd_e), Program(bwd)
        pack_ops = pack
        pack = self._pack_multi(pack)
        pl.pack, pl.evalprep = Program(pack), Program(evalprep)
        lossl = OpList()
        main = [h for h in self.heads if not h.aux][0]
        auxh = [h for h in self.heads if h.aux]
        xent, cw = (_lib.OP_SOFTMAX_XENT, ()) if self.class_weight is None else (_lib.OP_SOFTMAX_XENT_W, (_vp(self.class_weight),))
        lossl.add(xent, 'loss', p=(_vp(main.logits), _vp(self.target), _vp(self.loss), _vp(main.dlogits)) + cw,
                  i=(N, net.NC), f=(1.0,))
        for h in auxh:
            lossl.add(xent, 'loss_aux', p=(_vp(h.logits), _vp(self.target), _vp(self.loss), _vp(h.dlogits)) + cw,
                      i=(N, net.NC), f=(0.4,), flags=1)
        pl.loss = Program(lossl)
        evl = OpList()
        evl.add(xent, 'val_loss', p=(_vp(main.logits), _vp(self.target), _vp(self.loss), None) + cw, i=(N, net.NC), f=(1.0,))
        pl.eval_loss = Program(evl)
        sm = OpList()
        sm.add(_lib.OP_SOFTMAX, 'softmax', p=(_vp(main.logits), _vp(self.probs)), i=(N, net.NC))
        pl.softmax = Program(sm)
        opt = OpList()
        if self.optimizer == 'sgd':
            opt.add(_lib.OP_SGD, 'sgd', p=(_vp(self.P), _vp(self.G), _vp(self.M) if self.momentum else None),
                    i=(self.nparam_padded, 1), f=(self.lr, self.momentum, self.weight_decay, 1.0))
        else:
            opt.add(_lib.OP_ADAM, 'adam', p=(_vp(self.P), _vp(self.G), _vp(self.M), _vp(self.V)),
                    i=(self.nparam_padded, 1), f=(self.lr, self.betas[0], self.betas[1], self.eps, self.weight_decay, 1.0))
        pl.adam = Program(opt)
        cnt = OpList()
        cnt.add(_lib.OP_STEP_COUNTERS, 'step_counters', p=(_vp(self.nbt), _vp(self.loss_sum), _vp(self.loss)), i=(self.nbt.numel(),))
        allops = OpList()
        for prog_ops in (fwd_t, lossl) + self._bucketed_update(bwd, opt, pack_ops) + (cnt,):
            allops.extend(prog_ops)
        pl.step = Program(allops)
        pl.step_adam_idxs = pl.step.find(_lib.OP_SGD if self.optimizer == 'sgd' else _lib.OP_ADAM)
        pl.step_adam_idx = pl.step_adam_idxs[-1]
        fl = OpList()
        fl.extend(fwd_t)
        fl.extend(lossl)
        pl.fwd_loss = Program(fl)
        fb = OpList()
        for prog_ops in (fwd_t, lossl, bwd):
            fb.extend(prog_ops)
        pl.fwd_bwd = Program(fb)
        pl.graphs = {}
        ap = OpList()
        ap.extend(opt)
        ap.extend(pack)
        ap.extend(cnt)
        pl.adam_pack = Program(ap)
        pl.bwd_list = bwd
        pl.ddp_segs = None
        pl.keep = keep
        return pl

    def _bucketed_update(self, bwd, opt, pack_ops):
        nb = int(os.environ.get('IFCBK_OPT_BUCKETS', '6'))
        whole = (bwd, opt, self._pack_multi(pack_ops))
        if nb <= 1:
            return whole
        from .dp import segment_plan
        offs = [self._op_param_offsets(o) for o in bwd.ops]
        try:
            segs = segment_plan(offs, self.palloc, self.nparam_padded, nb)
        except RuntimeError:
            return whole
        if len(segs) < 2:
            return whole
        pbase, sbase = self.P.data_ptr(), self.Wsh.data_ptr()
        regions = [(g.wT_off, g.wT_off + g.Ktot * g.x.C) for g in self.groups]

        def skey(elem_off):
            for (r0, r1) in regions:
                if r0 <= elem_off < r1:
                    return r0
            return elem_off
        owners = {}
        for o in pack_ops.ops:
            if o.p[2]:
                owners.setdefault(skey((o.p[2] - sbase) // self.esize), []).append((o.p[0] - pbase) // 4)
        dkinds = (_lib.OP_CONV_DGRAD, _lib.OP_CONV_DGRAD_BNSTAT)
        last_reader = {}
        shreads = {}
        for k, o in enumerate(bwd.ops):
            if o.kind in dkinds:
                own = owners.get(skey((o.p[1] - sbase) // self.esize))
                if own is None:
                    return whole
                shreads[k] = [('SH', off, off + self.palloc[off]) for off in own]
                for off in own:
                    last_reader[off] = k
        LW = self.NL - 1 if self.wgrad_lane else 0
        inserts = {}
        prev_ins = 0
        for (b0, b1, lo, hi) in segs[:-1]:
            ins = max([b1, prev_ins] + [1 + k for off, k in last_reader.items() if lo <= off < hi])
            prev_ins = ins
            ol = inserts.setdefault(ins, OpList())
            o0 = opt.ops[0]
            ptrs = [(o0.p[j] + 4 * lo) if o0.p[j] else None for j in range(4 if self.optimizer != 'sgd' else 3)]
            ol.add(o0.kind, opt.tags[0] + '[%d:%d]' % (lo, hi), p=ptrs, i=(hi - lo, int(o0.i[1])), f=tuple(o0.f[j] for j in range(8)),
                   lane=LW, reads=[('G', lo, hi)], writes=[('P', lo, hi)])
            sub = OpList()
            for o, tg, mt in zip(pack_ops.ops, pack_ops.tags, pack_ops.meta):
                if lo <= (o.p[0] - pbase) // 4 < hi:
                    sub.ops.append(o); sub.tags.append(tg); sub.meta.append(mt)
            if sub.ops:
                pm = self._pack_multi(sub, key=(lo, hi))
                pm.meta[0] = (LW, [('P', lo, hi)], [('SH', lo, hi)])
                ol.extend(pm)
        out = OpList()
        for k, (o, tg, mt) in enumerate(zip(bwd.ops, bwd.tags, bwd.meta)):
            if k in inserts:
                out.extend(inserts[k])
            lane, reads, writes = mt
            if not (reads is None and writes is None):
                extra_w = [('G', off, off + self.palloc[off]) for off in offs[k]]
                mt = (lane, list(reads or ()) + shreads.get(k, []), list(writes or ()) + extra_w)
            out.ops.append(o); out.tags.append(tg); out.meta.append(mt)
        for k in sorted(inserts):
            if k >= len(bwd.ops):
                out.extend(inserts[k])
        lo, hi = segs[-1][2], segs[-1][3]
        last_opt, last_pack = OpList(), OpList()
        o0 = opt.ops[0]
# ... 278 lines not shown
```

include/ifcbk.h:

```cpp
#ifndef IFCBK_H
#define IFCBK_H
#include <stdint.h>
#include <stddef.h>

#ifdef __cplusplus
extern "C" {
#endif

#define IFCBK_API __attribute__((visibility("default")))

#define IFCBK_OK          0
#define IFCBK_EINVAL     -1
#define IFCBK_EHIP       -2
#define IFCBK_ENOMEM     -3
#define IFCBK_EUNSUPPORTED -4

#define IFCBK_BF16 0
#define IFCBK_F32  1

typedef struct ifcbk_ctx ifcbk_ctx;

IFCBK_API const char* ifcbk_version(void);
IFCBK_API int  ifcbk_ctx_create(int device, ifcbk_ctx** out);
IFCBK_API int  ifcbk_ctx_destroy(ifcbk_ctx* ctx);
IFCBK_API int  ifcbk_ctx_reserve(ifcbk_ctx* ctx, size_t bytes);
IFCBK_API size_t ifcbk_ctx_workspace_bytes(ifcbk_ctx* ctx);
IFCBK_API int  ifcbk_ctx_set_lanes(ifcbk_ctx* ctx, int lanes);
IFCBK_API int  ifcbk_ctx_live_graphs(ifcbk_ctx* ctx);
IFCBK_API const char* ifcbk_last_error(ifcbk_ctx* ctx);

typedef struct {
    int32_t N, H, W, C;
    int32_t ldx;
    int32_t K;
    int32_t R, S;
    int32_t stride_h, stride_w, pad_h, pad_w;
    int32_t P, Q;
    int32_t ldy;
    int32_t Cw;
    int32_t dtype;
} ifcbk_conv_desc;

IFCBK_API int ifcbk_conv2d_fwd(ifcbk_ctx*, const ifcbk_conv_desc*, const void* x, const void* w, void* y,
                     float* bn_part, void* stream);
IFCBK_API int ifcbk_conv2d_fwd_affine(ifcbk_ctx*, const ifcbk_conv_desc*, const void* x, const void* w, void* y,
                            const float* scale, const float* shift, const void* residual, int ldr, int relu,
                            void* stream);
IFCBK_API int ifcbk_conv2d_fwd_affine_maxpool_ok(const ifcbk_conv_desc*);
IFCBK_API int ifcbk_conv2d_fwd_affine_maxpool(ifcbk_ctx*, const ifcbk_conv_desc*, const void* x, const void* w, void* y_pooled, int ldp,
                                    const float* scale, const float* shift, int relu, void* stream);
IFCBK_API int ifcbk_conv2d_fwd_affine_segments(ifcbk_ctx*, const ifcbk_conv_desc* d, const void* x, const void* w, int nseg,
                                     void* const* ys, const int32_t* ldys, const int32_t* ksegs, const int32_t* affine,
                                     const float* scale, const float* shift, void* stream);
IFCBK_API int ifcbk_conv2d_dgrad(ifcbk_ctx*, const ifcbk_conv_desc*, const void* dy, const void* wT, void* dx,
                       int accumulate, void* stream);
IFCBK_API int ifcbk_conv2d_wgrad(ifcbk_ctx*, const ifcbk_conv_desc*, const void* x, const void* dy, float* dw,
                       int accumulate, void* stream);
IFCBK_API int ifcbk_conv2d_wgrad_segments(ifcbk_ctx*, const ifcbk_conv_desc*, const void* x, const void* dy, int nseg,
                                float* const* dws, const int32_t* kseg, int accumulate, void* stream);
IFCBK_API size_t ifcbk_conv2d_wgrad_workspace(const ifcbk_conv_desc*);
IFCBK_API int ifcbk_conv2d_wgrad_group(ifcbk_ctx*, int n, const ifcbk_conv_desc* descs, const void* const* xs, const void* const* dys,
                             float* const* dws, int accumulate, void* stream);
IFCBK_API size_t ifcbk_conv2d_wgrad_group_workspace(int n, const ifcbk_conv_desc* descs);
IFCBK_API int ifcbk_conv2d_wgrad_group_info(int n, const ifcbk_conv_desc* descs, int* kh, int* blocks, int* nsplit);
IFCBK_API int ifcbk_conv2d_wgrad_group_member_kh(const ifcbk_conv_desc*);
IFCBK_API int  ifcbk_conv2d_fwd_mblocks(const ifcbk_conv_desc*);
IFCBK_API int ifcbk_weight_pack(ifcbk_ctx*, const ifcbk_conv_desc*, const float* w_master, void* w, void* wT,
                      void* stream);

typedef struct {
    const float* w_master;
    void*   w;
    void*   wT;
    int32_t K, RS, C, Cw;
    int64_t first_block;
    int32_t wT_ld;
    int32_t pad_;
} ifcbk_pack_item;
IFCBK_API int ifcbk_weight_pack_multi(ifcbk_ctx*, const ifcbk_pack_item* items_dev, int n_items, int64_t total_blocks, int dtype,
                            void* stream);

typedef struct {
    int32_t M;
    int32_t C;
    int32_t ldx, ldy;
    int32_t relu;
    int32_t dtype;
    float   eps, momentum;
} ifcbk_bn_desc;

IFCBK_API int ifcbk_bn_finalize_ld(ifcbk_ctx*, const ifcbk_bn_desc*, const float* part, int mblocks, int part_ld,
                         const float* gamma, const float* beta, float* running_mean, float* running_var,
                         float* mean, float* invstd, float* scale, float* shift, void* stream);
IFCBK_API int ifcbk_bn_finalize(ifcbk_ctx*, const ifcbk_bn_desc*, const float* part, int mblocks,
                      const float* gamma, const float* beta, float* running_mean, float* running_var,
                      float* mean, float* invstd, float* scale, float* shift, void* stream);
IFCBK_API int ifcbk_bn_apply(ifcbk_ctx*, const ifcbk_bn_desc*, const void* x, const float* scale,
                   const float* shift, const void* residual, int ldr, void* y, void* stream);
IFCBK_API int ifcbk_bn_bwd(ifcbk_ctx*, const ifcbk_bn_desc*, const void* x, const void* y, const void* dy, int lddy,
                 const float* gamma, const float* mean, const float* invstd,
                 void* dx, int lddx, void* dres, int lddres, int dres_accumulate,
                 float* dgamma, float* dbeta, int param_accumulate,
                 const float* scale, const float* shift , void* stream);

typedef struct {
    int32_t N, H, W, C, ldx;
    int32_t R, S, stride_h, stride_w, pad_h, pad_w;
    int32_t P, Q, ldy;
    int32_t dtype;
} ifcbk_pool_desc;
IFCBK_API int ifcbk_maxpool_fwd(ifcbk_ctx*, const ifcbk_pool_desc*, const void* x, void* y, uint8_t* argmax, void* stream);
IFCBK_API int ifcbk_maxpool_bwd(ifcbk_ctx*, const ifcbk_pool_desc*, const void* dy, const uint8_t* argmax, void* dx,
                      int accumulate, void* stream);
IFCBK_API int ifcbk_avgpool_fwd(ifcbk_ctx*, const ifcbk_pool_desc*, const void* x, void* y, void* stream);
IFCBK_API int ifcbk_avgpool_bwd(ifcbk_ctx*, const ifcbk_pool_desc*, const void* dy, void* dx, int accumulate, void* stream);

typedef struct {
    int32_t N, HW, C, ldx;
    int32_t NC;
    int32_t dtype;
    float   keep_scale;
} ifcbk_head_desc;
IFCBK_API int ifcbk_head_fwd(ifcbk_ctx*, const ifcbk_head_desc*, const void* x, const uint8_t* mask,
                   const float* W, const float* b, float* feat, float* logits, void* stream);
IFCBK_API int ifcbk_head_bwd(ifcbk_ctx*, const ifcbk_head_desc*, const float* dlogits, const float* feat,
                   const uint8_t* mask, const float* W, float* dW, float* db, void* dx, int lddx,
                   int param_accumulate, void* stream);
IFCBK_API int ifcbk_dropout_mask(ifcbk_ctx*, uint8_t* mask, int64_t n, float p, uint64_t seed, uint64_t offset, void* stream);

IFCBK_API int ifcbk_softmax_xent(ifcbk_ctx*, const float* logits, const int64_t* target, int N, int NC, float weight,
                       float* loss_out, int loss_accumulate, float* dlogits, void* stream);
IFCBK_API int ifcbk_softmax(ifcbk_ctx*, const float* logits, int N, int NC, float* probs, void* stream);
IFCBK_API int ifcbk_softmax_xent_w(ifcbk_ctx*, const float* logits, const int64_t* target, const float* class_weight, int N, int NC,
                         float weight, float* loss_out, int loss_accumulate, float* dlogits , void* stream);
IFCBK_API int ifcbk_step_counters(ifcbk_ctx*, int64_t* num_batches_tracked, int n, float* loss_sum, const float* loss, void* stream);

IFCBK_API int ifcbk_adam_flat(ifcbk_ctx*, float* p, const float* g, float* m, float* v, int64_t n, float lr,
                    float beta1, float beta2, float eps, float weight_decay, int step, float grad_scale,
                    void* stream);
IFCBK_API int ifcbk_sgd_flat(ifcbk_ctx*, float* p, const float* g, float* mom, int64_t n, float lr, float momentum,
                   float weight_decay, float grad_scale, void* stream);

typedef struct {
    int32_t n_img;
    int32_t S;
    int32_t in_channels;
    int32_t out_channels;
    int32_t flip_bits_valid;
    int32_t dtype;
    float   mean[3], std[3];
    float   tin_scale[3], tin_shift[3];
} ifcbk_roi_desc;
IFCBK_API int ifcbk_roi_preprocess(ifcbk_ctx*, const ifcbk_roi_desc*, const uint8_t* pixels, const int64_t* offs,
                         const int32_t* hs, const int32_t* ws, const uint8_t* flips, int max_h, int max_w,
                         void* out, uint8_t* out_u8 , void* stream);
IFCBK_API size_t ifcbk_roi_preprocess_workspace(const ifcbk_roi_desc*, int max_h, int max_w);
IFCBK_API int ifcbk_u8_channel_moments(ifcbk_ctx*, const uint8_t* x, int n_img, int64_t pixels_per_img,
                                        int channels, uint64_t* out, void* stream);
IFCBK_API int ifcbk_stem_u8_rows(const ifcbk_conv_desc*);
IFCBK_API int ifcbk_stem_u8_fwd(ifcbk_ctx*, const ifcbk_conv_desc* d, const uint8_t* g, const float* w_master, const float* ab, void* y,
                      float* bn_part, const float* scale, const float* shift, int relu, void* stream);
IFCBK_API size_t ifcbk_stem_u8_wgrad_workspace(const ifcbk_conv_desc*);
IFCBK_API int ifcbk_stem_u8_wgrad(ifcbk_ctx*, const ifcbk_conv_desc* d, const uint8_t* g, const void* dy, const float* ab, float* dw,
                        int accumulate, void* stream);
IFCBK_API int ifcbk_nchw_to_nhwc(ifcbk_ctx*, const float* x, int N, int C, int H, int W, int Cpad, int dtype,
                       const float* scale3, const float* shift3, void* y, void* stream);
IFCBK_API int ifcbk_nhwc_to_nchw_f32(ifcbk_ctx*, const void* x, int N, int C, int H, int W, int ldx, int dtype,
                           float* y, void* stream);

IFCBK_API int ifcbk_bn_apply_maxpool(ifcbk_ctx*, const ifcbk_pool_desc* d, const void* x, const float* scale,
                           const float* shift, int relu, void* y, uint8_t* argmax, void* stream);
IFCBK_API int ifcbk_avgpool3x3_affine(ifcbk_ctx*, const ifcbk_pool_desc* d, const void* x, const float* scale, const float* shift,
                            int relu, void* y, void* stream);
IFCBK_API int ifcbk_bn_stats_rows(int64_t M);
IFCBK_API int ifcbk_bn_stats(ifcbk_ctx*, const ifcbk_bn_desc* d, const void* x, float* part, void* stream);

IFCBK_API int ifcbk_bn_bwd_maxpool(ifcbk_ctx*, const ifcbk_pool_desc* d, const void* x, const void* dpool,
                         const uint8_t* argmax, const float* gamma, const float* mean, const float* invstd,
                         const float* scale, const float* shift, int relu, void* dx, int lddx, float* dgamma,
                         float* dbeta, int param_accumulate, void* stream);

IFCBK_API int ifcbk_conv2d_dgrad_bnstat_mblocks(const ifcbk_conv_desc*);
IFCBK_API int ifcbk_conv2d_dgrad_bnstat(ifcbk_ctx*, const ifcbk_conv_desc*, const void* dy, const void* wT, void* dx,
                              const void* prev_raw, int prev_ld, const float* prev_mean, const float* prev_invstd,
                              const float* prev_scale, const float* prev_shift, float* part, void* stream);
IFCBK_API int ifcbk_bn_bwd_partials(ifcbk_ctx*, const ifcbk_bn_desc*, const void* x, const void* dy, int lddy,
                          const float* gamma, const float* mean, const float* invstd, const float* scale,
                          const float* shift, const float* part, int ntiles, void* dx, int lddx, float* dgamma,
                          float* dbeta, int param_accumulate, void* stream);
IFCBK_API int ifcbk_bn_bwd_partials_ld(ifcbk_ctx*, const ifcbk_bn_desc*, const void* x, const void* dy, int lddy,
                             const float* gamma, const float* mean, const float* invstd, const float* scale,
                             const float* shift, const float* part, int ntiles, int part_ld, void* dx, int lddx,
                             float* dgamma, float* dbeta, int param_accumulate, void* stream);

IFCBK_API int ifcbk_bias_relu_bwd(ifcbk_ctx*, int64_t M, int K, int dtype, const void* y, int ldy, const void* dy, int lddy, void* dz,
                        int lddz, int relu, float* dbias, int param_accumulate, void* stream);
IFCBK_API size_t ifcbk_bias_relu_bwd_workspace(int64_t M, int K);
IFCBK_API int ifcbk_bias_relu_bwd_rows(int64_t M);
IFCBK_API int ifcbk_dropout_apply(ifcbk_ctx*, int64_t n, int dtype, const void* x, const uint8_t* mask, float scale, void* y, int accumulate,
                        void* stream);
IFCBK_API int ifcbk_flatten_chw(ifcbk_ctx*, int N, int HW, int C, int dtype, void* x, int ldx, void* flat, int to_chw, int accumulate,
                      void* stream);

enum {
    IFCBK_OP_CONV_FWD = 1, IFCBK_OP_CONV_DGRAD, IFCBK_OP_CONV_WGRAD, IFCBK_OP_WEIGHT_PACK,
    IFCBK_OP_BN_FINALIZE, IFCBK_OP_BN_APPLY, IFCBK_OP_BN_BWD,
    IFCBK_OP_MAXPOOL_FWD, IFCBK_OP_MAXPOOL_BWD, IFCBK_OP_AVGPOOL_FWD, IFCBK_OP_AVGPOOL_BWD,
    IFCBK_OP_HEAD_FWD, IFCBK_OP_HEAD_BWD, IFCBK_OP_SOFTMAX_XENT, IFCBK_OP_SOFTMAX,
    IFCBK_OP_ADAM, IFCBK_OP_MEMSET, IFCBK_OP_COPY2D, IFCBK_OP_DROPOUT_MASK, IFCBK_OP_CONV_FWD_AFFINE,
    IFCBK_OP_WEIGHT_PACK_MULTI, IFCBK_OP_CONV_WGRAD_SEG, IFCBK_OP_BN_APPLY_MAXPOOL, IFCBK_OP_BN_BWD_MAXPOOL,
    IFCBK_OP_CONV_DGRAD_BNSTAT, IFCBK_OP_BN_BWD_PARTIALS, IFCBK_OP_BN_STATS, IFCBK_OP_AVGPOOL_AFFINE,
    IFCBK_OP_CONV_FWD_AFFINE_SEG,
    IFCBK_OP_SGD,
    IFCBK_OP_RETIRED_31,
    IFCBK_OP_BIAS_RELU_BWD,
    IFCBK_OP_DROPOUT,
    IFCBK_OP_FLATTEN_CHW,
    IFCBK_OP_STEM_U8_FWD,
    IFCBK_OP_STEM_U8_WGRAD,
    IFCBK_OP_CONV_FWD_AFFINE_MAXPOOL,
    IFCBK_OP_STEP_COUNTERS,
    IFCBK_OP_CONV_WGRAD_GROUP,
    IFCBK_OP_SOFTMAX_XENT_W
};
typedef struct {
    ifcbk_conv_desc d;
    const void* x;
    const void* dy;
    float* dw;
} ifcbk_wgrad_item;
typedef struct {
    int32_t kind;
    int32_t flags;
    void*   p[12];
    int64_t i[4];
    float   f[8];
    union {
        ifcbk_conv_desc conv;
        ifcbk_bn_desc   bn;
        ifcbk_pool_desc pool;
        ifcbk_head_desc head;
    } u;
} ifcbk_op;
IFCBK_API int ifcbk_run_program(ifcbk_ctx*, const ifcbk_op* ops, int n, void* stream, float* op_ms);
IFCBK_API int ifcbk_run_program_ev(ifcbk_ctx*, const ifcbk_op* ops, int n, void* stream, int slot);
IFCBK_API int ifcbk_program_times(ifcbk_ctx*, int slot, int n, float* op_ms);
typedef struct ifcbk_graph ifcbk_graph;
IFCBK_API int ifcbk_program_capture(ifcbk_ctx*, const ifcbk_op* ops, int n, ifcbk_graph** out);
IFCBK_API int ifcbk_graph_launch(ifcbk_ctx*, ifcbk_graph*, void* stream);
IFCBK_API int ifcbk_graph_destroy(ifcbk_ctx*, ifcbk_graph*);
IFCBK_API int ifcbk_op_kernel(const ifcbk_op* op, char* name, size_t cap);
IFCBK_API int ifcbk_op_cost(const ifcbk_op* op, double* flops, double* bytes);

#ifdef __cplusplus
}
#endif
#endif
```

Measured before the change: 12060 images/s.

## Fuse stem BN backward dx into u8 stem weight-gradient kernel

```diff
diff --git a/ifcb_classifier_amd/_lib.py b/ifcb_classifier_amd/_lib.py
--- a/ifcb_classifier_amd/_lib.py
+++ b/ifcb_classifier_amd/_lib.py
@@ -117,6 +117,7 @@
                                    _vp]),
     'ifcbk_bn_bwd_partials_ld': (_i, [_vp, C.POINTER(BnDesc), _vp, _vp, _i, _vp, _vp, _vp, _vp, _vp, _vp, _i, _i, _vp, _i, _vp, _vp,
                                       _i, _vp]),
+    'ifcbk_bn_bwd_sums': (_i, [_vp, C.POINTER(BnDesc), _vp, _vp, _i, _vp, _vp, _vp, _vp, _vp, _vp, _i, _i, _vp, _vp, _i, _vp, _vp]),
     'ifcbk_bn_apply_maxpool': (_i, [_vp, C.POINTER(PoolDesc), _vp, _vp, _vp, _i, _vp, _vp, _vp]),
     'ifcbk_bn_bwd_maxpool': (_i, [_vp, C.POINTER(PoolDesc), _vp, _vp, _vp, _vp, _vp, _vp, _vp, _vp, _i, _vp, _i, _vp, _vp, _i,
                                   _vp]),
@@ -145,6 +146,7 @@
     'ifcbk_stem_u8_fwd': (_i, [_vp, C.POINTER(ConvDesc), _vp, _vp, _vp, _vp, _vp, _vp, _vp, _i, _vp]),
     'ifcbk_stem_u8_wgrad_workspace': (_sz, [C.POINTER(ConvDesc)]),
     'ifcbk_stem_u8_wgrad': (_i, [_vp, C.POINTER(ConvDesc), _vp, _vp, _vp, _vp, _i, _vp]),
+    'ifcbk_stem_u8_wgrad_bn': (_i, [_vp, C.POINTER(ConvDesc), _vp, _vp, _i, _vp, _i, _vp, _vp, _vp, _vp, _vp, _vp, _vp, _vp, _i, _vp]),
     'ifcbk_nchw_to_nhwc': (_i, [_vp, _vp, _i, _i, _i, _i, _i, _i, C.POINTER(_f), C.POINTER(_f), _vp, _vp]),
     'ifcbk_nhwc_to_nchw_f32': (_i, [_vp, _vp, _i, _i, _i, _i, _i, _i, _vp, _vp]),
     'ifcbk_run_program': (_i, [_vp, C.POINTER(Op), _i, _vp, C.POINTER(_f)]),
diff --git a/ifcb_classifier_amd/csrc/bn.hip b/ifcb_classifier_amd/csrc/bn.hip
--- a/ifcb_classifier_amd/csrc/bn.hip
+++ b/ifcb_classifier_amd/csrc/bn.hip
@@ -613,7 +613,8 @@
 int bwd_t(ifcbk_ctx* ctx, const ifcbk_bn_desc* d, const void* x, const void* y, const void* dy, int lddy,
           const float* gamma, const float* mean, const float* invstd, void* dx, int lddx, void* dres, int lddres,
           int dres_accumulate, float* dgamma, float* dbeta, int param_accumulate, const float* scale, const float* shift,
-          hipStream_t st, const PoolGather* pool = nullptr, const float* part_in = nullptr, int ntiles_in = 0, int part_ld_in = 0) {
+          hipStream_t st, const PoolGather* pool = nullptr, const float* part_in = nullptr, int ntiles_in = 0, int part_ld_in = 0,
+          float* sums_out = nullptr) {
     constexpr int E = Chunk<T>::N;
     constexpr int CG = 8 * E;
     PoolGather pg = {};
@@ -631,6 +632,7 @@
     dim3 g1(ntiles, cdiv(C, CG));
     const int mask = !d->relu ? 0 : ((scale && shift && !dres) ? 2 : 1);
     if (mask == 1 && !yy) IFCBK_FAIL(ctx, IFCBK_EINVAL, "bn_bwd: y is required for the ReLU mask");
+    if (!dx && (!sums_out || pool || dres)) IFCBK_FAIL(ctx, IFCBK_EINVAL, "bn_bwd: dx may only be left out with a place for the sums, without pool or residual");
     if (pool && pg.ph == 0 && pg.pw == 0) {
         if (mask == 1) IFCBK_FAIL(ctx, IFCBK_EINVAL, "bn_bwd_maxpool: needs scale/shift (the activation is not stored)");
         const int HB = (pg.H + 1) / 2, WB = (pg.W + 1) / 2;
@@ -668,8 +670,10 @@
     else if (mask == 1) hipLaunchKernelGGL((bn_bwd_reduce_kernel<T, 1, false>), g1, dim3(256), 0, st, xx, d->ldx, yy, d->ldy, dd, lddy, mean, invstd, scale, shift, part, M, C, pg, rows);
     else hipLaunchKernelGGL((bn_bwd_reduce_kernel<T, 0, false>), g1, dim3(256), 0, st, xx, d->ldx, yy, d->ldy, dd, lddy, mean, invstd, scale, shift, part, M, C, pg, rows);
     IFCBK_LAUNCH_CHECK(ctx, "bn_bwd_reduce");
+    if (sums_out) tmp = sums_out;
     if (!experiment_skip_finalize(st)) hipLaunchKernelGGL(bn_bwd_finalize_kernel, dim3(cdiv(C, 16)), dim3(1024), 0, st, (const float*)part, ntiles, C, dgamma, dbeta, tmp, param_accumulate, (part_in && part_ld_in > 0) ? part_ld_in : C);
     IFCBK_LAUNCH_CHECK(ctx, "bn_bwd_finalize");
+    if (!dx) return 0;
     const int64_t total = M * (C / E);
     if (total >= (1ll << 31)) IFCBK_FAIL(ctx, IFCBK_EINVAL, "bn_bwd: tensor too large");
     const float invM = (float)(1.0 / (double)M);
@@ -873,6 +877,20 @@
                                     param_accumulate, stream);
 }
 
+extern "C" int ifcbk_bn_bwd_sums(ifcbk_ctx* ctx, const ifcbk_bn_desc* d, const void* x, const void* dy, int lddy, const float* gamma,
+                                 const float* mean, const float* invstd, const float* scale, const float* shift, const float* part,
+                                 int ntiles, int part_ld, float* dgamma, float* dbeta, int param_accumulate, float* sums, void* stream) {
+    if (!d || !sums || (part && (ntiles <= 0 || part_ld < 0))) IFCBK_FAIL(ctx, IFCBK_EINVAL, "bn_bwd_sums: bad args");
+    if (!d->relu || !scale || !shift) IFCBK_FAIL(ctx, IFCBK_EINVAL, "bn_bwd_sums: ReLU layer with scale/shift (the mask is recomputed from x)");
+    if (d->dtype == IFCBK_F32)
+        return bwd_t<float>(ctx, d, x, nullptr, dy, lddy, gamma, mean, invstd, nullptr, 0, nullptr, 0, 0, dgamma, dbeta,
+                            param_accumulate, scale, shift, (hipStream_t)stream, nullptr, part, ntiles, part_ld, sums);
+    if (d->dtype == IFCBK_BF16)
+        return bwd_t<bf16_t>(ctx, d, x, nullptr, dy, lddy, gamma, mean, invstd, nullptr, 0, nullptr, 0, 0, dgamma, dbeta,
+                             param_accumulate, scale, shift, (hipStream_t)stream, nullptr, part, ntiles, part_ld, sums);
+    IFCBK_FAIL(ctx, IFCBK_EINVAL, "bn_bwd_sums: bad dtype");
+}
+
 extern "C" int ifcbk_bn_bwd_maxpool(ifcbk_ctx* ctx, const ifcbk_pool_desc* d, const void* x, const void* dpool,
                                     const uint8_t* argmax, const float* gamma, const float* mean, const float* invstd,
                                     const float* scale, const float* shift, int relu, void* dx, int lddx, float* dgamma,
diff --git a/ifcb_classifier_amd/csrc/conv_stem_u8.hip b/ifcb_classifier_amd/csrc/conv_stem_u8.hip
--- a/ifcb_classifier_amd/csrc/conv_stem_u8.hip
+++ b/ifcb_classifier_amd/csrc/conv_stem_u8.hip
@@ -20,6 +20,10 @@
     fastdiv_t dPQ, dQ;
     unsigned rows, gpr;
     fastdiv_t dP, dG;
+    const void* x;
+    const float *gamma, *mean, *invstd, *tmp;
+    float invM;
+    int ldx;
 #ifdef IFCBK_EXPERIMENT_STEM
     int dbg;
 #endif
@@ -141,9 +145,26 @@
     }
 }
 
-template <class T>
+__device__ __forceinline__ void stem_bn_coef(const StemArgs& a, float* coef) {
+    constexpr int C = K1;
+    for (int c = threadIdx.x; c < C; c += 256) {
+        float is = a.invstd[c], a_ = a.gamma[c] * is, dg = a.tmp[C + c] * a.invM, db = a.tmp[c] * a.invM;
+        coef[c] = a_;
+        coef[C + c] = -a_ * is * dg;
+        coef[2 * C + c] = a_ * (a.mean[c] * is * dg - db);
+        coef[3 * C + c] = a.scale[c];
+        coef[4 * C + c] = a.shift[c];
+    }
+}
+
+template <class T, bool BN = false>
 __global__ __launch_bounds__(256) void stem_u8_wgrad_kernel(StemArgs a) {
     const int c8 = threadIdx.x & 3, pl = threadIdx.x >> 2;
+    __shared__ float coef[5 * K1];
+    if (BN) {
+        stem_bn_coef(a, coef);
+        __syncthreads();
+    }
     float acc[8][10];
 #pragma unroll
     for (int j = 0; j < 8; ++j)
@@ -151,14 +172,16 @@
         for (int t = 0; t < 10; ++t) acc[j][t] = 0.f;
     const unsigned m0 = blockIdx.x * (unsigned)PIXB + pl;
     const T* dy = (const T*)a.dy;
+    const T* x = (const T*)a.x;
     for (int it = 0; it < PIXB / 64; it += UNR) {
         if (m0 + it * 64 >= a.M) break;
         uint8_t gb[UNR][9];
-        float d[UNR][8];
+        float d[UNR][8], fx[UNR][8];
 #pragma unroll
         for (int u = 0; u < UNR; ++u) {
             const unsigned m = m0 + (it + u) * 64, mc = m < a.M ? m : a.M - 1;
             load8<T>(dy + (size_t)mc * a.ld + c8 * 8, d[u]);
+            if (BN) load8<T>(x + (size_t)mc * a.ldx + c8 * 8, fx[u]);
             taps_raw(a, mc, gb[u]);
         }
 #pragma unroll
@@ -167,6 +190,17 @@
             float gt[9];
 #pragma unroll
             for (int t = 0; t < 9; ++t) gt[t] = (float)gb[u][t];
+            if (BN) {
+                const int c = c8 * 8;
+                constexpr int C = K1;
+#pragma unroll
+                for (int j = 0; j < 8; ++j) {
+                    float dz = d[u][j];
+                    dz = (fx[u][j] * coef[3 * C + c + j] + coef[4 * C + c + j]) > 0.f ? dz : 0.f;
+                    const float o = coef[c + j] * dz + (coef[C + c + j] * fx[u][j] + coef[2 * C + c + j]);
+                    d[u][j] = Chunk<T>::round(o);
+                }
+            }
 #pragma unroll
             for (int j = 0; j < 8; ++j) {
 #pragma unroll
@@ -332,6 +366,93 @@
     }
 }
 
+__device__ __forceinline__ void stem_wgrad_bn_items(const StemArgs& a, f32x4_t& acc0, f32x4_t& acc1) {
+    const int lane = threadIdx.x & 63, wv = __builtin_amdgcn_readfirstlane(threadIdx.x >> 6);
+    const int c = lane & 15, kg = lane >> 4;
+    const int tr = c < 9 ? c / 3 : 0, tc = c < 9 ? c % 3 : 0;
+    const unsigned row0 = blockIdx.x * (unsigned)RB, nitem = (unsigned)RB * a.gpr;
+    const bf16_t* dy = (const bf16_t*)a.dy;
+    __shared__ float coef[5 * K1];
+    __shared__ __attribute__((aligned(16))) bf16_t tile[4][32 * K1];
+    stem_bn_coef(a, coef);
+    __syncthreads();
+    const int c0 = (lane & 3) * 8, px = lane >> 2;
+    float cA[8], cB[8], cK[8], cS[8], cH[8];
+#pragma unroll
+    for (int j = 0; j < 8; ++j) {
+        cA[j] = coef[c0 + j]; cB[j] = coef[K1 + c0 + j]; cK[j] = coef[2 * K1 + c0 + j];
+        cS[j] = coef[3 * K1 + c0 + j]; cH[j] = coef[4 * K1 + c0 + j];
+    }
+    const bf16_t* x = (const bf16_t*)a.x;
+    typedef __attribute__((address_space(3))) void* lptr_t;
+    uint4* wr = reinterpret_cast<uint4*>(tile[wv]) + lane;
+    const unsigned rd = (unsigned)(size_t)(lptr_t)(tile[wv]) + (unsigned)((8 * kg + (c >> 2)) * 64 + (c & 3) * 8);
+    struct Item { uint4 d[2], x[2]; unsigned gb[8], row, grp; };
+    auto fetch = [&](unsigned item, Item& t) {
+        const unsigned rr = fdiv(item, a.dG);
+        t.grp = item - rr * a.gpr;
+        t.row = row0 + rr;
+        const unsigned rowc = t.row < a.rows ? t.row : a.rows - 1;
+        const unsigned n = fdiv(rowc, a.dP), p = rowc - n * (unsigned)a.P;
+#pragma unroll
+        for (int u = 0; u < 2; ++u) {
+            const unsigned q = t.grp * 32 + px + 16 * u, qc = q < (unsigned)a.Q ? q : (unsigned)a.Q - 1;
+            const size_t pix = (size_t)rowc * a.Q + qc;
+            t.d[u] = *reinterpret_cast<const uint4*>(dy + pix * a.ld + c0);
+            t.x[u] = *reinterpret_cast<const uint4*>(x + pix * a.ldx + c0);
+        }
+        const uint8_t* s = a.g + ((size_t)n * a.H + 2 * p + tr) * a.W + tc;
+#pragma unroll
+        for (int e = 0; e < 8; ++e) {
+            const unsigned q = t.grp * 32 + 8 * kg + e, qc = q < (unsigned)a.Q ? q : (unsigned)a.Q - 1;
+            t.gb[e] = s[2 * qc];
+        }
+    };
+    auto trip = [&](const Item& cu, Item& nx, unsigned next) -> bool {
+        if (cu.row >= a.rows) return false;
+        fetch(next < nitem ? next : next - 4, nx);
+        __builtin_amdgcn_sched_barrier(0);
+#pragma unroll
+        for (int u = 0; u < 2; ++u) {
+            float fd[8], fx[8], o[8];
+            unpack8(cu.d[u], fd);
+            unpack8(cu.x[u], fx);
+#pragma unroll
+            for (int j = 0; j < 8; ++j) {
+                float dz = fd[j];
+                dz = (fx[j] * cS[j] + cH[j]) > 0.f ? dz : 0.f;
+                o[j] = cA[j] * dz + (cB[j] * fx[j] + cK[j]);
+            }
+            uint4 v = pack8(o);
+            if (cu.grp * 32 + px + 16 * u >= (unsigned)a.Q) v = make_uint4(0u, 0u, 0u, 0u);
+            wr[64 * u] = v;
+        }
+        s16x4_t a0l, a0h, a1l, a1h;
+        asm volatile("ds_read_b64_tr_b16 %0, %4\n\tds_read_b64_tr_b16 %1, %4 offset:256\n\t"
+                     "ds_read_b64_tr_b16 %2, %4 offset:32\n\tds_read_b64_tr_b16 %3, %4 offset:288\n\t"
+                     "s_waitcnt lgkmcnt(0)"
+                     : "=&v"(a0l), "=&v"(a0h), "=&v"(a1l), "=&v"(a1h)
+                     : "v"(rd)
+                     : "memory");
+        unsigned g16[8];
+#pragma unroll
+        for (int e = 0; e < 8; ++e) g16[e] = c < 9 ? bfbits((float)cu.gb[e]) : (c == 9 ? 0x3f80u : 0u);
+        const bf16x8_t A0 = __builtin_bit_cast(bf16x8_t, __builtin_shufflevector(a0l, a0h, 0, 1, 2, 3, 4, 5, 6, 7));
+        const bf16x8_t A1 = __builtin_bit_cast(bf16x8_t, __builtin_shufflevector(a1l, a1h, 0, 1, 2, 3, 4, 5, 6, 7));
+        const bf16x8_t B = frag(bfpair(g16[0], g16[1]), bfpair(g16[2], g16[3]), bfpair(g16[4], g16[5]), bfpair(g16[6], g16[7]));
+        acc0 = __builtin_amdgcn_mfma_f32_16x16x32_bf16(A0, B, acc0, 0, 0, 0);
+        acc1 = __builtin_amdgcn_mfma_f32_16x16x32_bf16(A1, B, acc1, 0, 0, 0);
+        return next < nitem;
+    };
+    Item ia, ib;
+    fetch(wv, ia);
+    for (unsigned item = wv;; item += 8) {
+        if (!trip(ia, ib, item + 4)) break;
+        if (!trip(ib, ia, item + 8)) break;
+    }
+}
+
+template <bool BN = false>
 __global__ __launch_bounds__(256) void stem_u8_wgrad_mfma_kernel(StemArgs a) {
     const int lane = threadIdx.x & 63, wv = __builtin_amdgcn_readfirstlane(threadIdx.x >> 6);
     const int c = lane & 15, kg = lane >> 4;
@@ -339,6 +460,8 @@
     f32x4_t acc0 = {0.f, 0.f, 0.f, 0.f}, acc1 = {0.f, 0.f, 0.f, 0.f};
     const unsigned row0 = blockIdx.x * (unsigned)RB, nitem = (unsigned)RB * a.gpr;
     const bf16_t* dy = (const bf16_t*)a.dy;
+    if (BN) stem_wgrad_bn_items(a, acc0, acc1);
+    else
     for (unsigned item = wv; item < nitem; item += 4) {
         const unsigned rr = fdiv(item, a.dG), grp = item - rr * a.gpr, row = row0 + rr;
         if (row >= a.rows) break;
@@ -486,3 +609,28 @@
     IFCBK_LAUNCH_CHECK(ctx, "stem_u8_wgrad_reduce");
     return IFCBK_OK;
 }
+
+extern "C" int ifcbk_stem_u8_wgrad_bn(ifcbk_ctx* ctx, const ifcbk_conv_desc* d, const uint8_t* g, const void* dact, int lddact,
+                                      const void* raw, int ldraw, const float* gamma, const float* mean, const float* invstd,
+                                      const float* scale, const float* shift, const float* sums, const float* ab, float* dw,
+                                      int accumulate, void* stream) {
+    if (!stem_ok(d)) IFCBK_FAIL(ctx, IFCBK_EUNSUPPORTED, "stem_u8_wgrad_bn: 3x3 / stride 2 / unpadded / 32 output channels / Cw = 3 only");
+    if (!g || !dact || !raw || !gamma || !mean || !invstd || !scale || !shift || !sums || !ab || !dw)
+        IFCBK_FAIL(ctx, IFCBK_EINVAL, "stem_u8_wgrad_bn: null operand");
+    if (lddact < K1 || lddact % 8 || ldraw < K1 || ldraw % 8) IFCBK_FAIL(ctx, IFCBK_EINVAL, "stem_u8_wgrad_bn: row strides must be multiples of 8, >= 32");
+    const size_t need = ifcbk_stem_u8_wgrad_workspace(d);
+    if (need > ctx->ws_bytes) IFCBK_FAIL(ctx, IFCBK_ENOMEM, "stem_u8_wgrad_bn: workspace %zu > reserved %zu", need, ctx->ws_bytes);
+    StemArgs a = stem_args(d, g, nullptr, ab);
+    a.dy = dact; a.ld = lddact; a.x = raw; a.ldx = ldraw; a.part = (float*)ctx->ws;
+    a.gamma = gamma; a.mean = mean; a.invstd = invstd; a.scale = scale; a.shift = shift; a.tmp = sums;
+    a.invM = (float)(1.0 / (double)a.M);
+    const int nblk = ifcbk_stem_u8_rows(d);
+    hipStream_t st = (hipStream_t)stream;
+    if (d->dtype == IFCBK_F32) hipLaunchKernelGGL((stem_u8_wgrad_kernel<float, true>), dim3(nblk), dim3(256), 0, st, a);
+    else if (stem_mfma(d)) hipLaunchKernelGGL(stem_u8_wgrad_mfma_kernel<true>, dim3(nblk), dim3(256), 0, st, a);
+    else hipLaunchKernelGGL((stem_u8_wgrad_kernel<bf16_t, true>), dim3(nblk), dim3(256), 0, st, a);
+    IFCBK_LAUNCH_CHECK(ctx, "stem_u8_wgrad_bn");
+    hipLaunchKernelGGL(stem_u8_wgrad_reduce_kernel, dim3(K1), dim3(640), 0, st, (const float*)ctx->ws, nblk, ab, dw, accumulate);
+    IFCBK_LAUNCH_CHECK(ctx, "stem_u8_wgrad_reduce");
+    return IFCBK_OK;
+}
diff --git a/ifcb_classifier_amd/csrc/ctx.hip b/ifcb_classifier_amd/csrc/ctx.hip
--- a/ifcb_classifier_amd/csrc/ctx.hip
+++ b/ifcb_classifier_amd/csrc/ctx.hip
@@ -140,6 +140,10 @@
             return ifcbk_stem_u8_fwd(c, &o->u.conv, (const uint8_t*)p[0], (const float*)p[1], (const float*)p[2], p[3], (float*)p[4],
                                      (const float*)p[5], (const float*)p[6], (o->flags >> 2) & 1, st);
         case IFCBK_OP_STEM_U8_WGRAD:
+            if (p[4])
+                return ifcbk_stem_u8_wgrad_bn(c, &o->u.conv, (const uint8_t*)p[0], p[1], (int)o->i[0], p[4], (int)o->i[1], (const float*)p[5],
+                                              (const float*)p[6], (const float*)p[7], (const float*)p[8], (const float*)p[9],
+                                              (const float*)p[10], (const float*)p[2], (float*)p[3], acc, st);
             return ifcbk_stem_u8_wgrad(c, &o->u.conv, (const uint8_t*)p[0], p[1], (const float*)p[2], (float*)p[3], acc, st);
         case IFCBK_OP_CONV_WGRAD_SEG: {
             float* dws[4];
@@ -157,6 +161,10 @@
         case IFCBK_OP_BN_APPLY:
             return ifcbk_bn_apply(c, &o->u.bn, p[0], (const float*)p[1], (const float*)p[2], p[3], (int)o->i[0], p[4], st);
         case IFCBK_OP_BN_BWD:
+            if (!p[6])
+                return ifcbk_bn_bwd_sums(c, &o->u.bn, p[0], p[2], (int)o->i[0], (const float*)p[3], (const float*)p[4], (const float*)p[5],
+                                         (const float*)p[10], (const float*)p[11], nullptr, 0, 0, (float*)p[8], (float*)p[9], pacc,
+                                         (float*)p[7], st);
             return ifcbk_bn_bwd(c, &o->u.bn, p[0], p[1], p[2], (int)o->i[0], (const float*)p[3], (const float*)p[4],
                                 (const float*)p[5], p[6], (int)o->i[1], p[7], (int)o->i[2], acc | (((o->flags >> 3) & 1) << 1), (float*)p[8], (float*)p[9],
                                 pacc, (const float*)p[10], (const float*)p[11], st);
@@ -164,6 +172,10 @@
             return ifcbk_conv2d_dgrad_bnstat(c, &o->u.conv, p[0], p[1], p[2], p[3], (int)o->i[0], (const float*)p[4], (const float*)p[5],
                                              (const float*)p[6], (const float*)p[7], (float*)p[8], st);
         case IFCBK_OP_BN_BWD_PARTIALS:
+            if (!p[8])
+                return ifcbk_bn_bwd_sums(c, &o->u.bn, p[0], p[1], (int)o->i[0], (const float*)p[2], (const float*)p[3], (const float*)p[4],
+                                         (const float*)p[5], (const float*)p[6], (const float*)p[7], (int)o->i[1], (int)o->i[3],
+                                         (float*)p[9], (float*)p[10], pacc, (float*)p[11], st);
             return ifcbk_bn_bwd_partials_ld(c, &o->u.bn, p[0], p[1], (int)o->i[0], (const float*)p[2], (const float*)p[3], (const float*)p[4],
                                             (const float*)p[5], (const float*)p[6], (const float*)p[7], (int)o->i[1], (int)o->i[3], p[8],
                                             (int)o->i[2], (float*)p[9], (float*)p[10], pacc, st);
@@ -574,10 +586,14 @@
         }
         case IFCBK_OP_CONV_FWD_AFFINE_MAXPOOL: snprintf(name, cap, "conv_rows3x3<%d, %d, true>", o->u.conv.C, o->u.conv.K); break;
         case IFCBK_OP_STEM_U8_FWD: snprintf(name, cap, "stem_u8_fwd_kernel"); break;
-        case IFCBK_OP_STEM_U8_WGRAD: snprintf(name, cap, "stem_u8_wgrad_kernel"); break;
+        case IFCBK_OP_STEM_U8_WGRAD:
+            if (!o->p[4]) snprintf(name, cap, "stem_u8_wgrad_kernel");
+            else if (o->u.conv.dtype == IFCBK_BF16 && o->u.conv.Q >= 32) snprintf(name, cap, "stem_u8_wgrad_mfma_kernel<true>");
+            else snprintf(name, cap, "stem_u8_wgrad_kernel<%s, true>", o->u.conv.dtype == IFCBK_F32 ? "float" : "unsigned short");
+            break;
         case IFCBK_OP_BN_APPLY: snprintf(name, cap, "bn_apply_kernel"); break;
-        case IFCBK_OP_BN_BWD: snprintf(name, cap, "bn_bwd"); break;
-        case IFCBK_OP_BN_BWD_PARTIALS: snprintf(name, cap, "bn_bwd(partials)"); break;
+        case IFCBK_OP_BN_BWD: snprintf(name, cap, o->p[6] ? "bn_bwd" : "bn_bwd(no dx)"); break;
+        case IFCBK_OP_BN_BWD_PARTIALS: snprintf(name, cap, o->p[8] ? "bn_bwd(partials)" : "bn_bwd_finalize_kernel"); break;
         case IFCBK_OP_BN_APPLY_MAXPOOL: snprintf(name, cap, "bn_apply_maxpool_kernel"); break;
         case IFCBK_OP_BN_BWD_MAXPOOL: snprintf(name, cap, "bn_bwd(maxpool)"); break;
         case IFCBK_OP_BN_FINALIZE: snprintf(name, cap, "bn_finalize_kernel"); break;
@@ -630,12 +646,16 @@
             const ifcbk_conv_desc& d = o->u.conv;
             fl = 2.0 * d.N * d.P * d.Q * d.K * d.R * d.S * d.Cw;
             by = (double)d.N * d.H * d.W + (double)d.N * d.P * d.Q * d.K * 2;
+            if (o->kind == IFCBK_OP_STEM_U8_WGRAD && o->p[4]) by += (double)d.N * d.P * d.Q * d.K * 2;
             break;
         }
         case IFCBK_OP_BN_APPLY: by = (double)o->u.bn.M * o->u.bn.C * (2 + 2 + (o->p[3] ? 2 : 0)); break;
         case IFCBK_OP_BN_STATS: by = (double)o->u.bn.M * o->u.bn.C * 2; break;
-        case IFCBK_OP_BN_BWD: by = (double)o->u.bn.M * o->u.bn.C * (2.0 * (o->u.bn.relu ? 6 : 4) + 2 + (o->p[7] ? 2 : 0)); break;
-        case IFCBK_OP_BN_BWD_PARTIALS: by = (double)o->u.bn.M * o->u.bn.C * (2 + 2 + 2); break;
+        case IFCBK_OP_BN_BWD:
+            if (!o->p[6]) by = (double)o->u.bn.M * o->u.bn.C * (2 + 2);
+            else by = (double)o->u.bn.M * o->u.bn.C * (2.0 * (o->u.bn.relu ? 6 : 4) + 2 + (o->p[7] ? 2 : 0));
+            break;
+        case IFCBK_OP_BN_BWD_PARTIALS: by = o->p[8] ? (double)o->u.bn.M * o->u.bn.C * (2 + 2 + 2) : 0.0; break;
         case IFCBK_OP_BN_APPLY_MAXPOOL: {
             const ifcbk_pool_desc& d = o->u.pool;
             by = ((double)d.N * d.H * d.W * 2 + (double)d.N * d.P * d.Q * 3) * d.C;
diff --git a/ifcb_classifier_amd/engine.py b/ifcb_classifier_amd/engine.py
--- a/ifcb_classifier_amd/engine.py
+++ b/ifcb_classifier_amd/engine.py
@@ -499,6 +499,11 @@
             self.in_u8 = [torch.zeros(N, net.S, net.S, dtype=torch.uint8, device=dev) for _ in range(2)]
             self.in_ab = [torch.zeros(6, dtype=torch.float32, device=dev) for _ in range(2)]
             self._in_ab_host = [None, None]
+            self.stem_sums = torch.zeros(2 * first[0].K, dtype=torch.float32, device=dev)
+        fuse_dx = os.environ.get('IFCBK_STEM_FUSE_DX', '1')
+        if fuse_dx not in ('0', '1'):
+            raise ValueError('IFCBK_STEM_FUSE_DX must be 0 or 1, got %r' % fuse_dx)
+        self.stem_fuse_dx = fuse_dx == '1'
         self.in_kind = ['nhwc', 'nhwc']
         self.pre_stream = self.pre_ctx = None
         self.ev_ready, self.ev_free, self.prefetched = [None, None], [None, None], None
@@ -736,6 +741,8 @@
             if getattr(self, '_draw_pool', None) is None:
                 tot = 0
                 for m in self.convs:
+                    if m is self.stem_u8 and self.stem_fuse_dx and self.in_kind[self.in_slot] == 'u8':
+                        continue
                     if m.group is None or m.cpool is not None:
                         tot += (self.train_batch * m.P * m.Q * m.K + 127) // 128 * 128
                 for gq in self.groups:
@@ -1124,7 +1131,12 @@
                 _, n, d, bnd, draw, wT, needs_dgrad = g
                 wgq = wg_of.get(n)
                 own = wgq is not None or (self.wgrad_lane and (n.group is None or n.cpool is not None))
-                if own:
+                fuse_dx = (self.stem_fuse_dx and self.stem_u8 is n and self.in_kind[self.in_slot] == 'u8' and not needs_dgrad
+                           and n.residual is None and n.group is None and n.relu and n not in fused_pool and wgq is None)
+                rsum = ('ssum', id(n), 0, 1)
+                if fuse_dx:
+                    own, draw, sums = False, None, _vp(self.stem_sums)
+                elif own:
                     draw = _vp(own_draw(n))
                 elif self.wgrad_lane:
                     draw = _vp(group_draw(n.group), self.esize * n.koff)
@@ -1144,6 +1156,8 @@
                 rdraw = [rdg(n)] if (grp is not None and not cp) else [('draw', L, 0, 1)]
                 if own:
                     rdraw = [('drawn', id(n), 0, 1)]
+                if fuse_dx:
+                    rdraw = [rsum]
                 rawp, _ld = self._raw_ptr(n)
                 if n in fused_pool:
                     pn, pk = fused_pool[n]
@@ -1158,13 +1172,13 @@
                     bwd.add(_lib.OP_BN_BWD_PARTIALS, n.name,
                             p=(rawp, self._aptr(n.y, True), self._pptr(bkey + '.weight'), self._stat(n, 0), self._stat(n, 1),
                                self._stat(n, 2), self._stat(n, 3), ppart, draw, self._pptr(bkey + '.weight', 'G'),
-                               self._pptr(bkey + '.bias', 'G')),
+                               self._pptr(bkey + '.bias', 'G')) + ((sums,) if fuse_dx else ()),
                             i=(n.y.buf.C, nrow, n.K if (grp is None or cp) else grp.Ktot, 0), bn=bnd, lane=L,
                             reads=[rraw(n), rg(n.y), rst(n), pres], writes=rdraw)
                 else:
                     bwd.add(_lib.OP_BN_BWD, n.name,
                             p=(rawp, self._aptr(n.y), self._aptr(n.y, True), self._pptr(bkey + '.weight'),
-                               self._stat(n, 0), self._stat(n, 1), draw, dres, self._pptr(bkey + '.weight', 'G'),
+                               self._stat(n, 0), self._stat(n, 1), draw, sums if fuse_dx else dres, self._pptr(bkey + '.weight', 'G'),
                                self._pptr(bkey + '.bias', 'G'), self._stat(n, 2), self._stat(n, 3)),
                             i=(n.y.buf.C, n.K if (grp is None or cp) else grp.Ktot, lddres), flags=dres_acc, bn=bnd, lane=L,
                             reads=[rraw(n), ra(n.y), rg(n.y), rst(n)],
@@ -1205,6 +1219,12 @@
                         bwd.add(_lib.OP_CONV_WGRAD_GROUP, '+'.join(m.name for m in mem),
                                 p=[C.addressof(items)] + [items[kq].dw for kq in range(len(mem))], i=(len(mem),), lane=L if LW is None else LW,
                                 reads=[ra(m.x) for m in mem] + [('drawn', id(m), 0, 1) for m in mem], writes=[])
+                elif fuse_dx:
+                    bwd.add(_lib.OP_STEM_U8_WGRAD, n.name,
+                            p=(_vp(self.in_u8[self.in_slot]), self._aptr(n.y, True), _vp(self.in_ab[self.in_slot]), self._pptr(ckey, 'G'),
+                               rawp, self._pptr(bkey + '.weight'), self._stat(n, 0), self._stat(n, 1), self._stat(n, 2), self._stat(n, 3),
+                               sums), i=(n.y.buf.C, _ld), conv=dbw, lane=L if LW is None else LW,
+                            reads=[ra(n.x), rraw(n), rg(n.y), rst(n), rsum], writes=[])
                 elif self.stem_u8 is n and self.in_kind[self.in_slot] == 'u8':
                     bwd.add(_lib.OP_STEM_U8_WGRAD, n.name,
                             p=(_vp(self.in_u8[self.in_slot]), draw, _vp(self.in_ab[self.in_slot]), self._pptr(ckey, 'G')), conv=dbw,
diff --git a/include/ifcbk.h b/include/ifcbk.h
--- a/include/ifcbk.h
+++ b/include/ifcbk.h
@@ -163,6 +163,10 @@
 IFCBK_API size_t ifcbk_stem_u8_wgrad_workspace(const ifcbk_conv_desc*);
 IFCBK_API int ifcbk_stem_u8_wgrad(ifcbk_ctx*, const ifcbk_conv_desc* d, const uint8_t* g, const void* dy, const float* ab, float* dw,
                         int accumulate, void* stream);
+IFCBK_API int ifcbk_stem_u8_wgrad_bn(ifcbk_ctx*, const ifcbk_conv_desc* d, const uint8_t* g, const void* dact, int lddact,
+                           const void* raw, int ldraw, const float* gamma, const float* mean, const float* invstd,
+                           const float* scale, const float* shift, const float* sums, const float* ab, float* dw,
+                           int accumulate, void* stream);
 IFCBK_API int ifcbk_nchw_to_nhwc(ifcbk_ctx*, const float* x, int N, int C, int H, int W, int Cpad, int dtype,
                        const float* scale3, const float* shift3, void* y, void* stream);
 IFCBK_API int ifcbk_nhwc_to_nchw_f32(ifcbk_ctx*, const void* x, int N, int C, int H, int W, int ldx, int dtype,
@@ -192,6 +196,9 @@
                              const float* gamma, const float* mean, const float* invstd, const float* scale,
                              const float* shift, const float* part, int ntiles, int part_ld, void* dx, int lddx,
                              float* dgamma, float* dbeta, int param_accumulate, void* stream);
+IFCBK_API int ifcbk_bn_bwd_sums(ifcbk_ctx*, const ifcbk_bn_desc*, const void* x, const void* dy, int lddy, const float* gamma,
+                      const float* mean, const float* invstd, const float* scale, const float* shift, const float* part,
+                      int ntiles, int part_ld, float* dgamma, float* dbeta, int param_accumulate, float* sums, void* stream);
 
 IFCBK_API int ifcbk_bias_relu_bwd(ifcbk_ctx*, int64_t M, int K, int dtype, const void* y, int ldy, const void* dy, int lddy, void* dz,
                         int lddz, int relu, float* dbias, int param_accumulate, void* stream);
```

Measured after the change: 12160 images/s, median of 6. No clear change (+0.8%).
